# libmir/mir-optim

Measured on AMD Instinct MI355X. Metric: LM iterations/sec, higher is better.
Workload: dtype f64

## Files before the change

include/mir_optim_amd.h:

```cpp
#ifndef MIR_OPTIM_AMD_H
#define MIR_OPTIM_AMD_H

#include <stddef.h>
#include <stdint.h>

#ifdef __cplusplus
extern "C" {
#endif


typedef enum mir_least_squares_status {
    mir_ls_maxIterations = -1,
    mir_ls_furtherImprovement = 0,
    mir_ls_xConverged = 1,
    mir_ls_gConverged = 2,
    mir_ls_fConverged = 3,
    mir_ls_badBounds = -32,
    mir_ls_badGuess = -31,
    mir_ls_badMinStepQuality = -30,
    mir_ls_badGoodStepQuality = -29,
    mir_ls_badStepQuality = -28,
    mir_ls_badLambdaParams = -27,
    mir_ls_numericError = -26
} mir_least_squares_status;

typedef enum mir_box_qp_status {
    mir_box_qp_solved = 0,
    mir_box_qp_numericError = 1,
    mir_box_qp_maxIterations = 2
} mir_box_qp_status;

typedef struct mir_box_qp_settings_d { double relTolerance, absTolerance; uint32_t maxIterations; } mir_box_qp_settings_d;
typedef struct mir_box_qp_settings_s { float relTolerance, absTolerance; uint32_t maxIterations; } mir_box_qp_settings_s;

typedef struct mir_least_squares_settings_d {
    uint32_t maxIterations;
    uint32_t maxAge;
    double jacobianEpsilon;
    double absTolerance;
    double relTolerance;
    double gradTolerance;
    double maxGoodResidual;
    double maxStep;
    double maxLambda;
    double minLambda;
    double minStepQuality;
    double goodStepQuality;
    double lambdaIncrease;
    double lambdaDecrease;
    mir_box_qp_settings_d qpSettings;
} mir_least_squares_settings_d;

typedef struct mir_least_squares_settings_s {
    uint32_t maxIterations, maxAge;
    float jacobianEpsilon, absTolerance, relTolerance, gradTolerance, maxGoodResidual, maxStep,
          maxLambda, minLambda, minStepQuality, goodStepQuality, lambdaIncrease, lambdaDecrease;
    mir_box_qp_settings_s qpSettings;
} mir_least_squares_settings_s;

typedef struct mir_least_squares_result_d {
    int32_t status;
    uint32_t iterations, fCalls, gCalls;
    double residual;
    double lambda;
} mir_least_squares_result_d;
typedef struct mir_least_squares_result_s {
    int32_t status;
    uint32_t iterations, fCalls, gCalls;
    float residual, lambda;
} mir_least_squares_result_s;

typedef struct mir_slice_d { size_t length; double* ptr; } mir_slice_d;
typedef struct mir_slice_s { size_t length; float* ptr; } mir_slice_s;
typedef struct mir_slice_i { size_t length; int32_t* ptr; } mir_slice_i;

typedef void (*mir_least_squares_function_d)(void* context, size_t m, size_t n, const double* x, double* y);
typedef void (*mir_least_squares_jacobian_d)(void* context, size_t m, size_t n, const double* x, double* J);
typedef void (*mir_least_squares_function_s)(void* context, size_t m, size_t n, const float* x, float* y);
typedef void (*mir_least_squares_jacobian_s)(void* context, size_t m, size_t n, const float* x, float* J);

typedef struct mir_least_squares_task { void* context; void* function; } mir_least_squares_task;
typedef void (*mir_least_squares_task_function)(mir_least_squares_task task, uint32_t totalThreads,
                                                uint32_t threadId, uint32_t i);
typedef void (*mir_least_squares_thread_manager)(void* context, uint32_t count,
                                                 mir_least_squares_task taskContext,
                                                 mir_least_squares_task_function task);

size_t mir_least_squares_work_length(size_t m, size_t n);
size_t mir_least_squares_iwork_length(size_t m, size_t n);
size_t mir_box_qp_work_length(size_t n);
size_t mir_box_qp_iwork_length(size_t n);
size_t mir_box_qp_iwork_length_ilp64(size_t n);
size_t mir_least_squares_iwork_length_ilp64(size_t m, size_t n);
const char* mir_least_squares_status_string(mir_least_squares_status st);
void mir_least_squares_init_d(mir_least_squares_settings_d* settings);
void mir_least_squares_init_s(mir_least_squares_settings_s* settings);
void mir_least_squares_reset_d(mir_least_squares_settings_d* settings);
void mir_least_squares_reset_s(mir_least_squares_settings_s* settings);

mir_least_squares_result_d mir_optimize_least_squares_d(
    const mir_least_squares_settings_d* settings, size_t m, size_t n,
    double* x, const double* l, const double* u,
    mir_slice_d work, mir_slice_i iwork,
    void* fContext, mir_least_squares_function_d f,
    void* gContext, mir_least_squares_jacobian_d g,
    void* tmContext, mir_least_squares_thread_manager tm);

mir_least_squares_result_s mir_optimize_least_squares_s(
    const mir_least_squares_settings_s* settings, size_t m, size_t n,
    float* x, const float* l, const float* u,
    mir_slice_s work, mir_slice_i iwork,
    void* fContext, mir_least_squares_function_s f,
    void* gContext, mir_least_squares_jacobian_s g,
    void* tmContext, mir_least_squares_thread_manager tm);


typedef struct mir_lsq_comm mir_lsq_comm;
typedef struct mir_lsq_workspace mir_lsq_workspace;

typedef void (*mir_lsq_batched_function_d)(void* context, size_t m, size_t n, size_t p, const double* X, double* Y);
typedef void (*mir_lsq_batched_function_s)(void* context, size_t m, size_t n, size_t p, const float* X, float* Y);
enum {
    MIR_LSQ_DEVICE_CALLBACKS = 1u,
    MIR_LSQ_TIME_KERNELS = 2u
};

enum {
    MIR_LSQ_VARIANT_BROYDEN_REWRITE = 1u << 0,
    MIR_LSQ_VARIANT_FD_SEPARATE_FILL = 1u << 1,
    MIR_LSQ_VARIANT_NO_SPECULATION = 1u << 4,
    MIR_LSQ_VARIANT_NO_NULL_SKIP = 1u << 5,
    MIR_LSQ_VARIANT_SOLVE_BOUNDED = 1u << 6,
    MIR_LSQ_VARIANT_SOLVE_GENERIC = 1u << 10,
    MIR_LSQ_VARIANT_SOLVE_ONE_WORKGROUP = 1u << 11,
    MIR_LSQ_VARIANT_FD_HOST_COLUMNS = 1u << 13,
    MIR_LSQ_VARIANT_NO_PIPELINE = 1u << 22,
    MIR_LSQ_VARIANT_DEBUG_HELPERS_ABSENT = 1u << 12,
    MIR_LSQ_VARIANT_DEBUG_SOLVE = 1u << 7,
    MIR_LSQ_VARIANT_HOST_PROFILE = 1u << 8,
    MIR_LSQ_VARIANT_LR_CAP_SHIFT = 16
};

typedef struct mir_lsq_stats {
    uint64_t passes, accepted, rejected, step_guard_rejects;
    uint64_t jacobian_full, jacobian_broyden;
    uint64_t jtj_launches;
    uint64_t jtj_broyden_launches;
    double jtj_ms;
    double jtj_broyden_ms;
    double solve_ms;
    uint64_t solve_launches;
    double fd_ms;
    double total_ms;
    uint64_t qp_active_set_passes;
    uint64_t broyden_lr_columns;
    double jtj_fd_ms;
    uint64_t jtj_fd_launches;
    uint64_t elided_evaluations;
    uint64_t allreduce_calls[3];
    uint64_t allreduce_elems[3];
    uint64_t broyden_flushes;
    uint64_t jtj_resyncs;
    double fd_callback_ms;
    uint64_t fd_callback_calls, fd_callback_points;
    double trial_callback_ms;
    uint64_t trial_callback_calls, trial_callback_points;
    uint64_t library_launches;
    uint64_t round_launches[3];
    uint64_t rounds[3];
    double fd_host_wall_ms, fd_host_f_ms;
    uint64_t fd_host_columns;
    double host_f_ms;
    uint64_t host_f_calls;
    uint64_t fused_rounds;
    uint64_t fused_passes;
    uint64_t coop_timeouts;
} mir_lsq_stats;

typedef struct mir_lsq_trace_record {
    int32_t event;
    uint32_t iterations;
    double lambda, residual, trial_residual, dx_dot;
} mir_lsq_trace_record;
typedef struct mir_lsq_trace {
    mir_lsq_trace_record* records;
    uint64_t capacity;
    uint64_t count;
} mir_lsq_trace;

typedef struct mir_lsq_gpu_options {
    uint32_t struct_size;
    uint32_t flags;
    void* stream;
    mir_lsq_comm* comm;
    mir_lsq_workspace* workspace;
    void* fbContext;
    void* fb;
    uint32_t fd_batch;
    uint32_t variant;
    mir_lsq_stats* stats;
    mir_lsq_trace* trace;
    void* fbRowMajor;
    void* fbRowMajorDiff;
    uint32_t stats_size;
    uint32_t reserved0;
} mir_lsq_gpu_options;

mir_least_squares_result_d mir_optimize_least_squares_gpu_d(
    const mir_least_squares_settings_d* settings, size_t m, size_t n,
    double* x, const double* l, const double* u, const mir_lsq_gpu_options* options,
    void* fContext, mir_least_squares_function_d f,
    void* gContext, mir_least_squares_jacobian_d g,
    void* tmContext, mir_least_squares_thread_manager tm);
mir_least_squares_result_s mir_optimize_least_squares_gpu_s(
    const mir_least_squares_settings_s* settings, size_t m, size_t n,
    float* x, const float* l, const float* u, const mir_lsq_gpu_options* options,
    void* fContext, mir_least_squares_function_s f,
    void* gContext, mir_least_squares_jacobian_s g,
    void* tmContext, mir_least_squares_thread_manager tm);

int mir_solve_box_qp_gpu_d(const mir_box_qp_settings_d* settings, size_t n, const double* P,
                           const double* q, const double* l, const double* u, double* x,
                           int unconstrainedSolution, int* iterations);
int mir_solve_box_qp_gpu_s(const mir_box_qp_settings_s* settings, size_t n, const float* P,
                           const float* q, const float* l, const float* u, float* x,
                           int unconstrainedSolution, int* iterations);

enum { MIR_LSQ_MODEL_EXP_DECAY = 0, MIR_LSQ_MODEL_EXP3_AFFINE = 1,
       MIR_LSQ_MODEL_EXP_DECAY_PAD8 = 2 };
enum { MIR_LSQ_BATCHED_ANALYTIC_JACOBIAN = 2 };
enum { MIR_LSQ_BATCHED_NO_LADDER = 1 };
typedef struct mir_lsq_batched_options {
    uint32_t struct_size;
    uint32_t variant;
    void* stream;
    float* basis;
    size_t basis_bytes;
    uint64_t* timing;
} mir_lsq_batched_options;

int mir_optimize_least_squares_batched_s(const mir_least_squares_settings_s* settings, size_t count, size_t m, int model,
                                         float* x, const float* lower, const float* upper,
                                         const float* t, size_t t_stride, const float* data,
                                         mir_least_squares_result_s* results, const mir_lsq_batched_options* options);

enum { MIR_LSQ_BATCHED_NEEDS_GENERAL = -100 };
int mir_lsq_batched_kernel_s(const mir_least_squares_settings_s* settings, size_t count, size_t m, int model,
                             float* x, const float* lower, const float* upper,
                             const float* t, size_t t_stride, const float* data,
                             mir_least_squares_result_s* results, const mir_lsq_batched_options* options);

int mir_optimize_least_squares_batched_d(const mir_least_squares_settings_d* settings, size_t count, size_t m, int model,
                                         double* x, const double* lower, const double* upper,
                                         const double* t, size_t t_stride, const double* data,
                                         mir_least_squares_result_d* results, const mir_lsq_batched_options* options);
int mir_lsq_batched_kernel_d(const mir_least_squares_settings_d* settings, size_t count, size_t m, int model,
                             double* x, const double* lower, const double* upper,
                             const double* t, size_t t_stride, const double* data,
                             mir_least_squares_result_d* results, const mir_lsq_batched_options* options);

enum { MIR_LSQ_BATCHED_ABSOLUTE_SIGMA = 1u };
typedef struct mir_lsq_batched_extras {
    uint32_t struct_size;
    uint32_t flags;
    const void* weights;
    size_t weight_stride;
    void* covariance;
} mir_lsq_batched_extras;
int mir_optimize_least_squares_batched_ex_s(const mir_least_squares_settings_s* settings, size_t count, size_t m, int model,
                                            float* x, const float* lower, const float* upper,
                                            const float* t, size_t t_stride, const float* data,
                                            mir_least_squares_result_s* results, const mir_lsq_batched_options* options,
                                            const mir_lsq_batched_extras* extras);
int mir_optimize_least_squares_batched_ex_d(const mir_least_squares_settings_d* settings, size_t count, size_t m, int model,
                                            double* x, const double* lower, const double* upper,
                                            const double* t, size_t t_stride, const double* data,
                                            mir_least_squares_result_d* results, const mir_lsq_batched_options* options,
                                            const mir_lsq_batched_extras* extras);
int mir_lsq_batched_kernel_ex_s(const mir_least_squares_settings_s* settings, size_t count, size_t m, int model,
                                float* x, const float* lower, const float* upper,
                                const float* t, size_t t_stride, const float* data,
                                mir_least_squares_result_s* results, const mir_lsq_batched_options* options,
                                const mir_lsq_batched_extras* extras);
int mir_lsq_batched_kernel_ex_d(const mir_least_squares_settings_d* settings, size_t count, size_t m, int model,
                                double* x, const double* lower, const double* upper,
                                const double* t, size_t t_stride, const double* data,
                                mir_least_squares_result_d* results, const mir_lsq_batched_options* options,
                                const mir_lsq_batched_extras* extras);
int mir_lsq_batched_covariance_s(const mir_least_squares_settings_s* settings, size_t count, size_t m, int model,
                                 const float* x, const float* lower, const float* upper,
                                 const float* t, size_t t_stride, const float* data,
                                 const mir_least_squares_result_s* results, const mir_lsq_batched_options* options,
                                 const mir_lsq_batched_extras* extras);
int mir_lsq_batched_covariance_d(const mir_least_squares_settings_d* settings, size_t count, size_t m, int model,
                                 const double* x, const double* lower, const double* upper,
                                 const double* t, size_t t_stride, const double* data,
                                 const mir_least_squares_result_d* results, const mir_lsq_batched_options* options,
                                 const mir_lsq_batched_extras* extras);

enum { MIR_LSQ_RESIDENT_NO_NULL_SKIP = 1u,
       MIR_LSQ_RESIDENT_UNBOUNDED = 2u,
       MIR_LSQ_RESIDENT_NO_LOOKAHEAD = 4u,
       MIR_LSQ_RESIDENT_DEBUG_DROP_WORKGROUP = 16u,
       MIR_LSQ_RESIDENT_ANALYTIC_JACOBIAN = 32u,
       MIR_LSQ_RESIDENT_NO_STAMPS = 8u           };
typedef struct mir_lsq_resident_stats {
    uint64_t rounds, passes, accepted, rejected, step_guard_rejects, jacobian_full, jacobian_broyden, qp_active_set_passes,
        elided_evaluations;
    uint64_t t_total, t_stage, t_worker, t_group, t_total_wait, t_solver, t_solve_body, t_cmd_wait;
    uint64_t t_w_eval, t_w_fd, t_w_prod;
    uint64_t t_w_mma;
    uint64_t lookahead_rejections;
    uint64_t t_look;
    uint64_t t_unpack, t_publish;
    uint32_t abort_code, grid, rows, groups;
} mir_lsq_resident_stats;
typedef struct mir_lsq_resident_options {
    uint32_t struct_size;
    uint32_t variant;
    void* stream;
    void* workspace;
    size_t workspace_bytes;
    mir_lsq_trace_record* trace_records;
    uint32_t trace_capacity;
    uint32_t max_workgroups;
    uint32_t* trace_count;
    mir_lsq_resident_stats* stats;
} mir_lsq_resident_options;

int mir_lsq_batched_posvx_s(size_t count, size_t n, const float* P, const float* rhs, float* x, int* info, void* stream);
int mir_lsq_batched_posvx_d(size_t count, size_t n, const double* P, const double* rhs, double* x, int* info, void* stream);

int mir_lsq_jtj_d(size_t m, size_t n, double* J, const double* y, const double* y_old, const double* dx,
                  int broyden, double* JJ, double* Jy, void* stream, float* kernel_ms);
int mir_lsq_jtj_s(size_t m, size_t n, float* J, const float* y, const float* y_old, const float* dx,
                  int broyden, float* JJ, float* Jy, void* stream, float* kernel_ms);
int mir_lsq_fd_jtj_d(size_t m, size_t n, const double* Yrm, const double* twh, const double* y, double* J,
                     double* JJ, double* Jy, void* stream, float* kernel_ms);
int mir_lsq_fd_diff_jtj_d(size_t m, size_t n, const double* Drm, const double* twh, const double* y, double* J,
                          double* JJ, double* Jy, void* stream, float* kernel_ms);
int mir_lsq_jtj_plan(size_t elem_size, size_t m, size_t n, int num_cu, int op, int aligned16, size_t out[10]);

mir_lsq_workspace* mir_lsq_workspace_create(size_t m, size_t n, size_t elem_size);
void mir_lsq_workspace_destroy(mir_lsq_workspace* ws);

int mir_lsq_rccl_unique_id(void* out_128_bytes);
mir_lsq_comm* mir_lsq_comm_create_rccl(int nranks, int rank, const void* unique_id_128_bytes);
typedef void (*mir_lsq_allreduce_fn)(void* ctx, double* device_buf, size_t count, void* stream);
mir_lsq_comm* mir_lsq_comm_create_callback(int nranks, int rank, mir_lsq_allreduce_fn fn, void* ctx);
int mir_lsq_comm_create_local_group(int nranks, mir_lsq_comm** out_comms);
void mir_lsq_comm_destroy(mir_lsq_comm* comm);
int mir_lsq_comm_record(mir_lsq_comm* comm, double* host_buf, size_t capacity);
size_t mir_lsq_comm_recorded(const mir_lsq_comm* comm);
mir_lsq_comm* mir_lsq_comm_create_replay(int nranks, int rank, const double* totals_host, size_t len, mir_lsq_comm* inner);
int mir_lsq_comm_replay_rewind(mir_lsq_comm* comm);
int mir_lsq_comm_replay_set_delay(mir_lsq_comm* comm, unsigned microseconds);
int mir_lsq_comm_ranks(const mir_lsq_comm* comm);
int mir_lsq_comm_describe(const mir_lsq_comm* comm, char* buf, size_t len);
int mir_lsq_comm_allreduce_d(mir_lsq_comm* comm, double* buf, size_t count, void* stream);
int mir_lsq_comm_allreduce_s(mir_lsq_comm* comm, float* buf, size_t count, void* stream);

int mir_lsq_device_count(void);
void* mir_lsq_device_malloc(size_t bytes);
void mir_lsq_device_free(void* p);
int mir_lsq_memcpy_h2d(void* dst_device, const void* src_host, size_t bytes, void* stream);
int mir_lsq_memcpy_d2h(void* dst_host, const void* src_device, size_t bytes, void* stream);
int mir_lsq_memcpy_d2d(void* dst_device, const void* src_device, size_t bytes, void* stream);

int mir_lsq_selftest_reductions(int rounds, int mismatches[4]);
void* mir_lsq_stream_create(void);
void mir_lsq_stream_destroy(void* stream);
int mir_lsq_stream_synchronize(void* stream);
const char* mir_lsq_version(void);

enum { MIR_FIT_SPLINE_OK = 0, MIR_FIT_SPLINE_TOO_FEW_POINTS = 1, MIR_FIT_SPLINE_BAD_ARGUMENT = 2 };

int mir_fit_spline_d(const mir_least_squares_settings_d* settings, size_t npoints, const double* points, size_t nx,
                     const double* x, const double* l, const double* u, double lambda, double (*dist)(double, double),
                     double* splineY, double* splineD, mir_least_squares_result_d* result);
int mir_fit_spline_s(const mir_least_squares_settings_s* settings, size_t npoints, const float* points, size_t nx,
                     const float* x, const float* l, const float* u, float lambda, float (*dist)(float, float),
                     float* splineY, float* splineD, mir_least_squares_result_s* result);
void mir_fit_spline_residuals_d(size_t npoints, const double* points, size_t nx, const double* x, double lambda,
                                const double* splineY, size_t m, double* y);
void mir_spline_c2_derivatives_d(size_t n, const double* x, const double* y, double* d);
void mir_spline_c2_derivatives_s(size_t n, const float* x, const float* y, float* d);
void mir_spline_eval_d(size_t n, const double* x, const double* y, const double* d, double t, double* out3);
void mir_spline_eval_s(size_t n, const float* x, const float* y, const float* d, float t, float* out3);

#ifdef __cplusplus
}
#endif
#endif
```

mir_optim_amd/api.py:

```python
import ctypes as C
import enum
import os

import numpy as np

from . import build as _build

__all__ = [
    "LeastSquaresStatus", "BoxQPStatus", "LeastSquaresSettings", "LeastSquaresResult", "BoxQPSettings",
    "LeastSquaresException", "optimize", "optimizeLeastSquares", "solveBoxQP", "leastSquaresStatusString",
    "mir_least_squares_work_length", "mir_least_squares_iwork_length", "mir_box_qp_work_length",
    "mir_box_qp_iwork_length", "GpuOptions", "Stats", "lib", "workloads_lib", "device_count",
    "DeviceBuffer", "Stream", "jtj", "fd_jtj", "DEVICE_CALLBACKS", "TIME_KERNELS", "optimizeLeastSquaresBatched", "batchedPosvx", "BATCHED_NO_LADDER",
    "MODEL_EXP_DECAY", "MODEL_EXP3_AFFINE", "MODEL_EXP_DECAY_PAD8", "ResultS", "Trace", "TraceRecord", "Spline", "FitSplineResult", "fitSpline",
    "fit_spline_residuals", "variant_lr_cap",
    "VARIANT_BROYDEN_REWRITE", "VARIANT_FD_SEPARATE_FILL", "VARIANT_NO_SPECULATION", "VARIANT_NO_NULL_SKIP",
    "VARIANT_SOLVE_BOUNDED", "VARIANT_DEBUG_SOLVE", "VARIANT_HOST_PROFILE", "VARIANT_SOLVE_GENERIC", "VARIANT_SOLVE_ONE_WORKGROUP", "VARIANT_DEBUG_HELPERS_ABSENT", "VARIANT_FD_HOST_COLUMNS",
    "VARIANT_NO_PIPELINE", "BatchedOptions", "BatchedExtras", "BATCHED_ABSOLUTE_SIGMA",
]

MODEL_EXP_DECAY = 0
MODEL_EXP3_AFFINE = 1
MODEL_EXP_DECAY_PAD8 = 2

DEVICE_CALLBACKS = 1
TIME_KERNELS = 2

VARIANT_BROYDEN_REWRITE = 1 << 0
VARIANT_FD_SEPARATE_FILL = 1 << 1
VARIANT_NO_SPECULATION = 1 << 4
VARIANT_NO_NULL_SKIP = 1 << 5
VARIANT_SOLVE_BOUNDED = 1 << 6
VARIANT_DEBUG_SOLVE = 1 << 7
VARIANT_HOST_PROFILE = 1 << 8
VARIANT_SOLVE_GENERIC = 1 << 10
VARIANT_SOLVE_ONE_WORKGROUP = 1 << 11
VARIANT_DEBUG_HELPERS_ABSENT = 1 << 12
VARIANT_FD_HOST_COLUMNS = 1 << 13
VARIANT_NO_PIPELINE = 1 << 22


def variant_lr_cap(k):
    return (int(k) & 31) << 16


class LeastSquaresStatus(enum.IntEnum):
    maxIterations = -1
    furtherImprovement = 0
    xConverged = 1
    gConverged = 2
    fConverged = 3
    badBounds = -32
    badGuess = -31
    badMinStepQuality = -30
    badGoodStepQuality = -29
    badStepQuality = -28
    badLambdaParams = -27
    numericError = -26


class BoxQPStatus(enum.IntEnum):
    solved = 0
    numericError = 1
    maxIterations = 2


class LeastSquaresException(Exception):

    def __init__(self, status, result=None):
        self.status = LeastSquaresStatus(status)
        self.result = result
        super().__init__("mir-optim Least Squares: " + leastSquaresStatusString(status))


class _QPd(C.Structure):
    _fields_ = [("relTolerance", C.c_double), ("absTolerance", C.c_double), ("maxIterations", C.c_uint32)]


class _QPs(C.Structure):
    _fields_ = [("relTolerance", C.c_float), ("absTolerance", C.c_float), ("maxIterations", C.c_uint32)]


_FIELDS = ["jacobianEpsilon", "absTolerance", "relTolerance", "gradTolerance", "maxGoodResidual", "maxStep",
           "maxLambda", "minLambda", "minStepQuality", "goodStepQuality", "lambdaIncrease", "lambdaDecrease"]


class _Sd(C.Structure):
    _fields_ = ([("maxIterations", C.c_uint32), ("maxAge", C.c_uint32)] + [(k, C.c_double) for k in _FIELDS]
                + [("qpSettings", _QPd)])


class _Ss(C.Structure):
    _fields_ = ([("maxIterations", C.c_uint32), ("maxAge", C.c_uint32)] + [(k, C.c_float) for k in _FIELDS]
                + [("qpSettings", _QPs)])


class _Rd(C.Structure):
    _fields_ = [("status", C.c_int32), ("iterations", C.c_uint32), ("fCalls", C.c_uint32), ("gCalls", C.c_uint32),
                ("residual", C.c_double), ("lambda_", C.c_double)]


class _Rs(C.Structure):
    _fields_ = [("status", C.c_int32), ("iterations", C.c_uint32), ("fCalls", C.c_uint32), ("gCalls", C.c_uint32),
                ("residual", C.c_float), ("lambda_", C.c_float)]


ResultS = _Rs


class _SliceD(C.Structure):
    _fields_ = [("length", C.c_size_t), ("ptr", C.c_void_p)]


class _Task(C.Structure):
    _fields_ = [("context", C.c_void_p), ("function", C.c_void_p)]


class Stats(C.Structure):
    _fields_ = [("passes", C.c_uint64), ("accepted", C.c_uint64), ("rejected", C.c_uint64),
                ("step_guard_rejects", C.c_uint64), ("jacobian_full", C.c_uint64), ("jacobian_broyden", C.c_uint64),
                ("jtj_launches", C.c_uint64), ("jtj_broyden_launches", C.c_uint64), ("jtj_ms", C.c_double),
                ("jtj_broyden_ms", C.c_double), ("solve_ms", C.c_double), ("solve_launches", C.c_uint64),
                ("fd_ms", C.c_double), ("total_ms", C.c_double), ("qp_active_set_passes", C.c_uint64),
                ("broyden_lr_columns", C.c_uint64),
                ("jtj_fd_ms", C.c_double), ("jtj_fd_launches", C.c_uint64),
                ("elided_evaluations", C.c_uint64),
                ("allreduce_calls", C.c_uint64 * 3), ("allreduce_elems", C.c_uint64 * 3),
                ("broyden_flushes", C.c_uint64), ("jtj_resyncs", C.c_uint64),
                ("fd_callback_ms", C.c_double), ("fd_callback_calls", C.c_uint64), ("fd_callback_points", C.c_uint64),
                ("trial_callback_ms", C.c_double), ("trial_callback_calls", C.c_uint64),
                ("trial_callback_points", C.c_uint64),
                ("library_launches", C.c_uint64), ("round_launches", C.c_uint64 * 3), ("rounds", C.c_uint64 * 3),
                ("fd_host_wall_ms", C.c_double), ("fd_host_f_ms", C.c_double), ("fd_host_columns", C.c_uint64),
                ("host_f_ms", C.c_double), ("host_f_calls", C.c_uint64),
                ("fused_rounds", C.c_uint64), ("fused_passes", C.c_uint64), ("coop_timeouts", C.c_uint64)]

    def as_dict(self):
        return {k: (list(getattr(self, k)) if isinstance(getattr(self, k), C.Array) else getattr(self, k)) for k, _ in self._fields_}


class TraceRecord(C.Structure):
    _fields_ = [("event", C.c_int32), ("iterations", C.c_uint32), ("lambda_", C.c_double), ("residual", C.c_double),
                ("trial_residual", C.c_double), ("dx_dot", C.c_double)]


class _TraceHeader(C.Structure):
    _fields_ = [("records", C.POINTER(TraceRecord)), ("capacity", C.c_uint64), ("count", C.c_uint64)]


class Trace:

    EVENTS = {0: "jacobian_full", 1: "jacobian_broyden", 2: "rejected", 3: "accepted", 4: "step_guard"}

    def __init__(self, capacity=4096):
        self._buf = (TraceRecord * capacity)()
        self.header = _TraceHeader(C.cast(self._buf, C.POINTER(TraceRecord)), capacity, 0)

    @property
    def count(self):
        return int(self.header.count)

    def records(self):
        k = min(self.count, int(self.header.capacity))
        return [(r.event, r.iterations, r.lambda_, r.residual, r.trial_residual, r.dx_dot) for r in self._buf[:k]]


class GpuOptions(C.Structure):
    _fields_ = [("struct_size", C.c_uint32), ("flags", C.c_uint32), ("stream", C.c_void_p), ("comm", C.c_void_p),
                ("workspace", C.c_void_p), ("fbContext", C.c_void_p), ("fb", C.c_void_p), ("fd_batch", C.c_uint32),
                ("variant", C.c_uint32), ("stats", C.POINTER(Stats)), ("trace", C.POINTER(_TraceHeader)),
                ("fbRowMajor", C.c_void_p), ("fbRowMajorDiff", C.c_void_p), ("stats_size", C.c_uint32),
                ("reserved0", C.c_uint32)]

    def __init__(self, **kw):
        super().__init__(**kw)
        self.struct_size = C.sizeof(GpuOptions)
        self.stats_size = C.sizeof(Stats)


class BatchedOptions(C.Structure):
    _fields_ = [("struct_size", C.c_uint32), ("variant", C.c_uint32), ("stream", C.c_void_p), ("basis", C.c_void_p),
                ("basis_bytes", C.c_size_t), ("timing", C.c_void_p)]

    def __init__(self, **kw):
        super().__init__(**kw)
        self.struct_size = C.sizeof(BatchedOptions)


class BatchedExtras(C.Structure):
    _fields_ = [("struct_size", C.c_uint32), ("flags", C.c_uint32), ("weights", C.c_void_p), ("weight_stride", C.c_size_t),
                ("covariance", C.c_void_p)]

    def __init__(self, **kw):
        super().__init__(**kw)
        self.struct_size = C.sizeof(BatchedExtras)


TASK_FN = C.CFUNCTYPE(None, _Task, C.c_uint32, C.c_uint32, C.c_uint32)
TM_FN = C.CFUNCTYPE(None, C.c_void_p, C.c_uint32, _Task, TASK_FN)
ALLREDUCE_FN = C.CFUNCTYPE(None, C.c_void_p, C.c_void_p, C.c_size_t, C.c_void_p)


def _ftype(dtype):
    ct = C.c_double if dtype == np.float64 else C.c_float
    return C.CFUNCTYPE(None, C.c_void_p, C.c_size_t, C.c_size_t, C.POINTER(ct), C.POINTER(ct))


_lib = None
_wl = None


def _load(path):
    if not os.path.exists(path):
        raise ImportError(f"{path} is missing: build it with `python -m mir_optim_amd.build` "
                          "(hipcc --offload-arch=gfx950). mir_optim_amd has no CPU fallback.")
    return C.CDLL(path, mode=C.RTLD_GLOBAL)


def lib():
    global _lib
    if _lib is None:
        L = _load(_build.SOLVER_LIB)
        sz = C.c_size_t
        for name in ("mir_least_squares_work_length", "mir_least_squares_iwork_length"):
            getattr(L, name).restype = sz
            getattr(L, name).argtypes = [sz, sz]
        for name in ("mir_box_qp_work_length", "mir_box_qp_iwork_length"):
            getattr(L, name).restype = sz
            getattr(L, name).argtypes = [sz]
        L.mir_box_qp_iwork_length_ilp64.restype = sz
        L.mir_box_qp_iwork_length_ilp64.argtypes = [sz]
        L.mir_least_squares_iwork_length_ilp64.restype = sz
        L.mir_least_squares_iwork_length_ilp64.argtypes = [sz, sz]
        L.mir_least_squares_status_string.restype = C.c_char_p
        L.mir_least_squares_status_string.argtypes = [C.c_int]
        for suf, S, R in (("d", _Sd, _Rd), ("s", _Ss, _Rs)):
            getattr(L, "mir_least_squares_init_" + suf).argtypes = [C.POINTER(S)]
            getattr(L, "mir_least_squares_reset_" + suf).argtypes = [C.POINTER(S)]
            fn = getattr(L, "mir_optimize_least_squares_" + suf)
            fn.restype = R
            fn.argtypes = [C.POINTER(S), sz, sz, C.c_void_p, C.c_void_p, C.c_void_p, _SliceD, _SliceD,
                           C.c_void_p, C.c_void_p, C.c_void_p, C.c_void_p, C.c_void_p, C.c_void_p]
            fn = getattr(L, "mir_optimize_least_squares_gpu_" + suf)
            fn.restype = R
            fn.argtypes = [C.POINTER(S), sz, sz, C.c_void_p, C.c_void_p, C.c_void_p, C.POINTER(GpuOptions),
                           C.c_void_p, C.c_void_p, C.c_void_p, C.c_void_p, C.c_void_p, C.c_void_p]
            fn = getattr(L, "mir_solve_box_qp_gpu_" + suf)
            fn.restype = C.c_int
            fn.argtypes = [C.c_void_p, sz, C.c_void_p, C.c_void_p, C.c_void_p, C.c_void_p, C.c_void_p, C.c_int,
                           C.POINTER(C.c_int)]
            fn = getattr(L, "mir_lsq_jtj_" + suf)
            fn.restype = C.c_int
            fn.argtypes = [sz, sz, C.c_void_p, C.c_void_p, C.c_void_p, C.c_void_p, C.c_int, C.c_void_p, C.c_void_p,
                           C.c_void_p, C.POINTER(C.c_float)]
        L.mir_lsq_comm_create_local_group.restype = C.c_int
        L.mir_lsq_comm_create_local_group.argtypes = [C.c_int, C.POINTER(C.c_void_p)]
        L.mir_lsq_fd_diff_jtj_d.restype = C.c_int
        L.mir_lsq_fd_diff_jtj_d.argtypes = [sz, sz, C.c_void_p, C.c_void_p, C.c_void_p, C.c_void_p, C.c_void_p, C.c_void_p,
                                            C.c_void_p, C.POINTER(C.c_float)]
        L.mir_lsq_fd_jtj_d.restype = C.c_int
        L.mir_lsq_fd_jtj_d.argtypes = [sz, sz, C.c_void_p, C.c_void_p, C.c_void_p, C.c_void_p, C.c_void_p, C.c_void_p,
                                       C.c_void_p, C.c_void_p]
        L.mir_optimize_least_squares_batched_s.restype = C.c_int
        L.mir_optimize_least_squares_batched_s.argtypes = [C.POINTER(_Ss), sz, sz, C.c_int, C.c_void_p, C.c_void_p, C.c_void_p,
                                                           C.c_void_p, sz, C.c_void_p, C.c_void_p, C.POINTER(BatchedOptions)]
        L.mir_lsq_batched_kernel_s.restype = C.c_int
        L.mir_lsq_batched_kernel_s.argtypes = [C.POINTER(_Ss), sz, sz, C.c_int, C.c_void_p, C.c_void_p, C.c_void_p,
                                               C.c_void_p, sz, C.c_void_p, C.c_void_p, C.POINTER(BatchedOptions)]
        L.mir_lsq_jtj_plan.restype = C.c_int
        L.mir_lsq_jtj_plan.argtypes = [sz, sz, sz, C.c_int, C.c_int, C.c_int, C.POINTER(sz * 10)]
        L.mir_lsq_selftest_reductions.restype = C.c_int
        L.mir_lsq_selftest_reductions.argtypes = [C.c_int, C.POINTER(C.c_int * 4)]
        L.mir_lsq_batched_posvx_s.restype = C.c_int
        L.mir_lsq_batched_posvx_s.argtypes = [sz, sz, C.c_void_p, C.c_void_p, C.c_void_p, C.c_void_p, C.c_void_p]
        L.mir_optimize_least_squares_batched_d.restype = C.c_int
        L.mir_optimize_least_squares_batched_d.argtypes = [C.POINTER(_Sd), sz, sz, C.c_int, C.c_void_p, C.c_void_p, C.c_void_p,
                                                           C.c_void_p, sz, C.c_void_p, C.c_void_p, C.POINTER(BatchedOptions)]
        L.mir_lsq_batched_kernel_d.restype = C.c_int
        L.mir_lsq_batched_kernel_d.argtypes = [C.POINTER(_Sd), sz, sz, C.c_int, C.c_void_p, C.c_void_p, C.c_void_p,
                                               C.c_void_p, sz, C.c_void_p, C.c_void_p, C.POINTER(BatchedOptions)]
        L.mir_lsq_batched_posvx_d.restype = C.c_int
        L.mir_lsq_batched_posvx_d.argtypes = [sz, sz, C.c_void_p, C.c_void_p, C.c_void_p, C.c_void_p, C.c_void_p]
        for suf, S in (("s", _Ss), ("d", _Sd)):
            for name in ("mir_optimize_least_squares_batched_ex_", "mir_lsq_batched_kernel_ex_", "mir_lsq_batched_covariance_"):
                fn = getattr(L, name + suf)
                fn.restype = C.c_int
                fn.argtypes = [C.POINTER(S), sz, sz, C.c_int, C.c_void_p, C.c_void_p, C.c_void_p, C.c_void_p, sz, C.c_void_p,
                               C.c_void_p, C.POINTER(BatchedOptions), C.POINTER(BatchedExtras)]
        L.mir_lsq_comm_describe.restype = C.c_int
        L.mir_lsq_comm_describe.argtypes = [C.c_void_p, C.c_char_p, C.c_size_t]
        L.mir_lsq_workspace_create.restype = C.c_void_p
        L.mir_lsq_workspace_create.argtypes = [sz, sz, sz]
        L.mir_lsq_workspace_destroy.argtypes = [C.c_void_p]
        L.mir_lsq_rccl_unique_id.restype = C.c_int
        L.mir_lsq_rccl_unique_id.argtypes = [C.c_void_p]
        L.mir_lsq_comm_create_rccl.restype = C.c_void_p
        L.mir_lsq_comm_create_rccl.argtypes = [C.c_int, C.c_int, C.c_void_p]
        L.mir_lsq_comm_create_callback.restype = C.c_void_p
        L.mir_lsq_comm_create_callback.argtypes = [C.c_int, C.c_int, ALLREDUCE_FN, C.c_void_p]
        L.mir_lsq_comm_destroy.argtypes = [C.c_void_p]
        L.mir_lsq_comm_record.restype = C.c_int
        L.mir_lsq_comm_record.argtypes = [C.c_void_p, C.c_void_p, sz]
        L.mir_lsq_comm_recorded.restype = sz
        L.mir_lsq_comm_recorded.argtypes = [C.c_void_p]
        L.mir_lsq_comm_create_replay.restype = C.c_void_p
        L.mir_lsq_comm_create_replay.argtypes = [C.c_int, C.c_int, C.c_void_p, sz, C.c_void_p]
        L.mir_lsq_comm_replay_rewind.restype = C.c_int
        L.mir_lsq_comm_replay_rewind.argtypes = [C.c_void_p]
        L.mir_lsq_comm_replay_set_delay.restype = C.c_int
        L.mir_lsq_comm_replay_set_delay.argtypes = [C.c_void_p, C.c_uint]
        L.mir_lsq_comm_ranks.restype = C.c_int
        L.mir_lsq_comm_ranks.argtypes = [C.c_void_p]
        for name in ("mir_lsq_comm_allreduce_d", "mir_lsq_comm_allreduce_s"):
            getattr(L, name).restype = C.c_int
            getattr(L, name).argtypes = [C.c_void_p, C.c_void_p, sz, C.c_void_p]
        L.mir_lsq_device_count.restype = C.c_int
        L.mir_lsq_device_malloc.restype = C.c_void_p
        L.mir_lsq_device_malloc.argtypes = [sz]
        L.mir_lsq_device_free.argtypes = [C.c_void_p]
        for name in ("mir_lsq_memcpy_h2d", "mir_lsq_memcpy_d2h", "mir_lsq_memcpy_d2d"):
            getattr(L, name).restype = C.c_int
            getattr(L, name).argtypes = [C.c_void_p, C.c_void_p, sz, C.c_void_p]
        L.mir_lsq_stream_create.restype = C.c_void_p
        L.mir_lsq_stream_destroy.argtypes = [C.c_void_p]
        L.mir_lsq_stream_synchronize.restype = C.c_int
        L.mir_lsq_stream_synchronize.argtypes = [C.c_void_p]
        L.mir_lsq_version.restype = C.c_char_p
        for suf, S, R, ct in (("d", _Sd, _Rd, C.c_double), ("s", _Ss, _Rs, C.c_float)):
            fn = getattr(L, "mir_fit_spline_" + suf)
            fn.restype = C.c_int
            fn.argtypes = [C.POINTER(S), sz, C.c_void_p, sz, C.c_void_p, C.c_void_p, C.c_void_p, ct, C.c_void_p,
                           C.c_void_p, C.c_void_p, C.POINTER(R)]
            getattr(L, "mir_spline_c2_derivatives_" + suf).argtypes = [sz, C.c_void_p, C.c_void_p, C.c_void_p]
            getattr(L, "mir_spline_eval_" + suf).argtypes = [sz, C.c_void_p, C.c_void_p, C.c_void_p, ct, C.c_void_p]
        L.mir_fit_spline_residuals_d.argtypes = [sz, C.c_void_p, sz, C.c_void_p, C.c_double, C.c_void_p, sz, C.c_void_p]
        _lib = L
    return _lib


def workloads_lib():
    global _wl
    if _wl is None:
        W = _load(_build.WORKLOADS_LIB)
        W.wl_uniform.argtypes = [C.c_uint64, C.c_uint64, C.c_size_t, C.c_void_p]
        W.wl_tanh_linear_generate.argtypes = [C.c_size_t, C.c_size_t, C.c_size_t, C.c_double, C.c_void_p, C.c_void_p,
                                              C.c_void_p, C.c_void_p]
        _wl = W
    return _wl


def device_count():
    return lib().mir_lsq_device_count()


def leastSquaresStatusString(st):
    return lib().mir_least_squares_status_string(int(st)).decode()


def mir_least_squares_work_length(m, n):
    return lib().mir_least_squares_work_length(m, n)


def mir_least_squares_iwork_length(m, n):
    return lib().mir_least_squares_iwork_length(m, n)


def mir_box_qp_work_length(n):
    return lib().mir_box_qp_work_length(n)


def mir_box_qp_iwork_length(n):
    return lib().mir_box_qp_iwork_length(n)


def LeastSquaresSettings(dtype=np.float64):
    s = _Sd() if dtype == np.float64 else _Ss()
    (lib().mir_least_squares_init_d if dtype == np.float64 else lib().mir_least_squares_init_s)(C.byref(s))
    return s


def BoxQPSettings(dtype=np.float64):
    return LeastSquaresSettings(dtype).qpSettings


class LeastSquaresResult:

    def __init__(self, raw):
        self.status = LeastSquaresStatus(raw.status)
        self.iterations = raw.iterations
        self.fCalls = raw.fCalls
        self.gCalls = raw.gCalls
        self.residual = raw.residual
        self.lambda_ = raw.lambda_

    def __repr__(self):
        return (f"LeastSquaresResult(status={self.status.name}, iterations={self.iterations}, fCalls={self.fCalls}, "
                f"gCalls={self.gCalls}, residual={self.residual!r}, lambda={self.lambda_!r})")


class Stream:
    def __init__(self):
        self.handle = lib().mir_lsq_stream_create()
        if not self.handle:
            raise RuntimeError("hipStreamCreate failed (no GPU?)")

    def synchronize(self):
        if lib().mir_lsq_stream_synchronize(self.handle) != 0:
            raise RuntimeError("stream synchronize failed")

    def close(self):
        if self.handle:
            lib().mir_lsq_stream_destroy(self.handle)
            self.handle = None

    def __del__(self):
        try:
            self.close()
        except Exception:
            pass


class DeviceBuffer:

    def __init__(self, array=None, nbytes=None, dtype=None, shape=None):
        if array is not None:
            array = np.ascontiguousarray(array)
            nbytes, dtype, shape = array.nbytes, array.dtype, array.shape
        self.nbytes, self.dtype, self.shape = int(nbytes), np.dtype(dtype), tuple(shape)
        self.ptr = lib().mir_lsq_device_malloc(max(self.nbytes, 8))
        if not self.ptr:
            raise MemoryError(f"hipMalloc({self.nbytes}) failed (no GPU?)")
        if array is not None:
            self.upload(array)

    def upload(self, array):
        array = np.ascontiguousarray(array, dtype=self.dtype)
        assert array.nbytes == self.nbytes
        if lib().mir_lsq_memcpy_h2d(self.ptr, array.ctypes.data, self.nbytes, None) != 0:
            raise RuntimeError("H2D copy failed")

    def upload_at(self, byte_offset, array):
        array = np.ascontiguousarray(array, dtype=self.dtype)
        assert 0 <= byte_offset and byte_offset + array.nbytes <= self.nbytes
        if lib().mir_lsq_memcpy_h2d(self.ptr + byte_offset, array.ctypes.data, array.nbytes, None) != 0:
            raise RuntimeError("H2D copy failed")

    def download(self):
        out = np.empty(self.shape, dtype=self.dtype)
        if lib().mir_lsq_memcpy_d2h(out.ctypes.data, self.ptr, self.nbytes, None) != 0:
            raise RuntimeError("D2H copy failed")
        return out

    def free(self):
        if self.ptr:
            lib().mir_lsq_device_free(self.ptr)
            self.ptr = None

    def __del__(self):
        try:
            self.free()
        except Exception:
            pass


def _as_fnptr(cb, ftype, wrap, keep):
    if cb is None:
        return C.c_void_p(None)
    if callable(cb):
        c = ftype(wrap(cb))
        keep.append(c)
        return C.cast(c, C.c_void_p)
    return C.c_void_p(int(cb))


def optimizeLeastSquares(f, m, x, l=None, u=None, g=None, tm=None, settings=None, dtype=np.float64,
                         fContext=None, gContext=None, options=None, gpu_entry=None):
    L = lib()
    dbl = dtype == np.float64
    x = np.ascontiguousarray(x, dtype=dtype)
    n = x.size
    lo = np.full(n, -np.inf, dtype=dtype) if l is None else np.ascontiguousarray(l, dtype=dtype)
    up = np.full(n, np.inf, dtype=dtype) if u is None else np.ascontiguousarray(u, dtype=dtype)
    if settings is None:
        settings = LeastSquaresSettings(dtype)
    ft = _ftype(dtype)
    keep = []
    errors = []

    def wrap_f(fn):
        def cb(_ctx, m_, n_, xp, yp):
            yv = np.ctypeslib.as_array(yp, shape=(m_,))
            try:
                xv = np.ctypeslib.as_array(xp, shape=(n_,))
                yv[:] = 0
                fn(xv, yv)
            except BaseException as e:
                errors.append(e)
                yv[:] = np.nan
        return cb

    def wrap_g(fn):
        def cb(_ctx, m_, n_, xp, Jp):
            Jv = np.ctypeslib.as_array(Jp, shape=(m_ * n_,)).reshape(m_, n_)
            try:
                xv = np.ctypeslib.as_array(xp, shape=(n_,))
                Jv[:] = 0
                fn(xv, Jv)
            except BaseException as e:
                errors.append(e)
                Jv[:] = np.nan
        return cb

    fptr = _as_fnptr(f, ft, wrap_f, keep)
    gptr = _as_fnptr(g, ft, wrap_g, keep)
    tmptr = C.c_void_p(None)
    if tm is not None:
        def tm_cb(_ctx, count, task, taskfn):
            try:
                tm(count, lambda total, tid, i: taskfn(task, total, tid, i))
            except BaseException as e:
                errors.append(e)
        tmc = TM_FN(tm_cb)
        keep.append(tmc)
        tmptr = C.cast(tmc, C.c_void_p)
    use_gpu_entry = gpu_entry if gpu_entry is not None else (options is not None)
    suf = "d" if dbl else "s"
    if use_gpu_entry:
        fn = getattr(L, "mir_optimize_least_squares_gpu_" + suf)
        raw = fn(C.byref(settings), m, n, x.ctypes.data, lo.ctypes.data, up.ctypes.data,
                 C.byref(options) if options is not None else None, fContext, fptr, gContext, gptr, None, tmptr)
    else:
        wl = L.mir_least_squares_work_length(m, n)
        iwl = L.mir_least_squares_iwork_length(m, n)
        iwork = np.zeros(iwl + 4, dtype=np.int32)
        work_slice = _SliceD(wl, None)
        iwork_slice = _SliceD(iwl, iwork.ctypes.data)
        fn = getattr(L, "mir_optimize_least_squares_" + suf)
        raw = fn(C.byref(settings), m, n, x.ctypes.data, lo.ctypes.data, up.ctypes.data, work_slice, iwork_slice,
                 fContext, fptr, gContext, gptr, None, tmptr)
    del keep
    if errors:
        raise errors[0]
    return LeastSquaresResult(raw), x


def optimize(f, m, x, l=None, u=None, g=None, tm=None, settings=None, dtype=np.float64, taskPool=None, **kw):
    if taskPool is not None and tm is None:
        import threading
        workers = max(1, getattr(taskPool, "_max_workers", 1))
        ids = {}
        lock = threading.Lock()

        def tm(count, task):
            def run(i):
                with lock:
                    tid = ids.setdefault(threading.get_ident(), len(ids))
                task(workers, tid % workers, i)
            list(taskPool.map(run, range(count)))
    res, xo = optimizeLeastSquares(f, m, x, l, u, g, tm, settings, dtype, **kw)
    if res.status < 0:
        raise LeastSquaresException(res.status, res)
    return res, xo


def _batched_suffix(dtype):
    if np.dtype(dtype) == np.float32:
        return "s"
    if np.dtype(dtype) == np.float64:
        return "d"
    raise ValueError(f"the batched entries exist in float32 and float64, not {np.dtype(dtype)}")


def optimizeLeastSquaresBatched(model, x, t, data, l=None, u=None, settings=None, variant=0, dtype=np.float32, weights=None,
                                covariance=False, absolute_sigma=False):
    suf = _batched_suffix(dtype)
    dtype = np.float32 if suf == "s" else np.float64
    L = lib()
    x = np.array(x, dtype=dtype, order="C")
    count, n = x.shape
    data = np.ascontiguousarray(data, dtype=dtype)
    m = data.shape[1]
    t = np.ascontiguousarray(t, dtype=dtype)
    t_stride = 0 if t.ndim == 1 else m
    lo = np.full(n, -np.inf, dtype=dtype) if l is None else np.ascontiguousarray(l, dtype=dtype)
    up = np.full(n, np.inf, dtype=dtype) if u is None else np.ascontiguousarray(u, dtype=dtype)
    if settings is None:
        settings = LeastSquaresSettings(dtype)
    raw = ((_Rs if suf == "s" else _Rd) * count)()
    if weights is None and not covariance and not absolute_sigma:
        fn = getattr(L, "mir_optimize_least_squares_batched_" + suf)
        rc = fn(C.byref(settings), count, m, int(model), x.ctypes.data, lo.ctypes.data, up.ctypes.data, t.ctypes.data, t_stride,
                data.ctypes.data, raw, C.byref(BatchedOptions(variant=variant)))
        if rc != 0:
            raise RuntimeError(f"mir_optimize_least_squares_batched_{suf} failed: {rc}")
        return [LeastSquaresResult(r) for r in raw], x
    ex = BatchedExtras(flags=BATCHED_ABSOLUTE_SIGMA if absolute_sigma else 0)
    if weights is not None:
        weights = np.ascontiguousarray(weights, dtype=dtype)
        if weights.shape not in ((m,), (count, m)):
            raise ValueError(f"weights: {m} values or {count} x {m}, not {weights.shape}")
        ex.weights = weights.ctypes.data
        ex.weight_stride = 0 if weights.ndim == 1 else m
    cov = np.empty((count, n, n), dtype=dtype) if covariance else None
    if covariance:
        ex.covariance = cov.ctypes.data
    fn = getattr(L, "mir_optimize_least_squares_batched_ex_" + suf)
    rc = fn(C.byref(settings), count, m, int(model), x.ctypes.data, lo.ctypes.data, up.ctypes.data, t.ctypes.data, t_stride,
            data.ctypes.data, raw, C.byref(BatchedOptions(variant=variant)), C.byref(ex))
    if rc != 0:
        raise RuntimeError(f"mir_optimize_least_squares_batched_ex_{suf} failed: {rc}")
    res = [LeastSquaresResult(r) for r in raw]
    return (res, x, cov) if covariance else (res, x)


BATCHED_NO_LADDER = 1
BATCHED_ABSOLUTE_SIGMA = 1


def batchedPosvx(P, rhs, dtype=np.float32):
    suf = _batched_suffix(dtype)
    dtype = np.float32 if suf == "s" else np.float64
    L = lib()
    P = np.asarray(P, dtype=dtype)
    count, n = P.shape[0], P.shape[1]
    Pp = np.zeros((count, 8, 8), dtype=dtype); Pp[:, :n, :n] = P
    bp = np.zeros((count, 8), dtype=dtype); bp[:, :n] = rhs
    dP, db = DeviceBuffer(Pp), DeviceBuffer(bp)
    dx = DeviceBuffer(nbytes=count * 8 * np.dtype(dtype).itemsize, dtype=dtype, shape=(count, 8))
    di = DeviceBuffer(nbytes=count * 4, dtype=np.int32, shape=(count,))
    st = Stream()
    rc = getattr(L, "mir_lsq_batched_posvx_" + suf)(count, n, dP.ptr, db.ptr, dx.ptr, di.ptr, st.handle)
    if rc != 0:
        raise RuntimeError(f"mir_lsq_batched_posvx_{suf} failed: {rc}")
    st.synchronize()
    x, info = dx.download()[:, :n].copy(), di.download().copy()
    for b in (dP, db, dx, di):
        b.free()
    return x, info


def solveBoxQP(P, q, l, u, x=None, settings=None, dtype=np.float64, unconstrainedSolution=False):
    L = lib()
    P = np.ascontiguousarray(P, dtype=dtype)
    n = P.shape[0]
    q = np.ascontiguousarray(q, dtype=dtype)
    l = np.ascontiguousarray(l, dtype=dtype)
    u = np.ascontiguousarray(u, dtype=dtype)
    xo = np.zeros(n, dtype=dtype) if x is None else np.ascontiguousarray(x, dtype=dtype).copy()
    if settings is None:
        settings = BoxQPSettings(dtype)
    it = C.c_int(0)
    fn = L.mir_solve_box_qp_gpu_d if dtype == np.float64 else L.mir_solve_box_qp_gpu_s
    st = fn(C.byref(settings), n, P.ctypes.data, q.ctypes.data, l.ctypes.data, u.ctypes.data, xo.ctypes.data,
            1 if unconstrainedSolution else 0, C.byref(it))
    return BoxQPStatus(st), xo, it.value


def jtj(J, y, y_old=None, dx=None, dtype=np.float64):
    L = lib()
    J = np.ascontiguousarray(J, dtype=dtype)
    m, n = J.shape
    dJ = DeviceBuffer(J)
    dy = DeviceBuffer(np.ascontiguousarray(y, dtype=dtype))
    broyden = dx is not None
    dyo = DeviceBuffer(np.ascontiguousarray(y_old if broyden else y, dtype=dtype))
    ddx = DeviceBuffer(np.ascontiguousarray(dx if broyden else np.zeros(n), dtype=dtype))
    dJJ = DeviceBuffer(nbytes=n * n * J.itemsize, dtype=dtype, shape=(n, n))
    dJy = DeviceBuffer(nbytes=n * J.itemsize, dtype=dtype, shape=(n,))
    ms = C.c_float(0)
    fn = L.mir_lsq_jtj_d if dtype == np.float64 else L.mir_lsq_jtj_s
    rc = fn(m, n, dJ.ptr, dy.ptr, dyo.ptr, ddx.ptr, 1 if broyden else 0, dJJ.ptr, dJy.ptr, None, C.byref(ms))
    if rc != 0:
        raise RuntimeError(f"mir_lsq_jtj failed: {rc}")
    out = dJJ.download(), dJy.download(), dJ.download(), ms.value
    for b in (dJ, dy, dyo, ddx, dJJ, dJy):
        b.free()
    return out


JTJ_OPS = ("plain", "rewrite", "fd", "fd_diff")
JTJ_FAMILIES = ("none", "stream", "fdp", "pc32", "ring8", "fdp8", "wide")


def jtj_plan(elem_size, m, n, num_cu, op, aligned=True):
    out = (C.c_size_t * 10)()
    rc = lib().mir_lsq_jtj_plan(elem_size, m, n, num_cu, JTJ_OPS.index(op), int(bool(aligned)), C.byref(out))
    if rc != 0:
        raise ValueError(f"mir_lsq_jtj_plan: {rc}")
    d = dict(zip(("family", "ncb", "flat", "grid", "jobs", "lds", "slabs", "slab_len", "reduce_ncb", "workspace_slab_elems"), map(int, out)))
    d["family"] = JTJ_FAMILIES[d["family"]]
    return d


def fd_jtj(Yrm, twh, y, diff=False):
    L = lib()
    Yrm = np.ascontiguousarray(Yrm, dtype=np.float64)
    m, n2 = Yrm.shape
    n = n2 if diff else n2 // 2
    dY = DeviceBuffer(Yrm)
    dt = DeviceBuffer(np.ascontiguousarray(twh, dtype=np.float64))
    dy = DeviceBuffer(np.ascontiguousarray(y, dtype=np.float64))
    dJ = DeviceBuffer(nbytes=m * n * 8, dtype=np.float64, shape=(m, n))
    dJJ = DeviceBuffer(nbytes=n * n * 8, dtype=np.float64, shape=(n, n))
    dJy = DeviceBuffer(nbytes=n * 8, dtype=np.float64, shape=(n,))
    ms = C.c_float(0)
    rc = (L.mir_lsq_fd_diff_jtj_d if diff else L.mir_lsq_fd_jtj_d)(m, n, dY.ptr, dt.ptr, dy.ptr, dJ.ptr, dJJ.ptr, dJy.ptr, None, C.byref(ms))
    if rc != 0:
        raise RuntimeError(f"mir_lsq_fd_jtj_d failed: {rc}")
    out = dJ.download(), dJJ.download(), dJy.download(), ms.value
    for b in (dY, dt, dy, dJ, dJJ, dJy):
        b.free()
    return out



class Spline:

    def __init__(self, x, values, dtype=np.float64):
        self.dtype = dtype
        self.x = np.ascontiguousarray(x, dtype=dtype)
        self.values = np.ascontiguousarray(values, dtype=dtype)
        self.derivatives = np.zeros_like(self.values)
        suf = "d" if dtype == np.float64 else "s"
        getattr(lib(), "mir_spline_c2_derivatives_" + suf)(self.x.size, self.x.ctypes.data, self.values.ctypes.data,
                                                         self.derivatives.ctypes.data)
        self._eval = getattr(lib(), "mir_spline_eval_" + suf)

    def withTwoDerivatives(self, t):
        out = np.zeros(3, dtype=self.dtype)
        self._eval(self.x.size, self.x.ctypes.data, self.values.ctypes.data, self.derivatives.ctypes.data, t, out.ctypes.data)
        return out

    def __call__(self, t):
        if np.ndim(t) == 0:
            return self.withTwoDerivatives(float(t))[0]
        return np.array([self.withTwoDerivatives(float(v))[0] for v in np.asarray(t).ravel()]).reshape(np.shape(t))


class FitSplineResult:

    def __init__(self, leastSquaresResult, spline):
        self.leastSquaresResult = leastSquaresResult
        self.spline = spline


def fit_spline_residuals(points, x, lambda_, splineY):
    points = np.ascontiguousarray(points, dtype=np.float64)
    x = np.ascontiguousarray(x, dtype=np.float64)
    v = np.ascontiguousarray(splineY, dtype=np.float64)
    m = points.shape[0] + (1 if lambda_ == 0 else 0)
    y = np.zeros(m)
    lib().mir_fit_spline_residuals_d(points.shape[0], points.ctypes.data, x.size, x.ctypes.data, lambda_, v.ctypes.data, m,
                                     y.ctypes.data)
    return y


def fitSpline(settings, points, x, l, u, lambda_=0.0, dtype=np.float64):
    L = lib()
    points = np.ascontiguousarray(points, dtype=dtype)
    x = np.ascontiguousarray(x, dtype=dtype)
    lo = np.ascontiguousarray(l, dtype=dtype)
    up = np.ascontiguousarray(u, dtype=dtype)
    if not lambda_ >= 0:
        raise ValueError("fitSpline: lambda has to be non-negative")
    y = np.zeros(x.size, dtype=dtype)
    d = np.zeros(x.size, dtype=dtype)
    dbl = dtype == np.float64
    raw = (_Rd if dbl else _Rs)()
    fn = L.mir_fit_spline_d if dbl else L.mir_fit_spline_s
    rc = fn(C.byref(settings) if settings is not None else None, points.shape[0], points.ctypes.data, x.size,
            x.ctypes.data, lo.ctypes.data, up.ctypes.data, lambda_, None, y.ctypes.data, d.ctypes.data, C.byref(raw))
    if rc == 1:
        raise Exception("fitSpline: points.length has to be greater or equal x.length when lambda is 0.0")
    if rc != 0:
        raise ValueError("fitSpline: bad argument")
    res = LeastSquaresResult(raw)
    if res.status < 0:
        raise LeastSquaresException(int(res.status), res)
    return FitSplineResult(res, Spline(x, y, dtype))
```

mir_optim_amd/csrc/broyden_launch.h:

```cpp
#pragma once

#include "common.h"
#include "solve_types.h"

namespace mirlsq {

template <typename T>
struct LrArgs {
    const T* J;
    T* U;
    const T* D;
    const T* dx;
    const T* dx_dot;
    const T* y;
    const T* y_old;
    T* partials;
    size_t m;
    int n;
    int k;
    const ChainRec<T>* spec_rec;
    T absTolerance, relTolerance;
};

constexpr int kLrMaxBlocks = 1024;
inline int lr_blocks(size_t m, int num_cu)
{
    const size_t G = (m + 3) / 4;
    size_t want = (G + 4 * 8 - 1) / (4 * 8);
    size_t cap = (size_t)num_cu * 4;
    if (cap > (size_t)kLrMaxBlocks) cap = kLrMaxBlocks;
    if (want > cap) want = cap;
    return (int)(want ? want : 1);
}

template <typename T> hipError_t lr_sweep(const LrArgs<T>& a, int nblk, hipStream_t s);
template <typename T> hipError_t lr_reduce(const T* partials, int nblk, int n, T* out, hipStream_t s);
template <typename T> hipError_t lr_finish(const T* lr, T* D, const T* dx, int k, int n, T* JJ, T* Jy, LmState<T>* st, hipStream_t s);
template <typename T> hipError_t lr_sumsq(const T* v, size_t m, int count, size_t vstride, T* partials, int pstride, int nblk, hipStream_t s);
template <typename T> hipError_t lr_sumsq_final(const T* partials, int pstride, int nblk, int count, T* out, hipStream_t s);
template <typename T> hipError_t lr_flush(T* J, const T* U, const T* D, int k, size_t m, int n, int num_cu, hipStream_t s);

}
```

mir_optim_amd/csrc/broyden_lr.h:

```cpp
#pragma once

#include "broyden_launch.h"
#include "common.h"
#include "solve_types.h"

namespace mirlsq {


template <typename T> struct LrPair;
template <> struct LrPair<double> { using type = double2; };
template <> struct LrPair<float> { using type = float2; };



template <typename T>
__device__ __forceinline__ bool lr_spec_go(const ChainRec<T>& r, T absTolerance, T relTolerance)
{
    const T dxn = dsqrt(r.new_dx_dot);
    return r.qp_status == 0 && !(r.flags & (kFlagDxNaN | kFlagXNaN | kFlagStepTooLong | kFlagNullStep | kFlagGradSmall))
        && (dxn > absTolerance && r.trial_xnorm > dxn * relTolerance);
}

template <typename T>
__device__ __forceinline__ T lr_wave_sumsq(const T* __restrict__ y, size_t m, size_t gb, size_t ge, int q)
{
    T yy = 0;
    for (size_t g0 = gb; g0 < ge; g0 += 8) {
        T v[8];
#pragma unroll
        for (int e = 0; e < 8; ++e) {
            const size_t row = 4 * (g0 + e) + q;
            v[e] = (g0 + e < ge && row < m) ? y[row] : T(0);
        }
#pragma unroll
        for (int e = 0; e < 8; ++e)
            if (g0 + e < ge) yy = dfma(v[e], v[e], yy);
    }
    yy += wave_shfl_xor(yy, 16);
    yy += wave_shfl_xor(yy, 32);
    return yy;
}

template <typename T, int NCP, bool VEC>
__global__ __launch_bounds__(256, (NCP <= 4 ? 4 : 1)) void k_broyden_lr(const LrArgs<T> a)
{
    using P2 = typename LrPair<T>::type;
    __shared__ T red[4][lr_len(kLrMaxN)];
    __shared__ T coef[kLrMax];
    const int lane = threadIdx.x & 63, wave = threadIdx.x >> 6;
    const int q = lane >> 4, p = lane & 15;
    const int n = a.n, k = a.k;
    const size_t m = a.m;
    const size_t G = (m + 3) / 4;
    const size_t nw = (size_t)gridDim.x * 4, wid = (size_t)blockIdx.x * 4 + wave;
    const size_t per = (G + nw - 1) / nw;
    const size_t gb = wid * per;
    const size_t ge = gb + per < G ? gb + per : G;
    if (a.spec_rec && !lr_spec_go(a.spec_rec[0], a.absTolerance, a.relTolerance)) {
        const T yy = lr_wave_sumsq(a.y, m, gb, ge, q);
        if (q == 0 && p == 0) red[wave][0] = yy;
        __syncthreads();
        const int len = lr_len(n);
        T* out = a.partials + (size_t)blockIdx.x * len;
        for (int e = threadIdx.x; e < len; e += blockDim.x) out[e] = e == lr_yy(n) ? (red[0][0] + red[1][0]) + (red[2][0] + red[3][0]) : T(0);
        return;
    }

    for (int l = wave; l < k; l += 4) {
        T s = 0;
        for (int j = lane; j < n; j += kWave) s += a.D[(size_t)l * n + j] * a.dx[j];
        s = wave_sum(s);
        if (lane == 0) coef[l] = s;
    }
    T d0[NCP], d1[NCP];
    int coff[NCP];
    bool ok0[NCP], ok1[NCP];
#pragma unroll
    for (int c = 0; c < NCP; ++c) {
        const int col = 32 * c + 2 * p;
        ok0[c] = col < n;
        ok1[c] = col + 1 < n;
        coff[c] = ok0[c] ? col : 0;
        const T t0 = a.dx[ok0[c] ? col : 0], t1 = a.dx[ok1[c] ? col + 1 : 0];
        d0[c] = ok0[c] ? t0 : T(0);
        d1[c] = ok1[c] ? t1 : T(0);
    }
    __syncthreads();
    const bool own = p < k;
    const T cp = own ? coef[p] : T(0);
    const T* __restrict__ Up = a.U + (size_t)(own ? p : 0) * m;
    T* __restrict__ Uk = a.U + (size_t)k * m;
    const T nd = -(T(1) / *a.dx_dot);

    T va0[NCP], va1[NCP], ga0[NCP], ga1[NCP];
#pragma unroll
    for (int c = 0; c < NCP; ++c) { va0[c] = 0; va1[c] = 0; ga0[c] = 0; ga1[c] = 0; }
    T wl = 0, hl = 0, uu = 0, uy = 0, yy = 0;

    constexpr int UNR = NCP == 1 ? 4 : (NCP == 2 ? 2 : 1);
    for (size_t g0 = gb; g0 < ge; g0 += UNR) {
        T v0[UNR][NCP], v1[UNR][NCP], ynv[UNR], yov[UNR], ulv[UNR];
#pragma unroll
        for (int e = 0; e < UNR; ++e) {
            const size_t g = g0 + e < ge ? g0 + e : ge - 1;
            const size_t row = 4 * g + q;
            const size_t rr = row < m ? row : m - 1;
            const T* __restrict__ rp = a.J + rr * (size_t)n;
#pragma unroll
            for (int c = 0; c < NCP; ++c) {
                if constexpr (VEC) {
                    typedef T lr_v2 __attribute__((ext_vector_type(2)));
                    const lr_v2 t = __builtin_nontemporal_load(reinterpret_cast<const lr_v2*>(rp + coff[c]));
                    v0[e][c] = t.x;
                    v1[e][c] = t.y;
                } else {
                    v0[e][c] = rp[coff[c]];
                    v1[e][c] = rp[ok1[c] ? coff[c] + 1 : 0];
                }
            }
            ynv[e] = a.y[rr];
            yov[e] = a.y_old[rr];
            ulv[e] = own ? Up[rr] : T(0);
        }
#pragma unroll
        for (int e = 0; e < UNR; ++e) {
            if (g0 + e < ge) {
                const size_t row = 4 * (g0 + e) + q;
                const bool rok = row < m;
                T yn = ynv[e];
                const T yo = yov[e], ul = ulv[e];
                T s = ul * cp;
#pragma unroll
                for (int c = 0; c < NCP; ++c) s += v0[e][c] * d0[c] + v1[e][c] * d1[c];
                s = sum16(s);
                T u = nd * ((yo - yn) + s);
                if (!rok) { u = 0; yn = 0; }
                if (rok && p == 0) Uk[row] = u;
#pragma unroll
                for (int c = 0; c < NCP; ++c) {
                    va0[c] += v0[e][c] * u;
                    va1[c] += v1[e][c] * u;
                    ga0[c] += v0[e][c] * yn;
                    ga1[c] += v1[e][c] * yn;
                }
                wl += ul * u;
                hl += ul * yn;
                uu += u * u;
                uy += u * yn;
                yy = dfma(yn, yn, yy);
            }
        }
    }

    auto qsum = [](T v) { v += wave_shfl_xor(v, 16); v += wave_shfl_xor(v, 32); return v; };
#pragma unroll
    for (int c = 0; c < NCP; ++c) { va0[c] = qsum(va0[c]); va1[c] = qsum(va1[c]); ga0[c] = qsum(ga0[c]); ga1[c] = qsum(ga1[c]); }
    wl = qsum(wl); hl = qsum(hl); uu = qsum(uu); uy = qsum(uy); yy = qsum(yy);
    if (q == 0) {
#pragma unroll
        for (int c = 0; c < NCP; ++c) {
            if (ok0[c]) { red[wave][coff[c]] = va0[c]; red[wave][n + coff[c]] = ga0[c]; }
            if (ok1[c]) { red[wave][coff[c] + 1] = va1[c]; red[wave][n + coff[c] + 1] = ga1[c]; }
        }
        red[wave][2 * n + p] = wl;
        red[wave][2 * n + kLrMax + p] = hl;
        if (p == 0) { red[wave][2 * n + 2 * kLrMax] = uu; red[wave][2 * n + 2 * kLrMax + 1] = uy; red[wave][lr_yy(n)] = yy; }
    }
    __syncthreads();
    const int len = lr_len(n);
    T* out = a.partials + (size_t)blockIdx.x * len;
    for (int e = threadIdx.x; e < len; e += blockDim.x) out[e] = (red[0][e] + red[1][e]) + (red[2][e] + red[3][e]);
}

template <typename T>
__global__ __launch_bounds__(32 * kReduceRanges) void k_lr_reduce(const T* __restrict__ partials, int nparts, int len, T* __restrict__ out)
{
    __shared__ T part[kReduceRanges][33];
    const int es = threadIdx.x & 31, sp = threadIdx.x >> 5;
    const int e = blockIdx.x * 32 + es;
    T s = 0;
    if (e < len) {
        const int per = (nparts + kReduceRanges - 1) / kReduceRanges;
        const int b0 = sp * per, b1 = (b0 + per < nparts) ? b0 + per : nparts;
#pragma unroll 8
        for (int b = b0; b < b1; ++b) s += partials[(size_t)b * len + e];
    }
    part[sp][es] = s;
    __syncthreads();
    if (sp == 0 && e < len) {
        T tot = part[0][es];
#pragma unroll
        for (int r = 1; r < kReduceRanges; ++r) tot += part[r][es];
        out[e] = tot;
    }
}

template <typename T>
__device__ inline T lr_reduce_scalar(const T* __restrict__ partials, int nparts, T* part )
{
    if ((int)threadIdx.x < kReduceRanges) {
        const int per = (nparts + kReduceRanges - 1) / kReduceRanges;
        const int b0 = (int)threadIdx.x * per, b1 = (b0 + per < nparts) ? b0 + per : nparts;
        T s = 0;
#pragma unroll 8
        for (int b = b0; b < b1; ++b) s += partials[b];
        part[threadIdx.x] = s;
    }
    __syncthreads();
    T tot = part[0];
#pragma unroll
    for (int r = 1; r < kReduceRanges; ++r) tot += part[r];
    __syncthreads();
    return tot;
}

template <typename T>
__global__ __launch_bounds__(256) void k_lr_sumsq(const T* __restrict__ v0, size_t m, size_t vstride, T* __restrict__ partials0, int pstride)
{
    __shared__ T red[4];
    const int lane = threadIdx.x & 63, wave = threadIdx.x >> 6;
    const T* __restrict__ v = v0 + (size_t)blockIdx.y * vstride;
    const size_t G = (m + 3) / 4;
    const size_t nw = (size_t)gridDim.x * 4, wid = (size_t)blockIdx.x * 4 + wave;
    const size_t per = (G + nw - 1) / nw;
    const size_t gb = wid * per;
    const size_t ge = gb + per < G ? gb + per : G;
    const T yy = lr_wave_sumsq(v, m, gb, ge, lane >> 4);
    if (lane == 0) red[wave] = yy;
    __syncthreads();
    if (threadIdx.x == 0) partials0[(size_t)blockIdx.y * pstride + blockIdx.x] = (red[0] + red[1]) + (red[2] + red[3]);
}
template <typename T>
__global__ __launch_bounds__(256) void k_lr_sumsq_final(const T* __restrict__ partials0, int pstride, int nparts, T* __restrict__ out)
{
    __shared__ T part[kReduceRanges];
    const T tot = lr_reduce_scalar(partials0 + (size_t)blockIdx.x * pstride, nparts, part);
    if (threadIdx.x == 0) out[blockIdx.x] = tot;
}

template <typename T>
__global__ __launch_bounds__(256) void k_lr_finish(const T* __restrict__ lr, T* __restrict__ D, const T* __restrict__ dx,
                                                   int k, int n, T* __restrict__ JJ, T* __restrict__ Jy, LmState<T>* st)
{
    __shared__ T v[kLrMaxN];
    __shared__ T red[4];
    const T* __restrict__ w = lr + 2 * n;
    const T* __restrict__ h = w + kLrMax;
    const T uu = lr[2 * n + 2 * kLrMax], uy = lr[2 * n + 2 * kLrMax + 1];
    const int i = blockIdx.x;
    if (i < n) {
        for (int j = threadIdx.x; j < n; j += blockDim.x) {
            T s = lr[j];
            for (int l = 0; l < k; ++l) s = dfma(D[(size_t)l * n + j], w[l], s);
            v[j] = s;
        }
        __syncthreads();
        for (int j = threadIdx.x; j < n; j += blockDim.x) {
            const int r = i >= j ? i : j, c = i >= j ? j : i;
            JJ[(size_t)i * n + j] += lr_jj_term(v[r], v[c], dx[r], dx[c], uu);
        }
        return;
    }
    T mx = 0;
    for (int j = threadIdx.x; j < n; j += blockDim.x) {
        T s = lr[n + j];
        for (int l = 0; l < k; ++l) s = dfma(D[(size_t)l * n + j], h[l], s);
        s = dfma(dx[j], uy, s);
        Jy[j] = s;
        const T av = dabs(s);
        if (av > mx) mx = av;
        D[(size_t)k * n + j] = dx[j];
    }
    mx = wave_max(mx);
    if ((threadIdx.x & 63) == 0) red[threadIdx.x >> 6] = mx;
    __syncthreads();
    if (threadIdx.x == 0) {
        T r = red[0];
        for (int wv = 1; wv < (int)(blockDim.x >> 6); ++wv) r = red[wv] > r ? red[wv] : r;
        st->jy_inf = r;
    }
}

template <typename T, int NCP, bool VEC>
__global__ __launch_bounds__(256) void k_lr_flush(T* J, const T* __restrict__ U, const T* __restrict__ D,
                                                  int k, size_t m, int n)
{
    using P2 = typename LrPair<T>::type;
    extern __shared__ unsigned char lr_smem[];
    T* Ds = reinterpret_cast<T*>(lr_smem);
    for (int e = threadIdx.x; e < k * n; e += blockDim.x) Ds[e] = D[e];
    __syncthreads();
    const int lane = threadIdx.x & 63;
    const int q = lane >> 4, p = lane & 15;
    int coff[NCP];
    bool ok0[NCP], ok1[NCP];
#pragma unroll
    for (int c = 0; c < NCP; ++c) {
        const int col = 32 * c + 2 * p;
        ok0[c] = col < n;
        ok1[c] = col + 1 < n;
        coff[c] = ok0[c] ? col : 0;
    }
    const size_t G = (m + 3) / 4;
    const size_t wave_id = ((size_t)blockIdx.x * blockDim.x + threadIdx.x) >> 6;
    const size_t nwaves = ((size_t)gridDim.x * blockDim.x) >> 6;
    for (size_t g = wave_id; g < G; g += nwaves) {
        const size_t row = 4 * g + q;
        const bool rok = row < m;
        const size_t rr = rok ? row : m - 1;
        T* rp = J + rr * (size_t)n;
        const T* sp = rp;
        T v0[NCP], v1[NCP];
#pragma unroll
        for (int c = 0; c < NCP; ++c) {
            if constexpr (VEC) {
                typedef T lr_v2 __attribute__((ext_vector_type(2)));
                const lr_v2 t = __builtin_nontemporal_load(reinterpret_cast<const lr_v2*>(sp + coff[c]));
                v0[c] = t.x;
                v1[c] = t.y;
            } else {
                v0[c] = sp[coff[c]];
                v1[c] = sp[ok1[c] ? coff[c] + 1 : 0];
            }
        }
        for (int l = 0; l < k; ++l) {
            const T ul = U[(size_t)l * m + rr];
#pragma unroll
            for (int c = 0; c < NCP; ++c) {
                v0[c] += ul * Ds[l * n + coff[c]];
                v1[c] += ul * Ds[l * n + (ok1[c] ? coff[c] + 1 : 0)];
            }
        }
        if (rok) {
#pragma unroll
            for (int c = 0; c < NCP; ++c) {
                if constexpr (VEC) {
                    if (ok0[c]) {
                        typedef T lr_v2 __attribute__((ext_vector_type(2)));
                        lr_v2 t; t.x = v0[c]; t.y = v1[c];
                        __builtin_nontemporal_store(t, reinterpret_cast<lr_v2*>(rp + coff[c]));
                    }
                } else {
                    if (ok0[c]) rp[coff[c]] = v0[c];
                    if (ok1[c]) rp[coff[c] + 1] = v1[c];
                }
            }
        }
    }
}

}
```

mir_optim_amd/csrc/driver.h:

```cpp
#pragma once

#include <hip/hip_runtime.h>

#include <atomic>
#include <chrono>
#include <cmath>
#include <cstdlib>
#include <cstring>
#include <mutex>
#include <thread>
#include <vector>

#include "../../include/mir_optim_amd.h"
#include "broyden_launch.h"
#include "comm.h"
#include "common.h"
#include "jtj_plan.h"
#include "solve_launch.h"
#include "solve_types.h"

struct mir_lsq_workspace {
    size_t m = 0, n = 0, elem = 0;
    void* dev = nullptr;
    size_t dev_bytes = 0;
    void* ypanel = nullptr;
    size_t ypanel_bytes = 0;
    void* ytrial = nullptr;
    void* ulr = nullptr;
    int device = 0;
    std::vector<hipEvent_t> event_pool;
    void* pinned = nullptr;
    void* pinned_dev = nullptr;
    void* pinned_y = nullptr;
    void* pinned_J = nullptr;
    void* pinned_panel = nullptr;
    size_t pinned_panel_bytes = 0;
    static constexpr int kCopyStreams = 4;
    hipStream_t copy_stream[kCopyStreams] = {nullptr, nullptr, nullptr, nullptr};
    hipEvent_t copy_event[kCopyStreams] = {nullptr, nullptr, nullptr, nullptr};
    int num_cu = 256;
    uint32_t solve_epoch = 0;
};

namespace mirlsq {

template <typename T> struct Abi;
template <> struct Abi<double> {
    using Settings = mir_least_squares_settings_d;
    using Result = mir_least_squares_result_d;
    using F = mir_least_squares_function_d;
    using G = mir_least_squares_jacobian_d;
    using FB = mir_lsq_batched_function_d;
};
template <> struct Abi<float> {
    using Settings = mir_least_squares_settings_s;
    using Result = mir_least_squares_result_s;
    using F = mir_least_squares_function_s;
    using G = mir_least_squares_jacobian_s;
    using FB = mir_lsq_batched_function_s;
};

inline size_t align_up(size_t v, size_t a) { return (v + a - 1) / a * a; }

template <typename Settings>
int bad_settings(const Settings* S)
{
    using T = decltype(Settings::minStepQuality);
    if (!(0 <= S->minStepQuality && S->minStepQuality < 1)) return mir_ls_badMinStepQuality;
    if (!(0 <= S->goodStepQuality && S->goodStepQuality <= 1)) return mir_ls_badGoodStepQuality;
    if (!(S->minStepQuality < S->goodStepQuality)) return mir_ls_badStepQuality;
    if (!(1 <= S->lambdaIncrease && S->lambdaIncrease <= std::sqrt(Lim<T>::max))) return mir_ls_badLambdaParams;
    if (!(std::sqrt(Lim<T>::min_normal) <= S->lambdaDecrease && S->lambdaDecrease <= 1)) return mir_ls_badLambdaParams;
    return 0;
}

inline void cpu_relax()
{
#if defined(__x86_64__) || defined(__i386__)
    __builtin_ia32_pause();
#elif defined(__aarch64__)
    asm volatile("yield" ::: "memory");
#else
    std::atomic_signal_fence(std::memory_order_seq_cst);
#endif
}

bool device_available();
int query_num_cu();

template <typename T>
struct Buffers {
    T *J, *y, *mB, *ytmp;
    T *X, *twh;
    T *x, *lower, *upper, *dx, *dx_acc, *trial, *Jy, *JJ, *packed, *partials, *sum;
    LmState<T>* st;
    ChainRec<T>* rec;
    T* slabs;
    T *lrD, *lrvec, *lrpart;
    SolveScratch<T> sc[kChainMax];
    size_t bytes;
};

constexpr int kPartials = 1024;

template <typename T> Buffers<T> carve(void* base, size_t m, size_t n, int num_cu);
template <typename T> mir_lsq_workspace* workspace_create(size_t m, size_t n);
void workspace_destroy(mir_lsq_workspace* ws);

struct EventPair { hipEvent_t a, b; int kind; };

template <typename T>
struct Solver {
    using Settings = typename Abi<T>::Settings;
    using Result = typename Abi<T>::Result;
    using F = typename Abi<T>::F;
    using G = typename Abi<T>::G;
    using FB = typename Abi<T>::FB;

    const Settings* S;
    size_t m;
    uint32_t n;
    T* xh;
    const T *lh, *uh;
    void* fctx; F f;
    void* gctx; G g;
    void* tmctx; mir_least_squares_thread_manager tm;
    void* fbctx; FB fb;
    FB fbr = nullptr;
    FB fbd = nullptr;
    int fd_fused = 0;
    int sums_pending = 0;
    uint32_t fd_batch;
    bool device_cb;
    bool time_kernels;
    mir_lsq_comm* comm;
    mir_lsq_stats* stats;
    mir_lsq_trace* trace = nullptr;

    hipStream_t stream = nullptr;
    bool own_stream = false;
    mir_lsq_workspace* ws = nullptr;
    bool own_ws = false;
    Buffers<T> B;
    JtjPlan plan;
    LmSettingsDev<T> sd;
    uint32_t variant = 0;
    bool dbg_solve = false, no_speculation = false, lowrank = true, no_null_skip = false, host_profile = false;
    mir_lsq_stats stats_local{};
    mir_lsq_stats* stats_user = nullptr;
    size_t stats_bytes = 0;
    uint64_t launches_mark = 0;
    int round_kind = -1;
    uint64_t launches_excluded = 0;
    std::atomic<uint64_t> worker_launches{0};
    int lr_cap = kLrMax;
    int lr_k = 0;
    int device = 0, caller_device = -1;
    T* y = nullptr;
    T* mB = nullptr;
    T* fr = nullptr;
    bool has_bounds = true;
    bool tail_null = false;
    bool fused = false;
    bool spec_enqueue = false;
    size_t spec_events_from = 0;
    bool big_solve = false;
    bool coop_disabled = false;

    LmState<T>* st_h;
    LmState<T>* st_slot[2] = {nullptr, nullptr};
    LmState<T>* st_slot_d[2] = {nullptr, nullptr};
    T* x_slot[2] = {nullptr, nullptr};
    T* x_slot_d[2] = {nullptr, nullptr};
    T* x_h = nullptr;
    uint32_t seq = 0;
    T* trial_h;
    std::vector<T> twh_h;
    std::vector<EventPair> events;
    Result ret;

    struct Slot { T* p = nullptr; T* yp = nullptr; T* ym = nullptr; };
    std::vector<Slot> slots;
    std::vector<int> slot_count;
    std::mutex fd_mutex;
    std::atomic<bool> fd_failed{false};
    bool fd_panel_mode = false;
    std::atomic<uint32_t> fd_streams_used{0};
    std::atomic<uint64_t> fd_f_ns{0};
    std::atomic<uint32_t> fd_tasks_run{0};

    double hp_ms[6] = {0, 0, 0, 0, 0, 0};
    struct HpScope {
        Solver* s; int cat; std::chrono::steady_clock::time_point t0;
        HpScope(Solver* s_, int c) : s(s_), cat(c) { if (s->host_profile) t0 = std::chrono::steady_clock::now(); }
        ~HpScope() {
            if (!s->host_profile) return;
            const double ms = std::chrono::duration<double, std::milli>(std::chrono::steady_clock::now() - t0).count();
            s->hp_ms[cat] += ms;
            if (ms > s->hp_ms[5]) s->hp_ms[5] = ms;
        }
    };

    bool ok(hipError_t e, const char* what)
    {
        if (e == hipSuccess) return true;
        std::fprintf(stderr, "[mir_optim_amd] %s failed: %s\n", what, hipGetErrorName(e));
        return false;
    }
    uint64_t launches_now() const { return tl_launches + worker_launches.load(std::memory_order_relaxed); }
    void close_round()
    {
        const uint64_t now = launches_now();
        if (stats) {
            stats->library_launches += now - launches_mark;
            if (round_kind >= 0) { stats->round_launches[round_kind] += now - launches_mark - launches_excluded; stats->rounds[round_kind]++; }
        }
        launches_mark = now;
        launches_excluded = 0;
        round_kind = -1;
    }
    void ev_begin(int kind);
    void ev_end();

    bool setup();
    void teardown();
    bool eval_f(const T* x_dev, const T* x_host, T* y_dev);
    int sumsq_blocks() const;
    bool sumsq(const T* v, int slot);
    bool trial_sums(const T* v, int count, size_t vstride);
    bool allreduce(T* buf, size_t count, int kind);
    void trace_emit(int event, uint32_t iterations, T lambda, T residual, T trial_residual, T dx_dot);
    bool trace_round(int ks, T residual_before, uint32_t iterations_before);
    bool wait_state(uint32_t expect);
    bool read_state(const T* vec_dev);
    void print_solve_dbg(bool fused_round);
    LmSolveArgs<T> solve_args(int ks, const T* lam, bool check_grad, bool lambda_from_state);
    bool enqueue_solve(int ks, const T* lam, bool check_grad, bool lambda_from_state);
    DecideArgs<T> decide_args(int ks, bool check_grad, bool lambda_from_state);
    bool enqueue_decide(int ks, bool check_grad, bool lambda_from_state, const T* sum_v = nullptr);
    bool enqueue_fused_tail(const T* ytr, bool check_grad, bool lambda_from_state);
    void commit_spec_round();
    void drop_spec_round();
    Result run();

    bool broyden_lowrank(const T* y_dev, const T* yold_dev);
    bool plain_products(const T* y_vec);
    bool unpack_in_reduce(JtjOp op) const { return !comm && jtj_unpacks(plan, op); }
    JtjUnpack<T> unpack_target() { JtjUnpack<T> u; u.JJ = B.JJ; u.Jy = B.Jy; return u; }
    bool finish_products(bool direct);
    bool jacobian_products(bool broyden, const T* y_dev, const T* yold_dev);
    bool fd_device();
    static void fd_task_trampoline(mir_least_squares_task task, uint32_t totalThreads, uint32_t threadId, uint32_t j);
    void fd_task(uint32_t totalThreads, uint32_t threadId, uint32_t j);
    bool fd_host_prepare_panel();
    bool fd_host();
    bool analytic_jacobian();
};

template <typename T>
typename Abi<T>::Result solve_entry(const typename Abi<T>::Settings* settings, size_t m, size_t n, T* x, const T* l,
                                    const T* u, const mir_lsq_gpu_options* opt, void* fctx, typename Abi<T>::F f,
                                    void* gctx, typename Abi<T>::G g, void* tmctx, mir_least_squares_thread_manager tm);

}
```

mir_optim_amd/csrc/launch_broyden.hip:

```cpp
#include <hip/hip_runtime.h>

#include "broyden_launch.h"
#include "launch_util.h"
#include "broyden_lr.h"

namespace mirlsq {

namespace {
template <typename T, int NCP>
hipError_t lr_sweep_ncp(const LrArgs<T>& a, int nblk, bool vec, hipStream_t s)
{
    if (vec) MIRLSQ_LAUNCH((k_broyden_lr<T, NCP, true>), dim3(nblk), dim3(256), 0, s, a);
    else MIRLSQ_LAUNCH((k_broyden_lr<T, NCP, false>), dim3(nblk), dim3(256), 0, s, a);
    return hipGetLastError();
}
}
template <typename T>
hipError_t lr_sweep(const LrArgs<T>& a, int nblk, hipStream_t s)
{
    if (a.n > kLrMaxN || a.k < 0 || a.k >= kLrMax) return hipErrorInvalidValue;
    const bool vec = (a.n % 2 == 0) && (reinterpret_cast<uintptr_t>(a.J) % (2 * sizeof(T)) == 0);
    const int ncp = (a.n + 31) / 32;
    if (ncp <= 1) return lr_sweep_ncp<T, 1>(a, nblk, vec, s);
    if (ncp <= 2) return lr_sweep_ncp<T, 2>(a, nblk, vec, s);
    if (ncp <= 4) return lr_sweep_ncp<T, 4>(a, nblk, vec, s);
    if (ncp <= 8) return lr_sweep_ncp<T, 8>(a, nblk, vec, s);
    return lr_sweep_ncp<T, 16>(a, nblk, vec, s);
}

namespace {
template <typename T, int NCP>
hipError_t lr_flush_ncp(T* J, const T* U, const T* D, int k, size_t m, int n, int nblk, bool vec, hipStream_t s)
{
    const size_t lds = (size_t)k * n * sizeof(T);
    if (vec) MIRLSQ_LAUNCH((k_lr_flush<T, NCP, true>), dim3(nblk), dim3(256), lds, s, J, U, D, k, m, n);
    else MIRLSQ_LAUNCH((k_lr_flush<T, NCP, false>), dim3(nblk), dim3(256), lds, s, J, U, D, k, m, n);
    return hipGetLastError();
}
}
template <typename T>
hipError_t lr_flush(T* J, const T* U, const T* D, int k, size_t m, int n, int num_cu, hipStream_t s)
{
    if (k <= 0) return hipSuccess;
    if (n > kLrMaxN || k > kLrMax) return hipErrorInvalidValue;
    const size_t G = (m + 3) / 4;
    size_t blocks = (G + 3) / 4;
    if (blocks > (size_t)num_cu * 8) blocks = (size_t)num_cu * 8;
    if (blocks < 1) blocks = 1;
    const bool vec = (n % 2 == 0) && (reinterpret_cast<uintptr_t>(J) % (2 * sizeof(T)) == 0);
    const int ncp = (n + 31) / 32;
    if (ncp <= 1) return lr_flush_ncp<T, 1>(J, U, D, k, m, n, (int)blocks, vec, s);
    if (ncp <= 2) return lr_flush_ncp<T, 2>(J, U, D, k, m, n, (int)blocks, vec, s);
    if (ncp <= 4) return lr_flush_ncp<T, 4>(J, U, D, k, m, n, (int)blocks, vec, s);
    if (ncp <= 8) return lr_flush_ncp<T, 8>(J, U, D, k, m, n, (int)blocks, vec, s);
    return lr_flush_ncp<T, 16>(J, U, D, k, m, n, (int)blocks, vec, s);
}

template <typename T>
hipError_t lr_reduce(const T* partials, int nblk, int n, T* out, hipStream_t s)
{
    const int len = lr_len(n);
    MIRLSQ_LAUNCH(k_lr_reduce<T>, dim3((len + 31) / 32), dim3(32 * kReduceRanges), 0, s, partials, nblk, len, out);
    return hipGetLastError();
}

template <typename T>
hipError_t lr_finish(const T* lr, T* D, const T* dx, int k, int n, T* JJ, T* Jy, LmState<T>* st, hipStream_t s)
{
    MIRLSQ_LAUNCH(k_lr_finish<T>, dim3(n + 1), dim3(256), 0, s, lr, D, dx, k, n, JJ, Jy, st);
    return hipGetLastError();
}

template <typename T>
hipError_t lr_sumsq(const T* v, size_t m, int count, size_t vstride, T* partials, int pstride, int nblk, hipStream_t s)
{
    if (count < 1 || nblk < 1 || nblk > pstride) return hipErrorInvalidValue;
    MIRLSQ_LAUNCH(k_lr_sumsq<T>, dim3(nblk, count), dim3(256), 0, s, v, m, vstride, partials, pstride);
    return hipGetLastError();
}
template <typename T>
hipError_t lr_sumsq_final(const T* partials, int pstride, int nblk, int count, T* out, hipStream_t s)
{
    MIRLSQ_LAUNCH(k_lr_sumsq_final<T>, dim3(count), dim3(256), 0, s, partials, pstride, nblk, out);
    return hipGetLastError();
}

#define MIRLSQ_INSTANTIATE(T)                                                                                             \
    template hipError_t lr_sweep<T>(const LrArgs<T>&, int, hipStream_t);                                                  \
    template hipError_t lr_reduce<T>(const T*, int, int, T*, hipStream_t);                                                \
    template hipError_t lr_finish<T>(const T*, T*, const T*, int, int, T*, T*, LmState<T>*, hipStream_t);                 \
    template hipError_t lr_sumsq<T>(const T*, size_t, int, size_t, T*, int, int, hipStream_t);                            \
    template hipError_t lr_sumsq_final<T>(const T*, int, int, int, T*, hipStream_t);                                      \
    template hipError_t lr_flush<T>(T*, const T*, const T*, int, size_t, int, int, hipStream_t);
MIRLSQ_INSTANTIATE(double)
MIRLSQ_INSTANTIATE(float)
#undef MIRLSQ_INSTANTIATE

}

MIRLSQ_DEFINE_PRELOAD(broyden)
```

mir_optim_amd/csrc/misc_kernels.h:

```cpp
#pragma once

#include "broyden_lr.h"
#include "common.h"
#include "solve_types.h"

namespace mirlsq {

template <typename T>
__global__ __launch_bounds__(256) void k_sumsq_partial(const T* __restrict__ v0, size_t m, T* __restrict__ partials0,
                                                       size_t vstride = 0, int pstride = 0)
{
    __shared__ T red[4];
    const T* __restrict__ v = v0 + (size_t)blockIdx.y * vstride;
    T* __restrict__ partials = partials0 + (size_t)blockIdx.y * pstride;
    T s = 0;
    const size_t stride = (size_t)gridDim.x * blockDim.x;
    const size_t per = (m + gridDim.x - 1) / gridDim.x;
    const size_t b0 = (size_t)blockIdx.x * per;
    const size_t b1 = b0 + per < m ? b0 + per : m;
    (void)stride;
    for (size_t i = b0 + threadIdx.x; i < b1; i += blockDim.x) { const T t = v[i]; s += t * t; }
    s = wave_sum(s);
    if ((threadIdx.x & 63) == 0) red[threadIdx.x >> 6] = s;
    __syncthreads();
    if (threadIdx.x == 0) partials[blockIdx.x] = (red[0] + red[1]) + (red[2] + red[3]);
}

template <typename T>
__device__ inline T sumsq_final_block(const T* partials, int nparts, T* red )
{
    T s = 0;
    for (int i = threadIdx.x; i < nparts; i += 256) s += partials[i];
    s = wave_sum(s);
    if ((threadIdx.x & 63) == 0) red[threadIdx.x >> 6] = s;
    __syncthreads();
    const T tot = (red[0] + red[1]) + (red[2] + red[3]);
    __syncthreads();
    return tot;
}
template <typename T>
__global__ __launch_bounds__(256) void k_sumsq_final(const T* __restrict__ partials0, int nparts, T* __restrict__ out, int pstride = 0)
{
    __shared__ T red[4];
    const T tot = sumsq_final_block(partials0 + (size_t)blockIdx.x * pstride, nparts, red);
    if (threadIdx.x == 0) out[blockIdx.x] = tot;
}

template <typename T>
__device__ inline void publish_state(const LmState<T>& s, LmState<T>* host_st, uint32_t seq)
{
    if (!host_st) return;
    LmState<T> t = s;
    t.seq = 0;
    *host_st = t;
    __threadfence_system();
    *reinterpret_cast<volatile uint32_t*>(&host_st->seq) = seq;
    __threadfence_system();
}

template <typename T>
__global__ void k_init_state(const T* sum, LmState<T>* st, LmState<T>* host_st, uint32_t seq)
{
    LmState<T> s{};
    s.lambda = 0;
    s.mu = 1;
    s.residual = *sum;
    *st = s;
    publish_state(s, host_st, seq);
}

template <typename T>
__global__ __launch_bounds__(256) void k_unpack_grad(const T* __restrict__ packed, int n, T* __restrict__ JJ,
                                                     T* __restrict__ Jy, LmState<T>* st)
{
    __shared__ T red[4];
    const int i = blockIdx.x;
    if (i < n) {
        for (int j = threadIdx.x; j < n; j += blockDim.x) {
            const int r = i >= j ? i : j, c = i >= j ? j : i;
            JJ[(size_t)i * n + j] = packed[(size_t)r * (r + 1) / 2 + c];
        }
        return;
    }
    T mx = 0;
    for (int j = threadIdx.x; j < n; j += blockDim.x) {
        const T v = packed[(size_t)n * (n + 1) / 2 + j];
        Jy[j] = v;
        const T av = dabs(v);
        if (av > mx) mx = av;
    }
    mx = wave_max(mx);
    if ((threadIdx.x & 63) == 0) red[threadIdx.x >> 6] = mx;
    __syncthreads();
    if (threadIdx.x == 0) {
        T r = red[0];
        for (int w = 1; w < (int)(blockDim.x >> 6); ++w) r = red[w] > r ? red[w] : r;
        st->jy_inf = r;
    }
}

template <typename T>
__global__ void k_fd_points(const T* __restrict__ x, const T* __restrict__ lower, const T* __restrict__ upper,
                            T eps, int n, T* __restrict__ X, T* __restrict__ twh)
{
    const int j = blockIdx.x;
    const T save = x[j];
    T xmh = save - eps, xph = save + eps;
    xmh = dfmax(xmh, lower[j]);
    xph = dfmin(xph, upper[j]);
    for (int k = threadIdx.x; k < n; k += blockDim.x) {
        const T xv = x[k];
        X[(size_t)(2 * j) * n + k] = k == j ? xph : xv;
        X[(size_t)(2 * j + 1) * n + k] = k == j ? xmh : xv;
    }
    if (threadIdx.x == 0) twh[j] = xph - xmh;
}

template <typename T>
__global__ __launch_bounds__(256) void k_fd_fill(const T* __restrict__ Y, size_t ldy, const T* __restrict__ twh,
                                                 T* __restrict__ J, size_t m, int n, int j0, int pc)
{
    __shared__ T tile[32][65];
    const size_t i0 = (size_t)blockIdx.x * 64;
    const int c0 = blockIdx.y * 32;
    const int lane = threadIdx.x & 63, cw = threadIdx.x >> 6;
    for (int c = cw; c < 32; c += 4) {
        const int cc = c0 + c;
        T v = 0;
        if (cc < pc && i0 + lane < m) {
            const T t = twh[j0 + cc];
            if (t != 0) {
                const T a = Y[(size_t)(2 * cc) * ldy + i0 + lane];
                const T b = Y[(size_t)(2 * cc + 1) * ldy + i0 + lane];
                T d = a;
                d += T(-1) * b;
                v = d * (T(1) / t);
            }
        }
        tile[c][lane] = v;
    }
    __syncthreads();
    const int ncol = (pc - c0) < 32 ? (pc - c0) : 32;
    for (int idx = threadIdx.x; idx < 64 * 32; idx += 256) {
        const int r = idx >> 5, c = idx & 31;
        if (c < ncol && i0 + r < m) J[(i0 + r) * (size_t)n + j0 + c0 + c] = tile[c][r];
    }
}

template <typename T>
__global__ __launch_bounds__(256) void k_fd_fill_col(const T* __restrict__ yp, const T* __restrict__ ym, T twh,
                                                     T* __restrict__ J, size_t m, int n, int j)
{
    const size_t i = (size_t)blockIdx.x * blockDim.x + threadIdx.x;
    if (i >= m) return;
    T v = 0;
    if (twh != 0) { T d = yp[i]; d += T(-1) * ym[i]; v = d * (T(1) / twh); }
    J[i * (size_t)n + j] = v;
}

template <typename T> struct DecidePre { T xv, dv; };

template <typename T>
__device__ inline int decide_chain_body(const DecideArgs<T>& a, const DecidePre<T>* pre = nullptr, long long* dbg = nullptr)
{
    __shared__ int acc_s;
    __shared__ LmState<T> s_pub;
    if (a.nparts > 0) {
        __shared__ T part[kReduceRanges];
        for (int k = 0; k < a.ks; ++k) {
            const T tot = lr_reduce_scalar(a.partials + (size_t)k * a.pstride, a.nparts, part);
            if (threadIdx.x == 0) a.sums[k] = tot;
        }
    }
    if (threadIdx.x == 0) {
        LmState<T> s = *a.st;
        if (dbg) { asm volatile("s_waitcnt vmcnt(0)" ::: "memory"); dbg[29] = wall_clock64(); }
        int dec = kDecideReject, acc = -1;
        uint32_t consumed = 0, fcalls = 0, rejects = 0, guards = 0, qpact = 0, null_tail = 0;
        for (int k = 0; k < a.ks; ++k) {
            const ChainRec<T> r = a.rec[k];
            if (k == 0 && a.check_grad && (r.flags & kFlagGradSmall)) { dec = kDecideGradSmall; break; }
            ++consumed;
            if (k == 0 && a.lambda_from_state) s.lambda = r.lambda;
            if (r.qp_iterations > 0) ++qpact;
            s.qp_status = r.qp_status; s.qp_iterations = r.qp_iterations; s.flags = r.flags;
            if (r.qp_status != 0 || (r.flags & kFlagDxNaN)) { dec = kDecideNumericError; break; }
            if (r.flags & kFlagStepTooLong) {
                LM_REJECT(s.lambda, s.mu, a.set);
                ++guards;
                continue;
            }
            ++fcalls;
            const bool null_step = (r.flags & kFlagNullStep) != 0;
            if (null_step) a.sums[k] = s.residual;
            null_tail = null_step ? 1u : 0u;
            const T tr = a.sums[k];
            s.trial_residual = tr;
            if (!(tr <= Lim<T>::inf())) { dec = kDecideNumericError; s.flags |= kFlagTrialNotFinite; break; }
            const T improvement = s.residual - tr;
            s.improvement = improvement;
            if (!(improvement > 0)) {
                LM_REJECT(s.lambda, s.mu, a.set);
                ++rejects;
                continue;
            }
            s.mu = 1;
            s.iterations++;
            s.residual = tr;
            s.dx_dot = r.new_dx_dot;
            s.new_dx_dot = r.new_dx_dot;
            s.predicted = r.predicted;
            s.trial_xnorm = r.trial_xnorm;
            acc = k;
            if (!(r.predicted > 0)) { dec = kDecideAcceptNoPrediction; break; }
            const T rho = r.predicted / improvement;
            s.rho = rho;
            LM_RATE_STEP(rho, s.lambda, s.mu, a.set);
            dec = kDecideAccept;
            break;
        }
        int spec = 0;
        if (a.spec_static && dec == kDecideAccept && acc == 0) {
            spec = LM_PASS_MAY_START(s.residual, s.lambda, s.iterations, a.maxIterations, a.set)
                && LM_LAMBDA_SET(s.lambda, a.set) && lr_spec_go(a.rec[0], a.set.absTolerance, a.set.relTolerance);
        }
        s.spec_ok = spec;
        uint32_t rescued = 0;
        for (int k = 0; k < a.ks; ++k) if (a.rec[k].flags & kFlagCoopRescued) ++rescued;
        s.coop_rescued = rescued;
        s.decision = dec; s.accepted_k = acc; s.consumed = consumed; s.fcalls = fcalls;
        s.rejects = rejects; s.guards = guards; s.qp_active = qpact;
        s.null_tail = (dec == kDecideReject) ? null_tail : 0u;
        *a.st = s;
        s_pub = s;
        acc_s = acc;
        if (a.host_st) { LmState<T> t = s; t.seq = 0; *a.host_st = t; }
    }
    lds_barrier();
    const int acc = acc_s;
    if (acc >= 0) {
        if (pre) {
            if ((int)threadIdx.x < a.n) {
                a.x[threadIdx.x] = pre->xv;
                if (a.host_x) a.host_x[threadIdx.x] = pre->xv;
                a.dx_acc[threadIdx.x] = pre->dv;
            }
        } else {
            for (int i = threadIdx.x; i < a.n; i += blockDim.x) {
                const T xv = a.trial[(size_t)acc * a.n + i];
                a.x[i] = xv;
                if (a.host_x) a.host_x[i] = xv;
                a.dx_acc[i] = a.dx_chain[(size_t)acc * a.n + i];
            }
        }
    }
    if (dbg && threadIdx.x == 0) dbg[30] = wall_clock64();
    if (a.host_st) {
        __threadfence_system();
        __syncthreads();
        if (threadIdx.x == 0) *reinterpret_cast<volatile uint32_t*>(&a.host_st->seq) = a.seq;
    }
    if (dbg && threadIdx.x == 0) dbg[31] = wall_clock64();
    const int spec = s_pub.spec_ok;
    __syncthreads();
    return spec;
}

template <typename T>
__global__ __launch_bounds__(kSolveThreads) void k_decide_chain(DecideArgs<T> a)
{
    (void)decide_chain_body(a);
}

template <typename T>
__global__ void k_reset_mu(LmState<T>* st) { st->mu = 1; }

}
```

mir_optim_amd/csrc/solver_jacobian.hip:

```cpp
#include "driver.h"
#include "launch_util.h"
#include "misc_kernels.h"

namespace mirlsq {

template <typename T>
bool Solver<T>::broyden_lowrank(const T* y_dev, const T* yold_dev)
{
    T* U = static_cast<T*>(ws->ulr);
    if (lr_k >= lr_cap) {
        const uint64_t launches_before = launches_now();
        struct Excl { Solver* s; uint64_t l0; ~Excl() { s->launches_excluded += s->launches_now() - l0; } } excl{this, launches_before};
        if (!ok(lr_flush<T>(B.J, U, B.lrD, lr_k, m, (int)n, ws->num_cu, stream), "broyden flush")) return false;
        lr_k = 0;
        if (stats) stats->broyden_flushes++;
        if (!plain_products(yold_dev)) return false;
        if (stats) stats->jtj_resyncs++;
    }
    LrArgs<T> a{};
    a.J = B.J; a.U = U; a.D = B.lrD; a.dx = B.dx_acc; a.dx_dot = &B.st->dx_dot; a.y = y_dev; a.y_old = yold_dev;
    a.partials = B.lrpart; a.m = m; a.n = (int)n; a.k = lr_k;
    const int nblk = lr_blocks(m, ws->num_cu), len = lr_len((int)n);
    ev_begin(1);
    if (!ok(lr_sweep<T>(a, nblk, stream), "broyden sweep")) return false;
    ev_end();
    if (!ok(lr_reduce<T>(B.lrpart, nblk, (int)n, B.lrvec, stream), "broyden reduce")) return false;
    if (comm && !allreduce(B.lrvec, (size_t)len, 1)) return false;
    if (!ok(lr_finish<T>(B.lrvec, B.lrD, B.dx_acc, lr_k, (int)n, B.JJ, B.Jy, B.st, stream), "broyden finish")) return false;
    if (stats) stats->broyden_lr_columns += (uint64_t)lr_k;
    ++lr_k;
    return true;
}

template <typename T>
bool Solver<T>::plain_products(const T* y_vec)
{
    JtjArgs<T> a{};
    a.J = B.J; a.Jout = B.J; a.y = y_vec; a.y_old = y_vec; a.dx = B.dx_acc; a.dx_dot = &B.st->dx_dot;
    a.slabs = B.slabs; a.m = m; a.n = (int)n;
    const bool direct = unpack_in_reduce(JtjOp::plain);
    ev_begin(0);
    if (!ok(jtj_run<T>(plan, JtjOp::plain, a, B.packed, stream, direct ? unpack_target() : JtjUnpack<T>{}), "jtj kernel")) return false;
    ev_end();
    return finish_products(direct);
}

template <typename T>
bool Solver<T>::finish_products(bool direct)
{
    if (direct) return ok(hipGetLastError(), "jtj reduce");
    if (comm && !allreduce(B.packed, (size_t)n * (n + 1) / 2 + n, 0)) return false;
    return ok(jtj_unpack<T>(B.packed, (int)n, B.JJ, B.Jy, B.st, stream), "unpack");
}

template <typename T>
bool Solver<T>::jacobian_products(bool broyden, const T* y_dev, const T* yold_dev)
{
    if (broyden && lowrank) return broyden_lowrank(y_dev, yold_dev);
    if (!broyden) lr_k = 0;
    JtjArgs<T> a{};
    a.J = B.J; a.Jout = B.J; a.y = y_dev; a.y_old = yold_dev; a.dx = B.dx_acc; a.dx_dot = &B.st->dx_dot;
    a.slabs = B.slabs; a.m = m; a.n = (int)n;
    if (!broyden && fd_fused) {
        const JtjOp op = fd_fused == 2 ? JtjOp::fd_diff : JtjOp::fd;
        fd_fused = 0;
        a.J = static_cast<const T*>(ws->ypanel); a.twh = B.twh;
        const bool direct = unpack_in_reduce(op);
        ev_begin(3);
        if (!ok(jtj_run<T>(plan, op, a, B.packed, stream, direct ? unpack_target() : JtjUnpack<T>{}), "fd + jtj kernel")) return false;
        ev_end();
        return finish_products(direct);
    }
    const JtjOp op = broyden ? JtjOp::rewrite : JtjOp::plain;
    const bool direct = unpack_in_reduce(op);
    ev_begin(broyden ? 1 : 0);
    if (!ok(jtj_run<T>(plan, op, a, B.packed, stream, direct ? unpack_target() : JtjUnpack<T>{}), "jtj kernel")) return false;
    ev_end();
    return finish_products(direct);
}

template <typename T>
bool Solver<T>::fd_device()
{
    MIRLSQ_LAUNCH(k_fd_points<T>, dim3(n), dim3(64), 0, stream, B.x, B.lower, B.upper, sd.jacobianEpsilon, (int)n, B.X, B.twh);
    for (uint32_t j = 0; j < n; ++j) {
        const T save = xh[j];
        T xmh = save - S->jacobianEpsilon, xph = save + S->jacobianEpsilon;
        xmh = std::fmax(xmh, lh[j]);
        xph = std::fmin(xph, uh[j]);
        twh_h[j] = xph - xmh;
    }
    size_t pb = n;
    size_t cap = (size_t)64 << 30;
    if (ws->ypanel_bytes < 2 * pb * m * sizeof(T)) {
        size_t free_b = 0, total_b = 0;
        if (hipMemGetInfo(&free_b, &total_b) == hipSuccess) {
            const size_t have = ws->ypanel_bytes + free_b;
            if (have / 2 < cap) cap = have / 2;
        }
        if (cap < ((size_t)1 << 30)) cap = (size_t)1 << 30;
    }
    if (2 * pb * m * sizeof(T) > cap) {
        pb = cap / (2 * m * sizeof(T));
        if (pb >= 64) pb -= pb % 64;
    }
    if (pb < 1) pb = 1;
    if (fb && fd_batch && fd_batch / 2 < pb) pb = fd_batch / 2 ? fd_batch / 2 : 1;
    const bool no_fuse = (variant & MIR_LSQ_VARIANT_FD_SEPARATE_FILL) != 0;
    const bool use_diff = fbd && plan.fd_diff.kernel != JtjKernel::none && pb == n && !no_fuse;
    const size_t need = (use_diff ? 1 : 2) * pb * m * sizeof(T);
    if (ws->ypanel_bytes < need) {
        if (ws->ypanel) (void)hipFree(ws->ypanel);
        ws->ypanel = nullptr; ws->ypanel_bytes = 0;
        if (!ok(hipMalloc(&ws->ypanel, need), "hipMalloc(FD panel)")) return false;
        ws->ypanel_bytes = need;
    }
    T* Y = static_cast<T*>(ws->ypanel);
    if (use_diff) {
        ev_begin(4);
        fbd(fbctx, m, n, 2 * (size_t)n, B.X, Y);
        ev_end();
        if (stats) { stats->fd_callback_points += 2 * (uint64_t)n; stats->fd_callback_calls++; }
        fd_fused = 2;
        ret.fCalls += n;
        return ok(hipGetLastError(), "fd batched callback");
    }
    if (fbr && plan.fd.kernel != JtjKernel::none && pb == n && !no_fuse) {
        ev_begin(4);
        fbr(fbctx, m, n, 2 * (size_t)n, B.X, Y);
        ev_end();
        if (stats) { stats->fd_callback_points += 2 * (uint64_t)n; stats->fd_callback_calls++; }
        fd_fused = 1;
        ret.fCalls += n;
        return ok(hipGetLastError(), "fd batched callback");
    }
    for (size_t j0 = 0; j0 < n; j0 += pb) {
        const size_t pc = (j0 + pb <= n) ? pb : n - j0;
        ev_begin(4);
        if (fb) {
            fb(fbctx, m, n, 2 * pc, B.X + 2 * j0 * n, Y);
            if (stats) stats->fd_callback_points += 2 * (uint64_t)pc;
        } else {
            for (size_t c = 0; c < pc; ++c) {
                if (twh_h[j0 + c] == 0) continue;
                f(fctx, m, n, B.X + (2 * (j0 + c)) * n, Y + (2 * c) * m);
                f(fctx, m, n, B.X + (2 * (j0 + c) + 1) * n, Y + (2 * c + 1) * m);
                if (stats) stats->fd_callback_points += 2;
            }
        }
        ev_end();
        if (stats) stats->fd_callback_calls++;
        dim3 grid((unsigned)((m + 63) / 64), (unsigned)((pc + 31) / 32));
        MIRLSQ_LAUNCH(k_fd_fill<T>, grid, dim3(256), 0, stream, Y, m, B.twh, B.J, m, (int)n, (int)j0, (int)pc);
    }
    ret.fCalls += n;
    return ok(hipGetLastError(), "fd fill");
}

template <typename T>
void Solver<T>::fd_task_trampoline(mir_least_squares_task task, uint32_t totalThreads, uint32_t threadId, uint32_t j)
{
    static_cast<Solver<T>*>(task.context)->fd_task(totalThreads, threadId, j);
}
template <typename T>
void Solver<T>::fd_task(uint32_t totalThreads, uint32_t threadId, uint32_t j)
{
    const uint32_t idx = totalThreads >= n ? j : threadId;
    if (idx >= n || j >= n) { fd_failed = true; return; }
    ++fd_tasks_run;
    if (hipSetDevice(device) != hipSuccess) { fd_failed = true; return; }
    Slot* s;
    {
        std::lock_guard<std::mutex> lk(fd_mutex);
        s = &slots[idx];
        if (!s->p) {
            s->p = static_cast<T*>(std::malloc(n * sizeof(T)));
            if (!s->p) { fd_failed = true; return; }
        }
        if (!fd_panel_mode && !s->yp) {
            if (hipHostMalloc((void**)&s->yp, m * sizeof(T), hipHostMallocDefault) != hipSuccess
                || hipHostMalloc((void**)&s->ym, m * sizeof(T), hipHostMallocDefault) != hipSuccess) {
                fd_failed = true;
                return;
            }
        }
        if (slot_count[idx]++ == 0) std::memcpy(s->p, xh, n * sizeof(T));
    }
    T* p = s->p;
    const T save = p[j];
    T xmh = save - S->jacobianEpsilon, xph = save + S->jacobianEpsilon;
    xmh = std::fmax(xmh, lh[j]);
    xph = std::fmin(xph, uh[j]);
    const T twh = xph - xmh;
    if (fd_panel_mode) {
        if (twh != 0) {
            T* hp = static_cast<T*>(ws->pinned_panel) + (size_t)(2 * j) * m;
            const auto t0 = std::chrono::steady_clock::now();
            p[j] = xph;
            f(fctx, m, n, p, hp);
            p[j] = xmh;
            f(fctx, m, n, p, hp + m);
            p[j] = save;
            fd_f_ns += (uint64_t)std::chrono::duration_cast<std::chrono::nanoseconds>(std::chrono::steady_clock::now() - t0).count();
            const int k = (int)(idx % mir_lsq_workspace::kCopyStreams);
            fd_streams_used |= 1u << k;
            if (hipMemcpyAsync(static_cast<T*>(ws->ypanel) + (size_t)(2 * j) * m, hp, 2 * m * sizeof(T), hipMemcpyHostToDevice,
                               ws->copy_stream[k]) != hipSuccess)
                fd_failed = true;
        }
        return;
    }
    if (twh != 0) {
        p[j] = xph;
        f(fctx, m, n, p, s->yp);
        p[j] = xmh;
        f(fctx, m, n, p, s->ym);
        p[j] = save;
    }
    std::lock_guard<std::mutex> lk(fd_mutex);
    if (twh != 0) {
        if (hipMemcpyAsync(mB, s->yp, m * sizeof(T), hipMemcpyHostToDevice, stream) != hipSuccess
            || hipMemcpyAsync(fr, s->ym, m * sizeof(T), hipMemcpyHostToDevice, stream) != hipSuccess) {
            fd_failed = true;
            return;
        }
    }
    hipLaunchKernelGGL(k_fd_fill_col<T>, dim3((unsigned)((m + 255) / 256)), dim3(256), 0, stream, mB, fr, twh, B.J, m, (int)n, (int)j);
    worker_launches.fetch_add(1, std::memory_order_relaxed);
    if (hipStreamSynchronize(stream) != hipSuccess) fd_failed = true;
}
template <typename T>
bool Solver<T>::fd_host_prepare_panel()
{
    if (variant & MIR_LSQ_VARIANT_FD_HOST_COLUMNS) return false;
    const size_t need = 2 * (size_t)n * m * sizeof(T);
    if (need > ((size_t)16 << 30)) return false;
    if (ws->ypanel_bytes < need) {
        size_t free_b = 0, total_b = 0;
        if (hipMemGetInfo(&free_b, &total_b) != hipSuccess) return false;
        size_t cap = (ws->ypanel_bytes + free_b) / 2;
        if (cap > ((size_t)64 << 30)) cap = (size_t)64 << 30;
        if (need > cap) return false;
        if (ws->ypanel) (void)hipFree(ws->ypanel);
        ws->ypanel = nullptr; ws->ypanel_bytes = 0;
        if (hipMalloc(&ws->ypanel, need) != hipSuccess) return false;
        ws->ypanel_bytes = need;
    }
    if (ws->pinned_panel_bytes < need) {
        if (ws->pinned_panel) (void)hipHostFree(ws->pinned_panel);
        ws->pinned_panel = nullptr; ws->pinned_panel_bytes = 0;
        if (hipHostMalloc(&ws->pinned_panel, need, hipHostMallocDefault) != hipSuccess) return false;
        ws->pinned_panel_bytes = need;
    }
    for (int k = 0; k < mir_lsq_workspace::kCopyStreams; ++k) {
        if (!ws->copy_stream[k] && hipStreamCreateWithFlags(&ws->copy_stream[k], hipStreamNonBlocking) != hipSuccess) return false;
        if (!ws->copy_event[k] && hipEventCreateWithFlags(&ws->copy_event[k], hipEventDisableTiming) != hipSuccess) return false;
    }
    return true;
}
template <typename T>
bool Solver<T>::fd_host()
{
    slots.resize(n);
    slot_count.assign(n, 0);
    fd_panel_mode = fd_host_prepare_panel();
    fd_streams_used = 0;
    fd_tasks_run = 0;
    if (fd_panel_mode) {
        MIRLSQ_LAUNCH(k_fd_points<T>, dim3(n), dim3(64), 0, stream, B.x, B.lower, B.upper, sd.jacobianEpsilon, (int)n, B.X, B.twh);
    }
    mir_least_squares_task task{this, nullptr};
    const auto t0 = std::chrono::steady_clock::now();
    if (tm) tm(tmctx, n, task, &fd_task_trampoline);
    else for (uint32_t j = 0; j < n; ++j) fd_task(1, 0, j);
    uint32_t calls = 0;
    for (uint32_t k = 0; k < n; ++k) calls += (uint32_t)slot_count[k];
    ret.fCalls += calls;
    if (stats) {
        stats->fd_host_wall_ms += std::chrono::duration<double, std::milli>(std::chrono::steady_clock::now() - t0).count();
        stats->fd_host_f_ms += (double)fd_f_ns.exchange(0) * 1e-6;
        stats->fd_host_columns += n;
    }
    const bool incomplete = fd_tasks_run.load() != n;
    if (incomplete)
        std::fprintf(stderr, "[mir_optim_amd] thread manager ran %u of %u finite-difference tasks\n", fd_tasks_run.load(), n);
    if (incomplete || fd_failed) {
        if (fd_panel_mode)
            for (int k = 0; k < mir_lsq_workspace::kCopyStreams; ++k)
                if (fd_streams_used.load() & (1u << k)) (void)hipStreamSynchronize(ws->copy_stream[k]);
        return false;
    }
    if (fd_panel_mode) {
        const uint32_t used = fd_streams_used.load();
        for (int k = 0; k < mir_lsq_workspace::kCopyStreams; ++k) {
            if (!(used & (1u << k))) continue;
            if (!ok(hipEventRecord(ws->copy_event[k], ws->copy_stream[k]), "copy event")
                || !ok(hipStreamWaitEvent(stream, ws->copy_event[k], 0), "wait for the panel copies")) return false;
        }
        dim3 grid((unsigned)((m + 63) / 64), (unsigned)((n + 31) / 32));
        MIRLSQ_LAUNCH(k_fd_fill<T>, grid, dim3(256), 0, stream, static_cast<const T*>(ws->ypanel), m, B.twh, B.J, m, (int)n, 0, (int)n);
        return ok(hipGetLastError(), "fd fill");
    }
    return true;
}

template <typename T>
bool Solver<T>::analytic_jacobian()
{
    if (device_cb) {
        g(gctx, m, n, B.x, B.J);
    } else {
        if (!ws->pinned_J && !ok(hipHostMalloc(&ws->pinned_J, m * n * sizeof(T), hipHostMallocDefault), "hipHostMalloc(J)")) return false;
        T* Jh = static_cast<T*>(ws->pinned_J);
        g(gctx, m, n, xh, Jh);
        if (!ok(hipMemcpyAsync(B.J, Jh, m * n * sizeof(T), hipMemcpyHostToDevice, stream), "H2D J")
            || !ok(hipStreamSynchronize(stream), "sync")) return false;
    }
    ret.gCalls += 1;
    return true;
}

#define MIRLSQ_INSTANTIATE(T)                                                                       \
    template bool Solver<T>::broyden_lowrank(const T*, const T*);                                   \
    template bool Solver<T>::plain_products(const T*);                                              \
    template bool Solver<T>::finish_products(bool);                                                 \
    template bool Solver<T>::jacobian_products(bool, const T*, const T*);                           \
    template bool Solver<T>::fd_device();                                                           \
    template void Solver<T>::fd_task_trampoline(mir_least_squares_task, uint32_t, uint32_t, uint32_t); \
    template void Solver<T>::fd_task(uint32_t, uint32_t, uint32_t);                                 \
    template bool Solver<T>::fd_host_prepare_panel();                                               \
    template bool Solver<T>::fd_host();                                                             \
    template bool Solver<T>::analytic_jacobian();
MIRLSQ_INSTANTIATE(double)
MIRLSQ_INSTANTIATE(float)
#undef MIRLSQ_INSTANTIATE

}

MIRLSQ_DEFINE_PRELOAD(jacobian)
```

mir_optim_amd/csrc/solver_loop.hip:

```cpp
#include "driver.h"
#include "launch_util.h"
#include "misc_kernels.h"

namespace mirlsq {

template <typename T>
void Solver<T>::ev_begin(int kind)
{
    if (!time_kernels) return;
    HpScope hp(this, 0);
    EventPair p{};
    p.kind = spec_enqueue ? kind + 100 : kind;
    if (ws->event_pool.size() < 2 * (events.size() + 1)) {
        hipEvent_t ea, eb;
        (void)hipEventCreate(&ea);
        (void)hipEventCreate(&eb);
        ws->event_pool.push_back(ea);
        ws->event_pool.push_back(eb);
    }
    p.a = ws->event_pool[2 * events.size()];
    p.b = ws->event_pool[2 * events.size() + 1];
    (void)hipEventRecord(p.a, stream);
    events.push_back(p);
}
template <typename T>
void Solver<T>::ev_end()
{
    if (!time_kernels) return;
    HpScope hp(this, 0);
    (void)hipEventRecord(events.back().b, stream);
}

template <typename T>
bool Solver<T>::setup()
{
    if (!ws) {
        ws = workspace_create<T>(m, n);
        own_ws = true;
        if (!ws) return false;
    } else if (ws->m != m || ws->n != n || ws->elem != sizeof(T)) {
        std::fprintf(stderr, "[mir_optim_amd] workspace shape mismatch\n");
        ws = nullptr;
        return false;
    }
    if (hipGetDevice(&caller_device) != hipSuccess) caller_device = ws->device;
    if (caller_device != ws->device && !ok(hipSetDevice(ws->device), "hipSetDevice")) return false;
    plan = jtj_plan<T>(m, (int)n, ws->num_cu);
    B = carve<T>(ws->dev, m, n, ws->num_cu);
    device = ws->device;
    for (int k = 0; k < 2; ++k) {
        st_slot[k] = reinterpret_cast<LmState<T>*>(ws->pinned) + k;
        st_slot_d[k] = reinterpret_cast<LmState<T>*>(ws->pinned_dev) + k;
        x_slot[k] = reinterpret_cast<T*>(static_cast<char*>(ws->pinned) + 2 * sizeof(LmState<T>)) + (size_t)k * n;
        x_slot_d[k] = reinterpret_cast<T*>(static_cast<char*>(ws->pinned_dev) + 2 * sizeof(LmState<T>)) + (size_t)k * n;
        st_slot[k]->seq = 0;
    }
    st_h = st_slot[0];
    trial_h = reinterpret_cast<T*>(static_cast<char*>(ws->pinned) + 2 * sizeof(LmState<T>)) + 2 * (size_t)n;
    if (!stream) {
        if (!ok(hipStreamCreate(&stream), "hipStreamCreate")) return false;
        own_stream = true;
    }
    sd = lm_settings_dev(S);
    dbg_solve = (variant & MIR_LSQ_VARIANT_DEBUG_SOLVE) != 0;
    no_speculation = (variant & MIR_LSQ_VARIANT_NO_SPECULATION) != 0;
    lowrank = (variant & MIR_LSQ_VARIANT_BROYDEN_REWRITE) == 0;
    no_null_skip = (variant & MIR_LSQ_VARIANT_NO_NULL_SKIP) != 0;
    host_profile = (variant & MIR_LSQ_VARIANT_HOST_PROFILE) != 0;
    {
        const int v = (int)((variant >> MIR_LSQ_VARIANT_LR_CAP_SHIFT) & 31u);
        if (v >= 1 && v <= kLrMax) lr_cap = v;
    }
    y = B.y;
    mB = B.mB;
    fr = B.ytmp;
    big_solve = n > (uint32_t)kSolveMaxN || (variant & MIR_LSQ_VARIANT_SOLVE_GENERIC) != 0;
    if (n > (uint32_t)kLrMaxN) lowrank = false;
    fused = device_cb && lowrank && !big_solve && !trace && !(variant & MIR_LSQ_VARIANT_NO_PIPELINE);
    twh_h.resize(n);
    char* stage = static_cast<char*>(ws->pinned) + align_up(2 * sizeof(LmState<T>) + (3 * (size_t)n + 8) * sizeof(T), 256);
    const size_t ol = (size_t)(reinterpret_cast<char*>(B.lower) - reinterpret_cast<char*>(B.x));
    const size_t ou = (size_t)(reinterpret_cast<char*>(B.upper) - reinterpret_cast<char*>(B.x));
    std::memcpy(stage, xh, n * sizeof(T));
    std::memcpy(stage + ol, lh, n * sizeof(T));
    std::memcpy(stage + ou, uh, n * sizeof(T));
    return ok(hipMemcpyAsync(B.x, stage, ou + n * sizeof(T), hipMemcpyHostToDevice, stream), "H2D x, l, u");
}

template <typename T>
void Solver<T>::teardown()
{
    if (stream) (void)hipStreamSynchronize(stream);
    if (host_profile) std::fprintf(stderr, "[host profile] J %p  FD panel %p  y %p\n", (void*)B.J, ws ? ws->ypanel : nullptr, (void*)B.y);
    if (host_profile)
        std::fprintf(stderr, "[host profile] events %.3f ms  all-reduce calls %.3f  trial callbacks %.3f  readback+sync %.3f  solve launch %.3f  "
                             "longest single call %.3f\n", hp_ms[0], hp_ms[1], hp_ms[2], hp_ms[3], hp_ms[4], hp_ms[5]);
    if (stats) {
        for (auto& e : events) {
            if (e.kind < 0 || e.kind >= 100) continue;
            float ms = 0;
            (void)hipEventElapsedTime(&ms, e.a, e.b);
            if (e.kind == 0) { stats->jtj_ms += ms; stats->jtj_launches++; }
            else if (e.kind == 1) { stats->jtj_ms += ms; stats->jtj_launches++; stats->jtj_broyden_ms += ms; stats->jtj_broyden_launches++; }
            else if (e.kind == 2) { stats->solve_ms += ms; stats->solve_launches++; }
            else if (e.kind == 3) { stats->jtj_ms += ms; stats->jtj_launches++; stats->jtj_fd_ms += ms; stats->jtj_fd_launches++; }
            else if (e.kind == 4) stats->fd_callback_ms += ms;
            else if (e.kind == 5) stats->trial_callback_ms += ms;
        }
    }
    events.clear();
    for (auto& s : slots) {
        if (s.p) std::free(s.p);
        if (s.yp) (void)hipHostFree(s.yp);
        if (s.ym) (void)hipHostFree(s.ym);
    }
    slots.clear();
    if (own_stream && stream) (void)hipStreamDestroy(stream);
    if (ws && caller_device >= 0 && caller_device != ws->device) (void)hipSetDevice(caller_device);
    if (own_ws && ws) workspace_destroy(ws);
}

template <typename T>
bool Solver<T>::eval_f(const T* x_dev, const T* x_host, T* y_dev)
{
    if (device_cb) {
        f(fctx, m, n, x_dev, y_dev);
        return true;
    }
    if (!ws->pinned_y && !ok(hipHostMalloc(&ws->pinned_y, m * sizeof(T), hipHostMallocDefault), "hipHostMalloc(y)")) return false;
    T* yh = static_cast<T*>(ws->pinned_y);
    const auto t0 = std::chrono::steady_clock::now();
    f(fctx, m, n, x_host, yh);
    if (stats) { stats->host_f_ms += std::chrono::duration<double, std::milli>(std::chrono::steady_clock::now() - t0).count(); stats->host_f_calls++; }
    return ok(hipMemcpyAsync(y_dev, yh, m * sizeof(T), hipMemcpyHostToDevice, stream), "H2D y")
        && ok(hipStreamSynchronize(stream), "sync");
}

template <typename T>
int Solver<T>::sumsq_blocks() const
{
    int nb = (int)((m + 4095) / 4096);
    if (nb > kPartials) nb = kPartials;
    return nb < 1 ? 1 : nb;
}
template <typename T>
bool Solver<T>::sumsq(const T* v, int slot)
{
    const int nb = sumsq_blocks();
    MIRLSQ_LAUNCH(k_sumsq_partial<T>, dim3(nb), dim3(256), 0, stream, v, m, B.partials, (size_t)0, kPartials);
    MIRLSQ_LAUNCH(k_sumsq_final<T>, dim3(1), dim3(256), 0, stream, B.partials, nb, B.sum + slot, kPartials);
    if (comm && !allreduce(B.sum + slot, 1, 2)) return false;
    return ok(hipGetLastError(), "sumsq");
}

template <typename T>
bool Solver<T>::trial_sums(const T* v, int count, size_t vstride)
{
    static_assert(kPartials >= kLrMaxBlocks, "one partial per workgroup of the sweep's grid");
    const int nb = lr_blocks(m, ws->num_cu);
    if (!ok(lr_sumsq<T>(v, m, count, vstride, B.partials, kPartials, nb, stream), "trial sums")) return false;
    if (!comm) { sums_pending = nb; return true; }
    if (!ok(lr_sumsq_final<T>(B.partials, kPartials, nb, count, B.sum + 1, stream), "trial sums, stage 2")) return false;
    return allreduce(B.sum + 1, (size_t)count, 2);
}

template <typename T>
bool Solver<T>::allreduce(T* buf, size_t count, int kind)
{
    HpScope hp(this, 1);
    if (stats && !spec_enqueue) { stats->allreduce_calls[kind]++; stats->allreduce_elems[kind] += count; }
    return comm_allreduce<T>(comm, buf, count, stream) == 0;
}

template <typename T>
void Solver<T>::trace_emit(int event, uint32_t iterations, T lambda, T residual, T trial_residual, T dx_dot)
{
    if (!trace) return;
    if (trace->count < trace->capacity && trace->records) {
        mir_lsq_trace_record& r = trace->records[trace->count];
        r.event = event; r.iterations = iterations; r.lambda = (double)lambda; r.residual = (double)residual;
        r.trial_residual = (double)trial_residual; r.dx_dot = (double)dx_dot;
    }
    trace->count++;
}
template <typename T>
bool Solver<T>::trace_round(int ks, T residual_before, uint32_t iterations_before)
{
    ChainRec<T> rec[kChainMax];
    T sums[kChainMax];
    if (!ok(hipMemcpyAsync(rec, B.rec, (size_t)ks * sizeof(ChainRec<T>), hipMemcpyDeviceToHost, stream), "D2H rec")
        || !ok(hipMemcpyAsync(sums, B.sum + 1, (size_t)ks * sizeof(T), hipMemcpyDeviceToHost, stream), "D2H sums")
        || !ok(hipStreamSynchronize(stream), "sync"))
        return false;
    const int dec = st_h->decision;
    if (dec == kDecideGradSmall || dec == kDecideNumericError) return true;
    for (uint32_t k = 0; k < st_h->consumed && k < (uint32_t)ks; ++k) {
        if (rec[k].flags & kFlagStepTooLong)
            trace_emit(4, iterations_before, rec[k].lambda, residual_before, 0, rec[k].new_dx_dot);
        else if ((int)k != st_h->accepted_k)
            trace_emit(2, iterations_before, rec[k].lambda, residual_before, sums[k], rec[k].new_dx_dot);
        else
            trace_emit(3, iterations_before + 1, rec[k].lambda, sums[k], sums[k], rec[k].new_dx_dot);
    }
    return true;
}

template <typename T>
bool Solver<T>::wait_state(uint32_t expect)
{
    HpScope hp(this, 3);
    st_h = st_slot[expect & 1];
    x_h = x_slot[expect & 1];
    volatile uint32_t* sq = &st_h->seq;
    constexpr double kWaitBoundSeconds = 600.0;
    std::chrono::steady_clock::time_point t_wait{};
    for (uint64_t spins = 0;; ++spins) {
        if (*sq == expect) break;
        if ((spins & 0xfff) == 0xfff) {
            const hipError_t q = hipStreamQuery(stream);
            if (q == hipSuccess) {
                if (*sq == expect) break;
                std::fprintf(stderr, "[mir_optim_amd] decision point %u was not published\n", expect);
                return false;
            }
            if (q != hipErrorNotReady) return ok(q, "stream query");
            const auto now = std::chrono::steady_clock::now();
            if (t_wait == std::chrono::steady_clock::time_point{}) t_wait = now;
            else if (std::chrono::duration<double>(now - t_wait).count() > kWaitBoundSeconds) {
                std::fprintf(stderr, "[mir_optim_amd] decision point %u: no progress for %.0f s, giving up\n", expect, kWaitBoundSeconds);
                return false;
            }
        }
        if (spins < 20000) cpu_relax(); else std::this_thread::yield();
    }
    std::atomic_thread_fence(std::memory_order_acquire);
    return true;
}

template <typename T>
bool Solver<T>::read_state(const T* vec_dev)
{
    HpScope hp(this, 3);
    if (!ok(hipMemcpyAsync(st_h, B.st, sizeof(LmState<T>), hipMemcpyDeviceToHost, stream), "D2H state")) return false;
    if (vec_dev && !ok(hipMemcpyAsync(trial_h, vec_dev, n * sizeof(T), hipMemcpyDeviceToHost, stream), "D2H vec")) return false;
    return ok(hipStreamSynchronize(stream), "sync");
}

template <typename T>
void Solver<T>::print_solve_dbg(bool fused_round)
{
    long long h[32];
    if (hipMemcpy(h, B.sc[0].dbg, sizeof h, hipMemcpyDeviceToHost) != hipSuccess) return;
    if (fused_round)
        std::fprintf(stderr, "[solve dbg] fused round head (10ns ticks): decision + publication %lld (loads landed %lld, decided + point copied %lld, fence + sequence number %lld)  n x n side of the Broyden pass %lld\n", h[27] - h[26], h[29] - h[26], h[30] - h[29], h[31] - h[30], h[28] - h[27]);
    std::fprintf(stderr, "[solve dbg] (10ns ticks) build %lld  copy/equil %lld  scale %lld  potrf %lld  potrs %lld  refine %lld  epilogue %lld  total %lld  shader MHz %.0f  [matvec1 %lld berr %lld]\n",
                 h[1] - h[0], h[2] - h[1], h[3] - h[2], h[4] - h[3], h[5] - h[4], h[6] - h[5], h[8] - h[7], h[8] - h[0], (double)(h[10] - h[9]) / (double)(h[8] - h[0]) * 100.0, h[11] - h[5], h[12] - h[11]);
    if (n <= 128)
        std::fprintf(stderr, "[solve dbg] load (10ns ticks): kernel entry -> loads landed %lld (of which inside posvx %lld)  reduction + LDS commit %lld  rest of the phase %lld\n",
                     h[24] - h[0], h[24] - h[2], h[25] - h[24], h[3] - h[25]);
    if (n <= 128)
        std::fprintf(stderr, "[solve dbg] refinement (10ns ticks): residual 1 %lld  berr 1 %lld  potrs 2 %lld  residual 2 %lld  rest %lld  (correction applied: %lld)\n",
                     h[11] - h[5], h[12] - h[11], h[13] - h[12], h[14] - h[13], h[6] - h[14], h[15]);
    if (n <= 128)
        std::fprintf(stderr, "[solve dbg] lds_potrf, wave 0 (shader cycles, summed over the panels): diagonal update + factor %lld  wait %lld  rows below %lld  wait %lld\n", h[20], h[21], h[22], h[23]);
    if (n > 128)
        std::fprintf(stderr, "[solve dbg] potrf_panel steps (10ns ticks, summed over the panels): earlier panels on MFMA %lld (of which publishing / waiting for the helpers' look-ahead jobs %lld)  diagonal rows %lld  other rows + store %lld\n", h[16], h[19], h[17], h[18]);
}

template <typename T>
LmSolveArgs<T> Solver<T>::solve_args(int ks, const T* lam, bool check_grad, bool lambda_from_state)
{
    LmSolveArgs<T> a{};
    a.JJ = B.JJ; a.Jy = B.Jy; a.x = B.x; a.lower = B.lower; a.upper = B.upper;
    a.dx = B.dx; a.trial = B.trial; a.st = B.st; a.rec = B.rec; a.set = sd; a.n = (int)n;
    for (int k = 0; k < kChainMax; ++k) { a.sc[k] = B.sc[k]; a.lam[k] = (lam && k < ks) ? lam[k] : T(0); }
    a.f_in_lds = solve_nb((int)n, (int)sizeof(T)) > 0;
    a.check_grad = check_grad ? 1 : 0;
    a.lambda_from_state = lambda_from_state ? 1 : 0;
    if (!dbg_solve) a.sc[0].dbg = nullptr;
    a.coop_w = (big_solve && n > (uint32_t)kSolveMaxN && !(variant & MIR_LSQ_VARIANT_SOLVE_ONE_WORKGROUP) && !coop_disabled) ? coop_peers((int)n) : 1;
    if (a.coop_w > ws->num_cu / 2) a.coop_w = ws->num_cu / 2 >= 2 ? ws->num_cu / 2 : 1;
    a.coop_epoch = a.coop_w > 1 ? ++ws->solve_epoch : 0;
    a.coop_absent = (variant & MIR_LSQ_VARIANT_DEBUG_HELPERS_ABSENT) ? 1 : 0;
    return a;
}
template <typename T>
bool Solver<T>::enqueue_solve(int ks, const T* lam, bool check_grad, bool lambda_from_state)
{
    const LmSolveArgs<T> a = solve_args(ks, lam, check_grad, lambda_from_state);
    ev_begin(2);
    {
        HpScope hp(this, 4);
        if (!ok(launch_lm_solve<T>(a, ks, has_bounds, big_solve, stream), "solve launch")) return false;
    }
    ev_end();
    return true;
}

template <typename T>
DecideArgs<T> Solver<T>::decide_args(int ks, bool check_grad, bool lambda_from_state)
{
    DecideArgs<T> d{};
    d.sums = B.sum + 1; d.rec = B.rec; d.st = B.st; d.set = sd; d.x = B.x; d.trial = B.trial; d.dx_chain = B.dx;
    d.dx_acc = B.dx_acc; d.n = (int)n; d.ks = ks; d.check_grad = check_grad ? 1 : 0;
    d.lambda_from_state = lambda_from_state ? 1 : 0;
    ++seq;
    d.host_st = st_slot_d[seq & 1]; d.host_x = x_slot_d[seq & 1]; d.seq = seq;
    d.maxIterations = S->maxIterations;
    d.partials = B.partials; d.nparts = sums_pending; d.pstride = kPartials;
    sums_pending = 0;
    return d;
}
template <typename T>
bool Solver<T>::enqueue_decide(int ks, bool check_grad, bool lambda_from_state, const T* sum_v)
{
    if (sum_v && !trial_sums(sum_v, ks, m)) return false;
    const DecideArgs<T> d = decide_args(ks, check_grad, lambda_from_state);
    MIRLSQ_LAUNCH(k_decide_chain<T>, dim3(1), dim3(kSolveThreads), 0, stream, d);
    return ok(hipGetLastError(), "decide kernel");
}

template <typename T>
bool Solver<T>::enqueue_fused_tail(const T* ytr, bool check_grad, bool lambda_from_state)
{
    spec_events_from = events.size();
    if (stats) stats->fused_rounds++;
    LrArgs<T> a{};
    a.J = B.J; a.U = static_cast<T*>(ws->ulr); a.D = B.lrD; a.dx = B.dx; a.dx_dot = &B.rec[0].new_dx_dot; a.y = ytr; a.y_old = y;
    a.partials = B.lrpart; a.m = m; a.n = (int)n; a.k = lr_k;
    a.spec_rec = B.rec; a.absTolerance = sd.absTolerance; a.relTolerance = sd.relTolerance;
    const int nblk = lr_blocks(m, ws->num_cu), len = lr_len((int)n);
    spec_enqueue = true;
    ev_begin(1);
    const bool swept = ok(lr_sweep<T>(a, nblk, stream), "broyden sweep");
    ev_end();
    spec_enqueue = false;
    if (!swept || !ok(lr_reduce<T>(B.lrpart, nblk, (int)n, B.lrvec, stream), "broyden reduce")) return false;
    if (comm && !allreduce(B.lrvec, (size_t)len, 1)) return false;
    LmSolveArgs<T> sa = solve_args(1, nullptr, true, false);
    sa.lambda_from_device = 1;
    sa.fused = 1;
    sa.dec = decide_args(1, check_grad, lambda_from_state);
    sa.dec.sums = B.lrvec + lr_yy((int)n);
    sa.dec.spec_static = 1;
    sa.fin_lr = B.lrvec; sa.fin_D = B.lrD; sa.fin_JJ = B.JJ; sa.fin_Jy = B.Jy; sa.fin_k = lr_k;
    spec_enqueue = true;
    ev_begin(2);
    bool good;
    {
        HpScope hp(this, 4);
        good = ok(launch_lm_solve<T>(sa, 1, has_bounds, false, stream), "fused round launch");
    }
    ev_end();
    spec_enqueue = false;
    return good;
}
template <typename T>
void Solver<T>::commit_spec_round()
{
    for (size_t i = spec_events_from; i < events.size(); ++i) if (events[i].kind >= 100) events[i].kind -= 100;
    if (stats) {
        stats->jacobian_broyden++;
        stats->fused_passes++;
        stats->broyden_lr_columns += (uint64_t)lr_k;
    }
    ++lr_k;
}
template <typename T>
void Solver<T>::drop_spec_round()
{
    for (size_t i = spec_events_from; i < events.size(); ++i) if (events[i].kind >= 100) events[i].kind = -1;
}

template <typename T>
typename Solver<T>::Result Solver<T>::run()
{
    ret.status = mir_ls_numericError; ret.iterations = 0; ret.fCalls = 0; ret.gCalls = 0;
    ret.residual = Lim<T>::inf(); ret.lambda = 0;
    const auto t_start = std::chrono::steady_clock::now();
    launches_mark = launches_now();

    {
        bool finite = true;
        for (uint32_t i = 0; i < n; ++i) if (!(-Lim<T>::inf() < xh[i] && xh[i] < Lim<T>::inf())) finite = false;
        if (m == 0 || n == 0 || !finite) { ret.status = mir_ls_badGuess; return ret; }
        for (uint32_t i = 0; i < n; ++i) if (!(lh[i] <= xh[i]) || !(xh[i] <= uh[i])) { ret.status = mir_ls_badBounds; return ret; }
        if (const int bad = bad_settings(S)) { ret.status = bad; return ret; }
    }
    if (!device_available()) return ret;
    if (!setup()) { teardown(); return ret; }
    has_bounds = (variant & MIR_LSQ_VARIANT_SOLVE_BOUNDED) != 0;
    for (uint32_t i = 0; i < n; ++i)
        if (lh[i] > -Lim<T>::inf() || uh[i] < Lim<T>::inf()) has_bounds = true;

    const uint32_t maxAge = S->maxAge ? S->maxAge : (g ? 3 : 2 * n);

    bool fail = false;
    do {
        if (!eval_f(B.x, xh, y)) { fail = true; break; }
        ++ret.fCalls;
        ++seq;
        if (!sumsq(y, 0)) { fail = true; break; }
        MIRLSQ_LAUNCH(k_init_state<T>, dim3(1), dim3(1), 0, stream, B.sum, B.st, st_slot_d[seq & 1], seq);
        if (!ok(hipGetLastError(), "init state") || !wait_state(seq)) { fail = true; break; }
    } while (false);
    if (fail) { teardown(); ret.status = mir_ls_numericError; return ret; }

    ret.residual = st_h->residual;
    bool fConverged = LM_F_CONVERGED(ret.residual, sd);
    bool needJacobian = true;
    bool last_rejected = false;
    bool spec_live = false;
    bool spec_predict = true;
    const bool speculate = device_cb && !no_speculation;
    uint32_t age = maxAge;
    ret.lambda = 0;
    T mu = 1;
    ret.status = mir_ls_maxIterations;

    do {
        close_round();
        if (stats) stats->passes++;
        if (fConverged) { ret.status = mir_ls_fConverged; break; }
        if (!LM_LAMBDA_IN_RANGE(ret.lambda, sd)) { ret.status = mir_ls_furtherImprovement; break; }
        if (mu > kSuspiciousMu && age) {
            needJacobian = true;
            age = maxAge;
            mu = 1;
            MIRLSQ_LAUNCH(k_reset_mu<T>, dim3(1), dim3(1), 0, stream, B.st);
        }
        {
            bool nan = false;
            for (uint32_t i = 0; i < n; ++i) if (!(xh[i] <= xh[i])) nan = true;
            if (nan) { ret.status = mir_ls_numericError; break; }
        }
        bool newJacobian = false;
        int ks = 1;
        bool lambda_from_state = false, skip_eval = false;
        T* ytr = fr;
        bool solve_enqueued = false;
        if (spec_live) {
            spec_live = false;
            if (!needJacobian || !(age < maxAge) || lr_k >= lr_cap) {
                std::fprintf(stderr, "[mir_optim_amd] internal error: the pass run ahead by the fused round is not the next pass\n");
                fail = true;
                break;
            }
            needJacobian = false;
            newJacobian = true;
            last_rejected = false;
            age++;
            commit_spec_round();
            solve_enqueued = true;
        }
        round_kind = solve_enqueued ? 1 : 2;
        if (needJacobian) {
            needJacobian = false;
            newJacobian = true;
            last_rejected = false;
            round_kind = age < maxAge ? 1 : 0;
            if (age < maxAge) {
                age++;
                if (stats) stats->jacobian_broyden++;
                if (!jacobian_products(true, y, mB)) { fail = true; break; }
                trace_emit(1, ret.iterations, ret.lambda, ret.residual, 0, st_h->dx_dot);
            } else {
                age = 0;
                if (stats) stats->jacobian_full++;
                const auto t0 = std::chrono::steady_clock::now();
                bool okj;
                if (g) okj = analytic_jacobian();
                else okj = device_cb ? fd_device() : fd_host();
                if (!okj) { fail = true; break; }
                if (stats && !device_cb)
                    stats->fd_ms += std::chrono::duration<double, std::milli>(std::chrono::steady_clock::now() - t0).count();
                if (!jacobian_products(false, y, mB)) { fail = true; break; }
                trace_emit(0, ret.iterations, ret.lambda, ret.residual, 0, st_h->dx_dot);
            }
        }

        lambda_from_state = !solve_enqueued && !LM_LAMBDA_SET(ret.lambda, sd);
        T lam[kChainMax];
        lam[0] = ret.lambda;
        if (speculate && !newJacobian && !lambda_from_state && last_rejected) {
            T l2 = ret.lambda, m2 = mu;
            while (ks < kChainMax) {
                LM_REJECT(l2, m2, sd);
                if (!LM_LAMBDA_IN_RANGE(l2, sd)) break;
                if (m2 > kSuspiciousMu && age) break;
                lam[ks++] = l2;
            }
        }
        if (!solve_enqueued && !enqueue_solve(ks, lam, newJacobian, lambda_from_state)) { fail = true; break; }
        if (dbg_solve && !solve_enqueued) print_solve_dbg(false);

        if (device_cb && tail_null && last_rejected && !newJacobian && !no_null_skip) {
            HpScope hp(this, 3);
            ChainRec<T> rr[kChainMax];
            if (!ok(hipMemcpyAsync(rr, B.rec, (size_t)ks * sizeof(ChainRec<T>), hipMemcpyDeviceToHost, stream), "D2H rec")
                || !ok(hipStreamSynchronize(stream), "sync")) { fail = true; break; }
            skip_eval = true;
            for (int k = 0; k < ks; ++k) if (!(rr[k].flags & kFlagNullStep)) skip_eval = false;
            if (skip_eval && stats) stats->elided_evaluations += (uint64_t)ks;
        }

        if (ks > 1) ytr = static_cast<T*>(ws->ytrial);
        if (skip_eval) {
        } else if (device_cb) {
            HpScope hp(this, 2);
            ev_begin(5);
            if (ks > 1 && fb) fb(fbctx, m, n, (size_t)ks, B.trial, ytr);
            else for (int k = 0; k < ks; ++k) f(fctx, m, n, B.trial + (size_t)k * n, ytr + (size_t)k * m);
            ev_end();
            if (stats) { stats->trial_callback_points += (uint64_t)ks; stats->trial_callback_calls++; }
        } else {
            ChainRec<T> r0;
            if (!ok(hipMemcpyAsync(&r0, B.rec, sizeof r0, hipMemcpyDeviceToHost, stream), "D2H rec") || !read_state(B.trial)) { fail = true; break; }
            const bool null_step = (r0.flags & kFlagNullStep) && !no_null_skip;
            if (null_step && stats) stats->elided_evaluations++;
            const bool no_f = (newJacobian && (r0.flags & kFlagGradSmall)) || r0.qp_status != 0
                || (r0.flags & (kFlagDxNaN | kFlagStepTooLong)) || null_step;
            if (!no_f && !eval_f(B.trial, trial_h, ytr)) { fail = true; break; }
        }

        const bool fuse = fused && spec_predict && ks == 1 && !skip_eval && age < maxAge && lr_k < lr_cap;
        if (fuse ? !enqueue_fused_tail(ytr, newJacobian, lambda_from_state)
                 : !enqueue_decide(ks, newJacobian, lambda_from_state, skip_eval ? nullptr : ytr)) { fail = true; break; }
        const uint32_t round_seq = seq;
        if (!wait_state(round_seq)) { fail = true; break; }
        if (fuse) {
            if (st_h->spec_ok) spec_live = true; else drop_spec_round();
            if (dbg_solve && spec_live) print_solve_dbg(true);
        }
        if (ks == 1 && newJacobian) spec_predict = st_h->decision == kDecideAccept;

        if (trace && !trace_round(ks, ret.residual, ret.iterations)) { fail = true; break; }
        if (st_h->coop_rescued) {
            if (stats) stats->coop_timeouts += st_h->coop_rescued;
            coop_disabled = true;
        }
        const int dec = st_h->decision;
        tail_null = st_h->null_tail != 0;
        ret.fCalls += st_h->fcalls;
        if (stats) {
            if (st_h->consumed > 1) stats->passes += st_h->consumed - 1;
            stats->rejected += st_h->rejects;
            stats->step_guard_rejects += st_h->guards;
            stats->qp_active_set_passes += st_h->qp_active;
        }
        if (dec == kDecideGradSmall) {
            if (age == 0) { ret.status = mir_ls_gConverged; break; }
            age = maxAge;
            continue;
        }
        ret.lambda = st_h->lambda;
        mu = st_h->mu;
        if (dec == kDecideNumericError) { ret.status = mir_ls_numericError; break; }
        if (dec == kDecideReject) { last_rejected = true; continue; }
        last_rejected = false;

        needJacobian = true;
        ret.iterations = st_h->iterations;
        for (uint32_t i = 0; i < n; ++i) xh[i] = x_h[i];
        if (ytr != fr) {
            if (!ok(hipMemcpyAsync(fr, ytr + (size_t)st_h->accepted_k * m, m * sizeof(T), hipMemcpyDeviceToDevice, stream), "D2D y")) { fail = true; break; }
        }
        { T* t = mB; mB = y; y = fr; fr = t; }
        ret.residual = st_h->residual;
        fConverged = LM_F_CONVERGED(ret.residual, sd);
        if (stats) stats->accepted++;

        if (dec == kDecideAcceptNoPrediction) { ret.status = mir_ls_furtherImprovement; break; }

        const T dxn = std::sqrt(st_h->dx_dot);
        if (!LM_X_MOVING(dxn, st_h->trial_xnorm, sd)) {
            if (age == 0) { ret.status = mir_ls_xConverged; break; }
            age = maxAge;
            continue;
        }
    } while (ret.iterations < S->maxIterations);

    close_round();
    if (fail) ret.status = mir_ls_numericError;
    if (stats) stats->total_ms += std::chrono::duration<double, std::milli>(std::chrono::steady_clock::now() - t_start).count();
    teardown();
    return ret;
}

template <typename T>
typename Abi<T>::Result solve_entry(const typename Abi<T>::Settings* settings, size_t m, size_t n, T* x, const T* l,
                                    const T* u, const mir_lsq_gpu_options* opt, void* fctx, typename Abi<T>::F f,
                                    void* gctx, typename Abi<T>::G g, void* tmctx, mir_least_squares_thread_manager tm)
{
    Solver<T> s{};
    s.S = settings; s.m = m; s.n = (uint32_t)n; s.xh = x; s.lh = l; s.uh = u;
    s.fctx = fctx; s.f = f; s.gctx = gctx; s.g = g; s.tmctx = tmctx; s.tm = tm;
    if (opt) {
        s.device_cb = (opt->flags & MIR_LSQ_DEVICE_CALLBACKS) != 0;
        s.time_kernels = (opt->flags & MIR_LSQ_TIME_KERNELS) != 0 && opt->stats;
        s.stream = static_cast<hipStream_t>(opt->stream);
        s.comm = opt->comm;
        s.ws = opt->workspace;
        s.fbctx = opt->fbContext;
        s.fb = s.device_cb ? reinterpret_cast<typename Abi<T>::FB>(opt->fb) : nullptr;
        s.fd_batch = opt->fd_batch;
        s.variant = opt->variant;
        if (opt->stats) {
            size_t bytes = opt->struct_size >= offsetof(mir_lsq_gpu_options, fbRowMajorDiff) + sizeof(void*)
                ? offsetof(mir_lsq_stats, trial_callback_points) + sizeof(uint64_t)
                : (opt->struct_size >= offsetof(mir_lsq_gpu_options, fbRowMajor) + sizeof(void*)
                       ? offsetof(mir_lsq_stats, jtj_fd_launches) + sizeof(uint64_t)
                       : offsetof(mir_lsq_stats, qp_active_set_passes) + sizeof(uint64_t));
            if (opt->struct_size >= offsetof(mir_lsq_gpu_options, stats_size) + sizeof(uint32_t) && opt->stats_size)
                bytes = opt->stats_size;
            if (bytes > sizeof(mir_lsq_stats)) bytes = sizeof(mir_lsq_stats);
            s.stats_user = opt->stats;
            s.stats_bytes = bytes;
            std::memcpy(&s.stats_local, opt->stats, bytes);
            s.stats = &s.stats_local;
        }
        if (opt->struct_size >= offsetof(mir_lsq_gpu_options, trace) + sizeof(void*)) s.trace = opt->trace;
        if (opt->struct_size >= offsetof(mir_lsq_gpu_options, fbRowMajor) + sizeof(void*) && s.device_cb)
            s.fbr = reinterpret_cast<typename Abi<T>::FB>(opt->fbRowMajor);
        if (opt->struct_size >= offsetof(mir_lsq_gpu_options, fbRowMajorDiff) + sizeof(void*) && s.device_cb)
            s.fbd = reinterpret_cast<typename Abi<T>::FB>(opt->fbRowMajorDiff);
        if (s.trace) s.trace->count = 0;
    }
    const typename Abi<T>::Result r = s.run();
    if (s.stats_user) std::memcpy(s.stats_user, &s.stats_local, s.stats_bytes);
    return r;
}

#define MIRLSQ_INSTANTIATE(T)                                                                                                   \
    template struct Solver<T>;                                                                                                  \
    template Abi<T>::Result solve_entry<T>(const Abi<T>::Settings*, size_t, size_t, T*, const T*, const T*, const mir_lsq_gpu_options*, \
                                           void*, Abi<T>::F, void*, Abi<T>::G, void*, mir_least_squares_thread_manager);
MIRLSQ_INSTANTIATE(double)
MIRLSQ_INSTANTIATE(float)
#undef MIRLSQ_INSTANTIATE

}

MIRLSQ_DEFINE_PRELOAD(loop)
```

mir_optim_amd/csrc/unit_entries.hip:

```cpp
#include "driver.h"
#include "misc_kernels.h"

using namespace mirlsq;

namespace {
__global__ __launch_bounds__(256) void k_selftest_reductions(int rounds, uint32_t seed, int* out)
{
#pragma clang fp contract(off)
    uint32_t sr = seed ^ (0x9E3779B9u * (blockIdx.x * blockDim.x + threadIdx.x + 1));
    auto rnd = [&]() { sr ^= sr << 13; sr ^= sr >> 17; sr ^= sr << 5; return sr; };
    int bad[4] = {0, 0, 0, 0};
    for (int it = 0; it < rounds; ++it) {
        const float f = (float)(int32_t)rnd() * (1.0f / 65536.0f) * ((it & 7) == 0 ? 1e-20f : 1.0f);
        const double d = ((double)(int32_t)rnd() + (double)rnd() * 2.3283064365386963e-10) * ((it & 3) == 0 ? 1e-200 : 1.0);
        auto ref_sum = [](auto v) {
            v += __shfl_xor(v, 8, kWave); v += __shfl_xor(v, 4, kWave); v += __shfl_xor(v, 2, kWave); v += __shfl_xor(v, 1, kWave);
            v += __shfl_xor(v, 16, kWave); v += __shfl_xor(v, 32, kWave);
            return v;
        };
        auto ref_max = [](auto v) {
            for (int m : {8, 4, 2, 1, 16, 32}) { const auto o = __shfl_xor(v, m, kWave); v = o > v ? o : v; }
            return v;
        };
        const float sf = wave_sum(f), rf = ref_sum(f);
        const double sd = wave_sum(d), rdd = ref_sum(d);
        bad[0] += __float_as_uint(sf) != __float_as_uint(rf);
        bad[1] += __double_as_longlong(sd) != __double_as_longlong(rdd);
        bad[2] += __float_as_uint(wave_max(f)) != __float_as_uint(ref_max(f));
        bad[3] += __double_as_longlong(wave_max(d)) != __double_as_longlong(ref_max(d));
    }
    for (int k = 0; k < 4; ++k) if (bad[k]) atomicAdd(out + k, bad[k]);
}

template <typename T, typename QS>
int box_qp_entry(const QS* settings, size_t n_, const T* P, const T* q, const T* l, const T* u, T* x,
                 int unconstrainedSolution, int* iterations)
{
    if (iterations) *iterations = 0;
    if (n_ == 0) return mir_box_qp_solved;
    if (!device_available()) return mir_box_qp_numericError;
    const int n = (int)n_;
    size_t off = 0;
    auto take = [&](size_t bytes) { size_t o = off; off = align_up(off + bytes, 256); return o; };
    const size_t oP = take(sizeof(T) * n * n), oq = take(sizeof(T) * n), ol = take(sizeof(T) * n), ou = take(sizeof(T) * n),
                 ox = take(sizeof(T) * n), oPm = take(sizeof(T) * n * n), oA = take(sizeof(T) * n * n),
                 oF = take(sizeof(T) * n * (n | 1)), ov = take(sizeof(T) * 12 * n), oi = take(sizeof(int32_t) * 2 * n),
                 oo = take(sizeof(int) * 4);
    char* base = nullptr;
    if (hipMalloc((void**)&base, off) != hipSuccess) return mir_box_qp_numericError;
    BoxQpArgs<T> a{};
    a.P = (T*)(base + oP); a.q = (T*)(base + oq); a.l = (T*)(base + ol); a.u = (T*)(base + ou); a.x = (T*)(base + ox);
    a.sc.Pm = (T*)(base + oPm); a.sc.A = (T*)(base + oA); a.sc.Fg = (T*)(base + oF); a.sc.vec = (T*)(base + ov);
    a.sc.ivec = (int32_t*)(base + oi); a.out = (int*)(base + oo); a.sc.dbg = nullptr;
    a.relTol = settings->relTolerance; a.absTol = settings->absTolerance; a.maxIterations = settings->maxIterations;
    a.unconstrained = unconstrainedSolution; a.n = n;
    a.f_in_lds = solve_nb(n, (int)sizeof(T)) > 0;
    int out[2] = {mir_box_qp_numericError, 0};
    bool good = hipMemcpy((void*)a.P, P, sizeof(T) * n * n, hipMemcpyHostToDevice) == hipSuccess
        && hipMemcpy((void*)a.q, q, sizeof(T) * n, hipMemcpyHostToDevice) == hipSuccess
        && hipMemcpy((void*)a.l, l, sizeof(T) * n, hipMemcpyHostToDevice) == hipSuccess
        && hipMemcpy((void*)a.u, u, sizeof(T) * n, hipMemcpyHostToDevice) == hipSuccess
        && hipMemcpy((void*)a.x, x, sizeof(T) * n, hipMemcpyHostToDevice) == hipSuccess;
    if (good) good = launch_box_qp<T>(a, nullptr) == hipSuccess;
    if (good) {
        good = hipGetLastError() == hipSuccess && hipDeviceSynchronize() == hipSuccess
            && hipMemcpy(out, a.out, sizeof(out), hipMemcpyDeviceToHost) == hipSuccess
            && hipMemcpy(x, a.x, sizeof(T) * n, hipMemcpyDeviceToHost) == hipSuccess;
    }
    (void)hipFree(base);
    if (!good) return mir_box_qp_numericError;
    if (iterations) *iterations = out[1];
    return out[0];
}

template <typename T>
int jtj_entry(size_t m, size_t n, T* J, const T* y, const T* y_old, const T* dx, int broyden, T* JJ, T* Jy,
              void* stream_, float* kernel_ms)
{
    if (!device_available()) return -1;
    if (n == 0 || m == 0) return -2;
    hipStream_t stream = static_cast<hipStream_t>(stream_);
    const JtjPlan plan = jtj_plan<T>(m, (int)n, query_num_cu());
    const size_t packed_len = n * (n + 1) / 2 + n + 8;
    T *slabs = nullptr, *packed = nullptr, *dxdot = nullptr;
    LmState<T>* st = nullptr;
    const size_t slab_count = jtj_slab_elems(plan);
    if (hipMalloc((void**)&slabs, sizeof(T) * slab_count) != hipSuccess) return -3;
    if (hipMalloc((void**)&packed, sizeof(T) * packed_len) != hipSuccess) { (void)hipFree(slabs); return -3; }
    if (hipMalloc((void**)&st, sizeof(LmState<T>) + sizeof(T) * 8) != hipSuccess) { (void)hipFree(slabs); (void)hipFree(packed); return -3; }
    dxdot = reinterpret_cast<T*>(st + 1);
    int rc = 0;
    if (broyden) {
        hipLaunchKernelGGL(k_sumsq_partial<T>, dim3(1), dim3(256), 0, stream, dx, n, packed);
        hipLaunchKernelGGL(k_sumsq_final<T>, dim3(1), dim3(256), 0, stream, packed, 1, dxdot);
    }
    JtjArgs<T> a{};
    a.J = J; a.Jout = J; a.y = y; a.y_old = y_old; a.dx = dx; a.dx_dot = dxdot; a.slabs = slabs; a.m = m; a.n = (int)n;
    hipEvent_t e0, e1;
    (void)hipEventCreate(&e0); (void)hipEventCreate(&e1);
    (void)hipEventRecord(e0, stream);
    if (jtj_run<T>(plan, broyden ? JtjOp::rewrite : JtjOp::plain, a, packed, stream) != hipSuccess) rc = -4;
    (void)hipEventRecord(e1, stream);
    (void)jtj_unpack<T>(packed, (int)n, JJ, Jy, st, stream);
    if (hipStreamSynchronize(stream) != hipSuccess) rc = -5;
    if (kernel_ms) { float ms = 0; (void)hipEventElapsedTime(&ms, e0, e1); *kernel_ms = ms; }
    (void)hipEventDestroy(e0); (void)hipEventDestroy(e1);
    (void)hipFree(slabs); (void)hipFree(packed); (void)hipFree(st);
    return rc;
}
int fd_jtj_entry(size_t m, size_t n, const double* Yrm, const double* twh, const double* y, double* J,
                 double* JJ, double* Jy, void* stream_, float* kernel_ms, bool diff)
{
    if (!device_available()) return -1;
    if (n == 0 || m == 0) return -2;
    hipStream_t stream = static_cast<hipStream_t>(stream_);
    const JtjPlan plan = jtj_plan<double>(m, (int)n, query_num_cu());
    const JtjOp op = diff ? JtjOp::fd_diff : JtjOp::fd;
    if (plan.of(op).kernel == JtjKernel::none) return -6;
    const size_t packed_len = n * (n + 1) / 2 + n + 8;
    double *slabs = nullptr, *packed = nullptr;
    LmState<double>* st = nullptr;
    const size_t slab_count = jtj_slab_elems(plan);
    if (hipMalloc((void**)&slabs, sizeof(double) * slab_count) != hipSuccess) return -3;
    if (hipMalloc((void**)&packed, sizeof(double) * packed_len) != hipSuccess) { (void)hipFree(slabs); return -3; }
    if (hipMalloc((void**)&st, sizeof(LmState<double>)) != hipSuccess) { (void)hipFree(slabs); (void)hipFree(packed); return -3; }
    int rc = 0;
    JtjArgs<double> a{};
    a.J = Yrm; a.Jout = J; a.y = y; a.y_old = y; a.dx = nullptr; a.dx_dot = nullptr; a.slabs = slabs; a.m = m; a.n = (int)n;
    a.twh = twh;
    hipEvent_t e0, e1;
    (void)hipEventCreate(&e0); (void)hipEventCreate(&e1);
    (void)hipEventRecord(e0, stream);
    if (jtj_run<double>(plan, op, a, packed, stream) != hipSuccess) rc = -4;
    (void)hipEventRecord(e1, stream);
    (void)jtj_unpack<double>(packed, (int)n, JJ, Jy, st, stream);
    if (hipStreamSynchronize(stream) != hipSuccess) rc = -5;
    if (kernel_ms) { float ms = 0; (void)hipEventElapsedTime(&ms, e0, e1); *kernel_ms = ms; }
    (void)hipEventDestroy(e0); (void)hipEventDestroy(e1);
    (void)hipFree(slabs); (void)hipFree(packed); (void)hipFree(st);
    return rc;
}
}

extern "C" {

int mir_solve_box_qp_gpu_d(const mir_box_qp_settings_d* settings, size_t n, const double* P, const double* q,
                           const double* l, const double* u, double* x, int unconstrainedSolution, int* iterations)
{
    return box_qp_entry<double>(settings, n, P, q, l, u, x, unconstrainedSolution, iterations);
}
int mir_solve_box_qp_gpu_s(const mir_box_qp_settings_s* settings, size_t n, const float* P, const float* q,
                           const float* l, const float* u, float* x, int unconstrainedSolution, int* iterations)
{
    return box_qp_entry<float>(settings, n, P, q, l, u, x, unconstrainedSolution, iterations);
}

int mir_lsq_jtj_d(size_t m, size_t n, double* J, const double* y, const double* y_old, const double* dx, int broyden,
                  double* JJ, double* Jy, void* stream, float* kernel_ms)
{
    return jtj_entry<double>(m, n, J, y, y_old, dx, broyden, JJ, Jy, stream, kernel_ms);
}
int mir_lsq_fd_jtj_d(size_t m, size_t n, const double* Yrm, const double* twh, const double* y, double* J,
                     double* JJ, double* Jy, void* stream_, float* kernel_ms)
{
    return fd_jtj_entry(m, n, Yrm, twh, y, J, JJ, Jy, stream_, kernel_ms, false);
}
int mir_lsq_fd_diff_jtj_d(size_t m, size_t n, const double* Drm, const double* twh, const double* y, double* J,
                          double* JJ, double* Jy, void* stream_, float* kernel_ms)
{
    return fd_jtj_entry(m, n, Drm, twh, y, J, JJ, Jy, stream_, kernel_ms, true);
}
int mir_lsq_jtj_plan(size_t elem_size, size_t m, size_t n, int num_cu, int op, int aligned16, size_t out[10])
{
    if ((elem_size != 4 && elem_size != 8) || m == 0 || n == 0 || n > (size_t)1 << 20 || num_cu < 1 || op < 0 || op > 3 || !out) return -1;
    const JtjPlan p = elem_size == 8 ? jtj_plan<double>(m, (int)n, num_cu) : jtj_plan<float>(m, (int)n, num_cu);
    const JtjLaunch l = jtj_resolve(p, (JtjOp)op, aligned16 != 0);
    const bool wide = l.kernel == JtjKernel::wide;
    const size_t v[10] = {(size_t)l.kernel, (size_t)l.ncb, (size_t)l.flat, (size_t)l.nblk, (size_t)l.njobs, l.lds,
                          (size_t)l.nblk * l.njobs, (size_t)l.slab_len, wide ? 0 : (size_t)l.ncb, jtj_slab_elems(p)};
    for (int i = 0; i < 10; ++i) out[i] = v[i];
    return 0;
}
int mir_lsq_jtj_s(size_t m, size_t n, float* J, const float* y, const float* y_old, const float* dx, int broyden,
                  float* JJ, float* Jy, void* stream, float* kernel_ms)
{
    return jtj_entry<float>(m, n, J, y, y_old, dx, broyden, JJ, Jy, stream, kernel_ms);
}
int mir_lsq_selftest_reductions(int rounds, int mismatches[4])
{
    if (!mismatches || rounds <= 0) return -1;
    if (!device_available()) return -2;
    int* d = nullptr;
    if (hipMalloc((void**)&d, 4 * sizeof(int)) != hipSuccess) return -3;
    bool ok = hipMemset(d, 0, 4 * sizeof(int)) == hipSuccess;
    if (ok) {
        hipLaunchKernelGGL(k_selftest_reductions, dim3(2048), dim3(256), 0, nullptr, rounds, 12345u, d);
        ok = hipGetLastError() == hipSuccess && hipDeviceSynchronize() == hipSuccess
          && hipMemcpy(mismatches, d, 4 * sizeof(int), hipMemcpyDeviceToHost) == hipSuccess;
    }
    (void)hipFree(d);
    return ok ? 0 : -4;
}

}
```

mir_optim_amd/csrc/workspace.hip:

```cpp
#include "driver.h"
#include "launch_util.h"

namespace mirlsq {

bool device_available()
{
    int cnt = 0;
    if (hipGetDeviceCount(&cnt) != hipSuccess || cnt <= 0) {
        std::fprintf(stderr, "[mir_optim_amd] no usable HIP device: the MI355X kernels cannot run "
                             "(this library has no CPU fallback)\n");
        return false;
    }
    return true;
}

int query_num_cu()
{
    int dev = 0;
    hipDeviceProp_t prop;
    if (hipGetDevice(&dev) != hipSuccess || hipGetDeviceProperties(&prop, dev) != hipSuccess) return 256;
    return prop.multiProcessorCount > 0 ? prop.multiProcessorCount : 256;
}

template <typename T>
Buffers<T> carve(void* base, size_t m, size_t n, int num_cu)
{
    Buffers<T> b{};
    size_t off = 0;
    auto take = [&](size_t count, size_t elem) {
        void* p = base ? static_cast<char*>(base) + off : nullptr;
        off = align_up(off + count * elem, 256);
        return p;
    };
    b.J = (T*)take(m * n, sizeof(T));
    b.y = (T*)take(m, sizeof(T));
    b.mB = (T*)take(m, sizeof(T));
    b.ytmp = (T*)take(m, sizeof(T));
    b.X = (T*)take(2 * n * n, sizeof(T));
    b.twh = (T*)take(n, sizeof(T));
    b.x = (T*)take(n, sizeof(T));
    b.lower = (T*)take(n, sizeof(T));
    b.upper = (T*)take(n, sizeof(T));
    b.dx = (T*)take(kChainMax * n, sizeof(T));
    b.dx_acc = (T*)take(n, sizeof(T));
    b.trial = (T*)take(kChainMax * n, sizeof(T));
    b.Jy = (T*)take(n, sizeof(T));
    b.JJ = (T*)take(n * n, sizeof(T));
    b.packed = (T*)take(n * (n + 1) / 2 + n + 8, sizeof(T));
    b.partials = (T*)take((size_t)kChainMax * kPartials, sizeof(T));
    b.sum = (T*)take(8 + kChainMax, sizeof(T));
    b.st = (LmState<T>*)take(1, sizeof(LmState<T>));
    b.rec = (ChainRec<T>*)take(kChainMax, sizeof(ChainRec<T>));
    b.slabs = (T*)take(jtj_slab_elems(jtj_plan<T>(m, (int)n, num_cu)), sizeof(T));
    b.lrD = (T*)take((size_t)kLrMax * n, sizeof(T));
    b.lrvec = (T*)take((size_t)lr_len((int)n) + 6, sizeof(T));
    b.lrpart = (T*)take((size_t)lr_blocks(m, num_cu) * lr_len((int)n), sizeof(T));
    for (int k = 0; k < kChainMax; ++k) {
        b.sc[k].Pm = (T*)take(n * n, sizeof(T));
        b.sc[k].A = (T*)take(n * n, sizeof(T));
        b.sc[k].Fg = (T*)take(n * (n | 1), sizeof(T));
        b.sc[k].vec = (T*)take(12 * n, sizeof(T));
        b.sc[k].ivec = (int32_t*)take(2 * n, sizeof(int32_t));
        b.sc[k].dbg = nullptr;
        b.sc[k].coop = (unsigned long long*)take(n > (size_t)kSolveMaxN ? kCoopWords : 0, sizeof(unsigned long long));
        b.sc[k].cS = (T*)take(coop_scratch_elems((int)n), sizeof(T));
    }
    b.sc[0].dbg = (long long*)take(32, sizeof(long long));
    b.bytes = off;
    return b;
}

template <typename T>
mir_lsq_workspace* workspace_create(size_t m, size_t n)
{
    auto* ws = new mir_lsq_workspace();
    ws->m = m; ws->n = n; ws->elem = sizeof(T);
    ws->num_cu = query_num_cu();
    const Buffers<T> sz = carve<T>(nullptr, m, n, ws->num_cu);
    ws->dev_bytes = sz.bytes;
    if (hipMalloc(&ws->dev, ws->dev_bytes) != hipSuccess) {
        std::fprintf(stderr, "[mir_optim_amd] hipMalloc(%zu bytes) failed\n", ws->dev_bytes);
        delete ws;
        return nullptr;
    }
    if (n > (size_t)kSolveMaxN) {
        const Buffers<T> bb = carve<T>(ws->dev, m, n, ws->num_cu);
        for (int k = 0; k < kChainMax; ++k)
            if (hipMemset(bb.sc[k].coop, 0, kCoopWords * sizeof(unsigned long long)) != hipSuccess) {
                std::fprintf(stderr, "[mir_optim_amd] workspace: hipMemset failed\n");
                workspace_destroy(ws);
                return nullptr;
            }
        (void)hipStreamSynchronize(nullptr);
    }
    if (hipGetDevice(&ws->device) != hipSuccess) ws->device = 0;
    if (hipMalloc(&ws->ulr, (size_t)kLrMax * m * sizeof(T)) != hipSuccess
        || hipMalloc(&ws->ytrial, (size_t)kChainMax * m * sizeof(T)) != hipSuccess
        || hipHostMalloc(&ws->pinned, 2 * sizeof(LmState<T>) + (3 * n + 8) * sizeof(T) + 3 * align_up(n * sizeof(T), 256) + 256, hipHostMallocMapped | hipHostMallocCoherent) != hipSuccess
        || hipHostGetDevicePointer(&ws->pinned_dev, ws->pinned, 0) != hipSuccess) {
        std::fprintf(stderr, "[mir_optim_amd] workspace side buffers: allocation failed\n");
        workspace_destroy(ws);
        return nullptr;
    }
    return ws;
}

void workspace_destroy(mir_lsq_workspace* ws)
{
    if (!ws) return;
    for (hipEvent_t e : ws->event_pool) (void)hipEventDestroy(e);
    if (ws->dev) (void)hipFree(ws->dev);
    if (ws->ypanel) (void)hipFree(ws->ypanel);
    if (ws->ytrial) (void)hipFree(ws->ytrial);
    if (ws->ulr) (void)hipFree(ws->ulr);
    if (ws->pinned) (void)hipHostFree(ws->pinned);
    if (ws->pinned_y) (void)hipHostFree(ws->pinned_y);
    if (ws->pinned_J) (void)hipHostFree(ws->pinned_J);
    if (ws->pinned_panel) (void)hipHostFree(ws->pinned_panel);
    for (int k = 0; k < mir_lsq_workspace::kCopyStreams; ++k) {
        if (ws->copy_event[k]) (void)hipEventDestroy(ws->copy_event[k]);
        if (ws->copy_stream[k]) (void)hipStreamDestroy(ws->copy_stream[k]);
    }
    delete ws;
}

template Buffers<double> carve<double>(void*, size_t, size_t, int);
template Buffers<float> carve<float>(void*, size_t, size_t, int);
template mir_lsq_workspace* workspace_create<double>(size_t, size_t);
template mir_lsq_workspace* workspace_create<float>(size_t, size_t);

}


extern "C" {

mir_lsq_workspace* mir_lsq_workspace_create(size_t m, size_t n, size_t elem_size)
{
    if (!mirlsq::device_available() || n == 0 || m == 0) return nullptr;
    mirlsq::preload_jtj(); mirlsq::preload_broyden(); mirlsq::preload_loop(); mirlsq::preload_jacobian();
    if (elem_size == 8) mirlsq::preload_solve_d(); else mirlsq::preload_solve_s();
    (void)hipStreamSynchronize(nullptr);
    if (elem_size == 8) return mirlsq::workspace_create<double>(m, n);
    if (elem_size == 4) return mirlsq::workspace_create<float>(m, n);
    return nullptr;
}
void mir_lsq_workspace_destroy(mir_lsq_workspace* ws) { mirlsq::workspace_destroy(ws); }

}
```

Measured before the change: 1133.

## Skip writing FD Jacobian; keep difference panel and rescale on the fly in Broyden

When the fused finite-difference + JtJ kernel runs in diff mode for f64 with n ≤ 128 and low-rank Broyden enabled, the Jacobian is no longer written out. The raw difference panel is kept instead, and later Broyden sweep and flush kernels rebuild J rows on the fly as panel times 1/twh. This removes one m×n store per full Jacobian evaluation. In exchange the later kernels read the panel plus precomputed inverse step sizes, which adds a small kernel variant and more complex state tracking (j0_panel).

New measurement: 1133. About the same (-0.1%).

```diff
diff --git a/include/mir_optim_amd.h b/include/mir_optim_amd.h
--- a/include/mir_optim_amd.h
+++ b/include/mir_optim_amd.h
@@ -134,6 +134,7 @@
     MIR_LSQ_VARIANT_SOLVE_GENERIC = 1u << 10,
     MIR_LSQ_VARIANT_SOLVE_ONE_WORKGROUP = 1u << 11,
     MIR_LSQ_VARIANT_FD_HOST_COLUMNS = 1u << 13,
+    MIR_LSQ_VARIANT_FD_WRITE_J = 1u << 23,
     MIR_LSQ_VARIANT_NO_PIPELINE = 1u << 22,
     MIR_LSQ_VARIANT_DEBUG_HELPERS_ABSENT = 1u << 12,
     MIR_LSQ_VARIANT_DEBUG_SOLVE = 1u << 7,
@@ -205,6 +206,8 @@
     uint32_t stats_size;
     uint32_t reserved0;
 } mir_lsq_gpu_options;
+
+uint64_t mir_lsq_fd_j_writes_skipped(void);
 
 mir_least_squares_result_d mir_optimize_least_squares_gpu_d(
     const mir_least_squares_settings_d* settings, size_t m, size_t n,
@@ -339,6 +342,11 @@
                      double* JJ, double* Jy, void* stream, float* kernel_ms);
 int mir_lsq_fd_diff_jtj_d(size_t m, size_t n, const double* Drm, const double* twh, const double* y, double* J,
                           double* JJ, double* Jy, void* stream, float* kernel_ms);
+int mir_lsq_broyden_sweep_d(size_t m, size_t n, int k, const double* J, const double* twh, double* U, const double* D,
+                            const double* dx, const double* y, const double* y_old, double* partials, int* nblk, double* reduced,
+                            void* stream);
+int mir_lsq_broyden_flush_d(size_t m, size_t n, int k, double* J, const double* panel, const double* twh, const double* U,
+                            const double* D, void* stream);
 int mir_lsq_jtj_plan(size_t elem_size, size_t m, size_t n, int num_cu, int op, int aligned16, size_t out[10]);
 
 mir_lsq_workspace* mir_lsq_workspace_create(size_t m, size_t n, size_t elem_size);
diff --git a/mir_optim_amd/api.py b/mir_optim_amd/api.py
--- a/mir_optim_amd/api.py
+++ b/mir_optim_amd/api.py
@@ -16,7 +16,7 @@
     "fit_spline_residuals", "variant_lr_cap",
     "VARIANT_BROYDEN_REWRITE", "VARIANT_FD_SEPARATE_FILL", "VARIANT_NO_SPECULATION", "VARIANT_NO_NULL_SKIP",
     "VARIANT_SOLVE_BOUNDED", "VARIANT_DEBUG_SOLVE", "VARIANT_HOST_PROFILE", "VARIANT_SOLVE_GENERIC", "VARIANT_SOLVE_ONE_WORKGROUP", "VARIANT_DEBUG_HELPERS_ABSENT", "VARIANT_FD_HOST_COLUMNS",
-    "VARIANT_NO_PIPELINE", "BatchedOptions", "BatchedExtras", "BATCHED_ABSOLUTE_SIGMA",
+    "VARIANT_NO_PIPELINE", "VARIANT_FD_WRITE_J", "broyden_sweep", "fd_j_writes_skipped", "broyden_flush", "BatchedOptions", "BatchedExtras", "BATCHED_ABSOLUTE_SIGMA",
 ]
 
 MODEL_EXP_DECAY = 0
@@ -38,6 +38,7 @@
 VARIANT_DEBUG_HELPERS_ABSENT = 1 << 12
 VARIANT_FD_HOST_COLUMNS = 1 << 13
 VARIANT_NO_PIPELINE = 1 << 22
+VARIANT_FD_WRITE_J = 1 << 23
 
 
 def variant_lr_cap(k):
@@ -267,6 +268,12 @@
         L.mir_lsq_batched_kernel_s.restype = C.c_int
         L.mir_lsq_batched_kernel_s.argtypes = [C.POINTER(_Ss), sz, sz, C.c_int, C.c_void_p, C.c_void_p, C.c_void_p,
                                                C.c_void_p, sz, C.c_void_p, C.c_void_p, C.POINTER(BatchedOptions)]
+        L.mir_lsq_fd_j_writes_skipped.restype = C.c_uint64
+        L.mir_lsq_fd_j_writes_skipped.argtypes = []
+        L.mir_lsq_broyden_sweep_d.restype = C.c_int
+        L.mir_lsq_broyden_sweep_d.argtypes = [sz, sz, C.c_int] + [C.c_void_p] * 8 + [C.POINTER(C.c_int), C.c_void_p, C.c_void_p]
+        L.mir_lsq_broyden_flush_d.restype = C.c_int
+        L.mir_lsq_broyden_flush_d.argtypes = [sz, sz, C.c_int] + [C.c_void_p] * 6
         L.mir_lsq_jtj_plan.restype = C.c_int
         L.mir_lsq_jtj_plan.argtypes = [sz, sz, sz, C.c_int, C.c_int, C.c_int, C.POINTER(sz * 10)]
         L.mir_lsq_selftest_reductions.restype = C.c_int
@@ -713,6 +720,46 @@
     return out
 
 
+def fd_j_writes_skipped():
+    return int(lib().mir_lsq_fd_j_writes_skipped())
+
+
+def broyden_sweep(J, U, D, dx, y, y_old, k, twh=None):
+    J = np.ascontiguousarray(J, dtype=np.float64)
+    m, n = J.shape
+    ln = 2 * n + 35
+    dJ, dU, dD = DeviceBuffer(J), DeviceBuffer(np.ascontiguousarray(U, dtype=np.float64)), DeviceBuffer(np.ascontiguousarray(D, dtype=np.float64))
+    ddx, dy, dyo = (DeviceBuffer(np.ascontiguousarray(v, dtype=np.float64)) for v in (dx, y, y_old))
+    dt = DeviceBuffer(np.ascontiguousarray(twh, dtype=np.float64)) if twh is not None else None
+    dP = DeviceBuffer(nbytes=1024 * ln * 8, dtype=np.float64, shape=(1024, ln))
+    dR = DeviceBuffer(nbytes=ln * 8, dtype=np.float64, shape=(ln,))
+    nblk = C.c_int(0)
+    rc = lib().mir_lsq_broyden_sweep_d(m, n, int(k), dJ.ptr, dt.ptr if dt else None, dU.ptr, dD.ptr, ddx.ptr, dy.ptr, dyo.ptr, dP.ptr,
+                                       C.byref(nblk), dR.ptr, None)
+    if rc != 0:
+        raise RuntimeError(f"mir_lsq_broyden_sweep_d failed: {rc}")
+    out = dP.download()[:nblk.value].copy(), dR.download(), dU.download().reshape(16, m)[k].copy()
+    for b in (dJ, dU, dD, ddx, dy, dyo, dP, dR) + ((dt,) if dt else ()):
+        b.free()
+    return out
+
+
+def broyden_flush(J, U, D, k, panel=None, twh=None):
+    src = np.ascontiguousarray(J if panel is None else panel, dtype=np.float64)
+    m, n = src.shape
+    dJ = DeviceBuffer(src) if panel is None else DeviceBuffer(np.full((m, n), np.nan))
+    dU, dD = DeviceBuffer(np.ascontiguousarray(U, dtype=np.float64)), DeviceBuffer(np.ascontiguousarray(D, dtype=np.float64))
+    dp = DeviceBuffer(src) if panel is not None else None
+    dt = DeviceBuffer(np.ascontiguousarray(twh, dtype=np.float64)) if panel is not None else None
+    rc = lib().mir_lsq_broyden_flush_d(m, n, int(k), dJ.ptr, dp.ptr if dp else None, dt.ptr if dt else None, dU.ptr, dD.ptr, None)
+    if rc != 0:
+        raise RuntimeError(f"mir_lsq_broyden_flush_d failed: {rc}")
+    out = dJ.download()
+    for b in (dJ, dU, dD) + ((dp, dt) if dp else ()):
+        b.free()
+    return out
+
+
 
 class Spline:
 
diff --git a/mir_optim_amd/csrc/broyden_launch.h b/mir_optim_amd/csrc/broyden_launch.h
--- a/mir_optim_amd/csrc/broyden_launch.h
+++ b/mir_optim_amd/csrc/broyden_launch.h
@@ -40,4 +40,9 @@
 template <typename T> hipError_t lr_sumsq_final(const T* partials, int pstride, int nblk, int count, T* out, hipStream_t s);
 template <typename T> hipError_t lr_flush(T* J, const T* U, const T* D, int k, size_t m, int n, int num_cu, hipStream_t s);
 
+constexpr int kLrPanelMaxN = 128;
+hipError_t lr_sweep_panel(const LrArgs<double>& a, const double* inv_twh, int nblk, hipStream_t s);
+hipError_t lr_flush_panel(double* J, const double* panel, const double* inv_twh, const double* U, const double* D, int k, size_t m, int n,
+                          int num_cu, hipStream_t s);
+
 }
diff --git a/mir_optim_amd/csrc/broyden_lr.h b/mir_optim_amd/csrc/broyden_lr.h
--- a/mir_optim_amd/csrc/broyden_lr.h
+++ b/mir_optim_amd/csrc/broyden_lr.h
@@ -41,135 +41,25 @@
     return yy;
 }
 
+template <typename T>
+__device__ __forceinline__ T lr_panel_elem(T d, T inv)
+{
+#pragma clang fp contract(off)
+    return inv == T(0) ? T(0) : d * inv;
+}
+
 template <typename T, int NCP, bool VEC>
 __global__ __launch_bounds__(256, (NCP <= 4 ? 4 : 1)) void k_broyden_lr(const LrArgs<T> a)
 {
-    using P2 = typename LrPair<T>::type;
-    __shared__ T red[4][lr_len(kLrMaxN)];
-    __shared__ T coef[kLrMax];
-    const int lane = threadIdx.x & 63, wave = threadIdx.x >> 6;
-    const int q = lane >> 4, p = lane & 15;
-    const int n = a.n, k = a.k;
-    const size_t m = a.m;
-    const size_t G = (m + 3) / 4;
-    const size_t nw = (size_t)gridDim.x * 4, wid = (size_t)blockIdx.x * 4 + wave;
-    const size_t per = (G + nw - 1) / nw;
-    const size_t gb = wid * per;
-    const size_t ge = gb + per < G ? gb + per : G;
-    if (a.spec_rec && !lr_spec_go(a.spec_rec[0], a.absTolerance, a.relTolerance)) {
-        const T yy = lr_wave_sumsq(a.y, m, gb, ge, q);
-        if (q == 0 && p == 0) red[wave][0] = yy;
-        __syncthreads();
-        const int len = lr_len(n);
-        T* out = a.partials + (size_t)blockIdx.x * len;
-        for (int e = threadIdx.x; e < len; e += blockDim.x) out[e] = e == lr_yy(n) ? (red[0][0] + red[1][0]) + (red[2][0] + red[3][0]) : T(0);
-        return;
-    }
-
-    for (int l = wave; l < k; l += 4) {
-        T s = 0;
-        for (int j = lane; j < n; j += kWave) s += a.D[(size_t)l * n + j] * a.dx[j];
-        s = wave_sum(s);
-        if (lane == 0) coef[l] = s;
-    }
-    T d0[NCP], d1[NCP];
-    int coff[NCP];
-    bool ok0[NCP], ok1[NCP];
-#pragma unroll
-    for (int c = 0; c < NCP; ++c) {
-        const int col = 32 * c + 2 * p;
-        ok0[c] = col < n;
-        ok1[c] = col + 1 < n;
-        coff[c] = ok0[c] ? col : 0;
-        const T t0 = a.dx[ok0[c] ? col : 0], t1 = a.dx[ok1[c] ? col + 1 : 0];
-        d0[c] = ok0[c] ? t0 : T(0);
-        d1[c] = ok1[c] ? t1 : T(0);
-    }
-    __syncthreads();
-    const bool own = p < k;
-    const T cp = own ? coef[p] : T(0);
-    const T* __restrict__ Up = a.U + (size_t)(own ? p : 0) * m;
-    T* __restrict__ Uk = a.U + (size_t)k * m;
-    const T nd = -(T(1) / *a.dx_dot);
-
-    T va0[NCP], va1[NCP], ga0[NCP], ga1[NCP];
-#pragma unroll
-    for (int c = 0; c < NCP; ++c) { va0[c] = 0; va1[c] = 0; ga0[c] = 0; ga1[c] = 0; }
-    T wl = 0, hl = 0, uu = 0, uy = 0, yy = 0;
-
-    constexpr int UNR = NCP == 1 ? 4 : (NCP == 2 ? 2 : 1);
-    for (size_t g0 = gb; g0 < ge; g0 += UNR) {
-        T v0[UNR][NCP], v1[UNR][NCP], ynv[UNR], yov[UNR], ulv[UNR];
-#pragma unroll
-        for (int e = 0; e < UNR; ++e) {
-            const size_t g = g0 + e < ge ? g0 + e : ge - 1;
-            const size_t row = 4 * g + q;
-            const size_t rr = row < m ? row : m - 1;
-            const T* __restrict__ rp = a.J + rr * (size_t)n;
-#pragma unroll
-            for (int c = 0; c < NCP; ++c) {
-                if constexpr (VEC) {
-                    typedef T lr_v2 __attribute__((ext_vector_type(2)));
-                    const lr_v2 t = __builtin_nontemporal_load(reinterpret_cast<const lr_v2*>(rp + coff[c]));
-                    v0[e][c] = t.x;
-                    v1[e][c] = t.y;
-                } else {
-                    v0[e][c] = rp[coff[c]];
-                    v1[e][c] = rp[ok1[c] ? coff[c] + 1 : 0];
-                }
-            }
-            ynv[e] = a.y[rr];
-            yov[e] = a.y_old[rr];
-            ulv[e] = own ? Up[rr] : T(0);
-        }
-#pragma unroll
-        for (int e = 0; e < UNR; ++e) {
-            if (g0 + e < ge) {
-                const size_t row = 4 * (g0 + e) + q;
-                const bool rok = row < m;
-                T yn = ynv[e];
-                const T yo = yov[e], ul = ulv[e];
-                T s = ul * cp;
-#pragma unroll
-                for (int c = 0; c < NCP; ++c) s += v0[e][c] * d0[c] + v1[e][c] * d1[c];
-                s = sum16(s);
-                T u = nd * ((yo - yn) + s);
-                if (!rok) { u = 0; yn = 0; }
-                if (rok && p == 0) Uk[row] = u;
-#pragma unroll
-                for (int c = 0; c < NCP; ++c) {
-                    va0[c] += v0[e][c] * u;
-                    va1[c] += v1[e][c] * u;
-                    ga0[c] += v0[e][c] * yn;
-                    ga1[c] += v1[e][c] * yn;
-                }
-                wl += ul * u;
-                hl += ul * yn;
-                uu += u * u;
-                uy += u * yn;
-                yy = dfma(yn, yn, yy);
-            }
-        }
-    }
-
-    auto qsum = [](T v) { v += wave_shfl_xor(v, 16); v += wave_shfl_xor(v, 32); return v; };
-#pragma unroll
-    for (int c = 0; c < NCP; ++c) { va0[c] = qsum(va0[c]); va1[c] = qsum(va1[c]); ga0[c] = qsum(ga0[c]); ga1[c] = qsum(ga1[c]); }
-    wl = qsum(wl); hl = qsum(hl); uu = qsum(uu); uy = qsum(uy); yy = qsum(yy);
-    if (q == 0) {
-#pragma unroll
-        for (int c = 0; c < NCP; ++c) {
-            if (ok0[c]) { red[wave][coff[c]] = va0[c]; red[wave][n + coff[c]] = ga0[c]; }
-            if (ok1[c]) { red[wave][coff[c] + 1] = va1[c]; red[wave][n + coff[c] + 1] = ga1[c]; }
-        }
-        red[wave][2 * n + p] = wl;
-        red[wave][2 * n + kLrMax + p] = hl;
-        if (p == 0) { red[wave][2 * n + 2 * kLrMax] = uu; red[wave][2 * n + 2 * kLrMax + 1] = uy; red[wave][lr_yy(n)] = yy; }
-    }
-    __syncthreads();
-    const int len = lr_len(n);
-    T* out = a.partials + (size_t)blockIdx.x * len;
-    for (int e = threadIdx.x; e < len; e += blockDim.x) out[e] = (red[0][e] + red[1][e]) + (red[2][e] + red[3][e]);
+    constexpr bool PANEL = false;
+    const T* const inv_twh = nullptr;
+#include "broyden_lr_sweep.inc"
+}
+template <typename T, int NCP, bool VEC>
+__global__ __launch_bounds__(256, 4) void k_broyden_lr_panel(const LrArgs<T> a, const T* __restrict__ inv_twh)
+{
+    constexpr bool PANEL = true;
+#include "broyden_lr_sweep.inc"
 }
 
 template <typename T>
@@ -285,68 +175,17 @@
 __global__ __launch_bounds__(256) void k_lr_flush(T* J, const T* __restrict__ U, const T* __restrict__ D,
                                                   int k, size_t m, int n)
 {
-    using P2 = typename LrPair<T>::type;
-    extern __shared__ unsigned char lr_smem[];
-    T* Ds = reinterpret_cast<T*>(lr_smem);
-    for (int e = threadIdx.x; e < k * n; e += blockDim.x) Ds[e] = D[e];
-    __syncthreads();
-    const int lane = threadIdx.x & 63;
-    const int q = lane >> 4, p = lane & 15;
-    int coff[NCP];
-    bool ok0[NCP], ok1[NCP];
-#pragma unroll
-    for (int c = 0; c < NCP; ++c) {
-        const int col = 32 * c + 2 * p;
-        ok0[c] = col < n;
-        ok1[c] = col + 1 < n;
-        coff[c] = ok0[c] ? col : 0;
-    }
-    const size_t G = (m + 3) / 4;
-    const size_t wave_id = ((size_t)blockIdx.x * blockDim.x + threadIdx.x) >> 6;
-    const size_t nwaves = ((size_t)gridDim.x * blockDim.x) >> 6;
-    for (size_t g = wave_id; g < G; g += nwaves) {
-        const size_t row = 4 * g + q;
-        const bool rok = row < m;
-        const size_t rr = rok ? row : m - 1;
-        T* rp = J + rr * (size_t)n;
-        const T* sp = rp;
-        T v0[NCP], v1[NCP];
-#pragma unroll
-        for (int c = 0; c < NCP; ++c) {
-            if constexpr (VEC) {
-                typedef T lr_v2 __attribute__((ext_vector_type(2)));
-                const lr_v2 t = __builtin_nontemporal_load(reinterpret_cast<const lr_v2*>(sp + coff[c]));
-                v0[c] = t.x;
-                v1[c] = t.y;
-            } else {
-                v0[c] = sp[coff[c]];
-                v1[c] = sp[ok1[c] ? coff[c] + 1 : 0];
-            }
-        }
-        for (int l = 0; l < k; ++l) {
-            const T ul = U[(size_t)l * m + rr];
-#pragma unroll
-            for (int c = 0; c < NCP; ++c) {
-                v0[c] += ul * Ds[l * n + coff[c]];
-                v1[c] += ul * Ds[l * n + (ok1[c] ? coff[c] + 1 : 0)];
-            }
-        }
-        if (rok) {
-#pragma unroll
-            for (int c = 0; c < NCP; ++c) {
-                if constexpr (VEC) {
-                    if (ok0[c]) {
-                        typedef T lr_v2 __attribute__((ext_vector_type(2)));
-                        lr_v2 t; t.x = v0[c]; t.y = v1[c];
-                        __builtin_nontemporal_store(t, reinterpret_cast<lr_v2*>(rp + coff[c]));
-                    }
-                } else {
-                    if (ok0[c]) rp[coff[c]] = v0[c];
-                    if (ok1[c]) rp[coff[c] + 1] = v1[c];
-                }
-            }
-        }
-    }
+    constexpr bool PANEL = false;
+    const T* const panel = nullptr;
+    const T* const inv_twh = nullptr;
+#include "broyden_lr_flush.inc"
+}
+template <typename T, int NCP, bool VEC>
+__global__ __launch_bounds__(256) void k_lr_flush_panel(T* J, const T* __restrict__ panel, const T* __restrict__ inv_twh,
+                                                        const T* __restrict__ U, const T* __restrict__ D, int k, size_t m, int n)
+{
+    constexpr bool PANEL = true;
+#include "broyden_lr_flush.inc"
 }
 
 }
diff --git a/mir_optim_amd/csrc/broyden_lr_flush.inc b/mir_optim_amd/csrc/broyden_lr_flush.inc
--- /dev/null
+++ b/mir_optim_amd/csrc/broyden_lr_flush.inc
@@ -0,0 +1,75 @@
+    using P2 = typename LrPair<T>::type;
+    extern __shared__ unsigned char lr_smem[];
+    T* Ds = reinterpret_cast<T*>(lr_smem);
+    for (int e = threadIdx.x; e < k * n; e += blockDim.x) Ds[e] = D[e];
+    __syncthreads();
+    const int lane = threadIdx.x & 63;
+    const int q = lane >> 4, p = lane & 15;
+    int coff[NCP];
+    bool ok0[NCP], ok1[NCP];
+#pragma unroll
+    for (int c = 0; c < NCP; ++c) {
+        const int col = 32 * c + 2 * p;
+        ok0[c] = col < n;
+        ok1[c] = col + 1 < n;
+        coff[c] = ok0[c] ? col : 0;
+    }
+    T i0[PANEL ? NCP : 1], i1[PANEL ? NCP : 1];
+    if constexpr (PANEL) {
+#pragma unroll
+        for (int c = 0; c < NCP; ++c) {
+            i0[c] = inv_twh[coff[c]];
+            i1[c] = inv_twh[ok1[c] ? coff[c] + 1 : 0];
+        }
+    }
+    const size_t G = (m + 3) / 4;
+    const size_t wave_id = ((size_t)blockIdx.x * blockDim.x + threadIdx.x) >> 6;
+    const size_t nwaves = ((size_t)gridDim.x * blockDim.x) >> 6;
+    for (size_t g = wave_id; g < G; g += nwaves) {
+        const size_t row = 4 * g + q;
+        const bool rok = row < m;
+        const size_t rr = rok ? row : m - 1;
+        T* rp = J + rr * (size_t)n;
+        const T* sp = rp;
+        if constexpr (PANEL) sp = panel + rr * (size_t)n;
+        T v0[NCP], v1[NCP];
+#pragma unroll
+        for (int c = 0; c < NCP; ++c) {
+            if constexpr (VEC) {
+                typedef T lr_v2 __attribute__((ext_vector_type(2)));
+                const lr_v2 t = __builtin_nontemporal_load(reinterpret_cast<const lr_v2*>(sp + coff[c]));
+                v0[c] = t.x;
+                v1[c] = t.y;
+            } else {
+                v0[c] = sp[coff[c]];
+                v1[c] = sp[ok1[c] ? coff[c] + 1 : 0];
+            }
+            if constexpr (PANEL) {
+                v0[c] = lr_panel_elem(v0[c], i0[c]);
+                v1[c] = lr_panel_elem(v1[c], i1[c]);
+            }
+        }
+        for (int l = 0; l < k; ++l) {
+            const T ul = U[(size_t)l * m + rr];
+#pragma unroll
+            for (int c = 0; c < NCP; ++c) {
+                v0[c] += ul * Ds[l * n + coff[c]];
+                v1[c] += ul * Ds[l * n + (ok1[c] ? coff[c] + 1 : 0)];
+            }
+        }
+        if (rok) {
+#pragma unroll
+            for (int c = 0; c < NCP; ++c) {
+                if constexpr (VEC) {
+                    if (ok0[c]) {
+                        typedef T lr_v2 __attribute__((ext_vector_type(2)));
+                        lr_v2 t; t.x = v0[c]; t.y = v1[c];
+                        __builtin_nontemporal_store(t, reinterpret_cast<lr_v2*>(rp + coff[c]));
+                    }
+                } else {
+                    if (ok0[c]) rp[coff[c]] = v0[c];
+                    if (ok1[c]) rp[coff[c] + 1] = v1[c];
+                }
+            }
+        }
+    }
diff --git a/mir_optim_amd/csrc/broyden_lr_sweep.inc b/mir_optim_amd/csrc/broyden_lr_sweep.inc
--- /dev/null
+++ b/mir_optim_amd/csrc/broyden_lr_sweep.inc
@@ -0,0 +1,138 @@
+    using P2 = typename LrPair<T>::type;
+    __shared__ T red[4][lr_len(kLrMaxN)];
+    __shared__ T coef[kLrMax];
+    const int lane = threadIdx.x & 63, wave = threadIdx.x >> 6;
+    const int q = lane >> 4, p = lane & 15;
+    const int n = a.n, k = a.k;
+    const size_t m = a.m;
+    const size_t G = (m + 3) / 4;
+    const size_t nw = (size_t)gridDim.x * 4, wid = (size_t)blockIdx.x * 4 + wave;
+    const size_t per = (G + nw - 1) / nw;
+    const size_t gb = wid * per;
+    const size_t ge = gb + per < G ? gb + per : G;
+    if (a.spec_rec && !lr_spec_go(a.spec_rec[0], a.absTolerance, a.relTolerance)) {
+        const T yy = lr_wave_sumsq(a.y, m, gb, ge, q);
+        if (q == 0 && p == 0) red[wave][0] = yy;
+        __syncthreads();
+        const int len = lr_len(n);
+        T* out = a.partials + (size_t)blockIdx.x * len;
+        for (int e = threadIdx.x; e < len; e += blockDim.x) out[e] = e == lr_yy(n) ? (red[0][0] + red[1][0]) + (red[2][0] + red[3][0]) : T(0);
+        return;
+    }
+
+    for (int l = wave; l < k; l += 4) {
+        T s = 0;
+        for (int j = lane; j < n; j += kWave) s += a.D[(size_t)l * n + j] * a.dx[j];
+        s = wave_sum(s);
+        if (lane == 0) coef[l] = s;
+    }
+    T d0[NCP], d1[NCP];
+    T i0[PANEL ? NCP : 1], i1[PANEL ? NCP : 1];
+    int coff[NCP];
+    bool ok0[NCP], ok1[NCP];
+#pragma unroll
+    for (int c = 0; c < NCP; ++c) {
+        const int col = 32 * c + 2 * p;
+        ok0[c] = col < n;
+        ok1[c] = col + 1 < n;
+        coff[c] = ok0[c] ? col : 0;
+        const T t0 = a.dx[ok0[c] ? col : 0], t1 = a.dx[ok1[c] ? col + 1 : 0];
+        d0[c] = ok0[c] ? t0 : T(0);
+        d1[c] = ok1[c] ? t1 : T(0);
+        if constexpr (PANEL) {
+            i0[c] = inv_twh[coff[c]];
+            i1[c] = inv_twh[ok1[c] ? coff[c] + 1 : 0];
+        }
+    }
+    __syncthreads();
+    const bool own = p < k;
+    const T cp = own ? coef[p] : T(0);
+    const T* __restrict__ Up = a.U + (size_t)(own ? p : 0) * m;
+    T* __restrict__ Uk = a.U + (size_t)k * m;
+    const T nd = -(T(1) / *a.dx_dot);
+
+    T va0[NCP], va1[NCP], ga0[NCP], ga1[NCP];
+#pragma unroll
+    for (int c = 0; c < NCP; ++c) { va0[c] = 0; va1[c] = 0; ga0[c] = 0; ga1[c] = 0; }
+    T wl = 0, hl = 0, uu = 0, uy = 0, yy = 0;
+
+    constexpr int UNR = NCP == 1 ? 4 : (NCP == 2 ? 2 : 1);
+    for (size_t g0 = gb; g0 < ge; g0 += UNR) {
+        T v0[UNR][NCP], v1[UNR][NCP], ynv[UNR], yov[UNR], ulv[UNR];
+#pragma unroll
+        for (int e = 0; e < UNR; ++e) {
+            const size_t g = g0 + e < ge ? g0 + e : ge - 1;
+            const size_t row = 4 * g + q;
+            const size_t rr = row < m ? row : m - 1;
+            const T* __restrict__ rp = a.J + rr * (size_t)n;
+#pragma unroll
+            for (int c = 0; c < NCP; ++c) {
+                if constexpr (VEC) {
+                    typedef T lr_v2 __attribute__((ext_vector_type(2)));
+                    const lr_v2 t = __builtin_nontemporal_load(reinterpret_cast<const lr_v2*>(rp + coff[c]));
+                    v0[e][c] = t.x;
+                    v1[e][c] = t.y;
+                } else {
+                    v0[e][c] = rp[coff[c]];
+                    v1[e][c] = rp[ok1[c] ? coff[c] + 1 : 0];
+                }
+            }
+            ynv[e] = a.y[rr];
+            yov[e] = a.y_old[rr];
+            ulv[e] = own ? Up[rr] : T(0);
+        }
+#pragma unroll
+        for (int e = 0; e < UNR; ++e) {
+            if (g0 + e < ge) {
+                const size_t row = 4 * (g0 + e) + q;
+                const bool rok = row < m;
+                T yn = ynv[e];
+                const T yo = yov[e], ul = ulv[e];
+                if constexpr (PANEL) {
+#pragma unroll
+                    for (int c = 0; c < NCP; ++c) {
+                        v0[e][c] = lr_panel_elem(v0[e][c], i0[c]);
+                        v1[e][c] = lr_panel_elem(v1[e][c], i1[c]);
+                    }
+                }
+                T s = ul * cp;
+#pragma unroll
+                for (int c = 0; c < NCP; ++c) s += v0[e][c] * d0[c] + v1[e][c] * d1[c];
+                s = sum16(s);
+                T u = nd * ((yo - yn) + s);
+                if (!rok) { u = 0; yn = 0; }
+                if (rok && p == 0) Uk[row] = u;
+#pragma unroll
+                for (int c = 0; c < NCP; ++c) {
+                    va0[c] += v0[e][c] * u;
+                    va1[c] += v1[e][c] * u;
+                    ga0[c] += v0[e][c] * yn;
+                    ga1[c] += v1[e][c] * yn;
+                }
+                wl += ul * u;
+                hl += ul * yn;
+                uu += u * u;
+                uy += u * yn;
+                yy = dfma(yn, yn, yy);
+            }
+        }
+    }
+
+    auto qsum = [](T v) { v += wave_shfl_xor(v, 16); v += wave_shfl_xor(v, 32); return v; };
+#pragma unroll
+    for (int c = 0; c < NCP; ++c) { va0[c] = qsum(va0[c]); va1[c] = qsum(va1[c]); ga0[c] = qsum(ga0[c]); ga1[c] = qsum(ga1[c]); }
+    wl = qsum(wl); hl = qsum(hl); uu = qsum(uu); uy = qsum(uy); yy = qsum(yy);
+    if (q == 0) {
+#pragma unroll
+        for (int c = 0; c < NCP; ++c) {
+            if (ok0[c]) { red[wave][coff[c]] = va0[c]; red[wave][n + coff[c]] = ga0[c]; }
+            if (ok1[c]) { red[wave][coff[c] + 1] = va1[c]; red[wave][n + coff[c] + 1] = ga1[c]; }
+        }
+        red[wave][2 * n + p] = wl;
+        red[wave][2 * n + kLrMax + p] = hl;
+        if (p == 0) { red[wave][2 * n + 2 * kLrMax] = uu; red[wave][2 * n + 2 * kLrMax + 1] = uy; red[wave][lr_yy(n)] = yy; }
+    }
+    __syncthreads();
+    const int len = lr_len(n);
+    T* out = a.partials + (size_t)blockIdx.x * len;
+    for (int e = threadIdx.x; e < len; e += blockDim.x) out[e] = (red[0][e] + red[1][e]) + (red[2][e] + red[3][e]);
diff --git a/mir_optim_amd/csrc/driver.h b/mir_optim_amd/csrc/driver.h
--- a/mir_optim_amd/csrc/driver.h
+++ b/mir_optim_amd/csrc/driver.h
@@ -92,6 +92,7 @@
 struct Buffers {
     T *J, *y, *mB, *ytmp;
     T *X, *twh;
+    T* inv_twh;
     T *x, *lower, *upper, *dx, *dx_acc, *trial, *Jy, *JJ, *packed, *partials, *sum;
     LmState<T>* st;
     ChainRec<T>* rec;
@@ -129,6 +130,9 @@
     FB fbr = nullptr;
     FB fbd = nullptr;
     int fd_fused = 0;
+    bool j0_panel = false;
+    bool fd_keep_panel = false;
+    uint64_t fd_j_writes_skipped = 0;
     int sums_pending = 0;
     uint32_t fd_batch;
     bool device_cb;
@@ -248,6 +252,17 @@
     bool unpack_in_reduce(JtjOp op) const { return !comm && jtj_unpacks(plan, op); }
     JtjUnpack<T> unpack_target() { JtjUnpack<T> u; u.JJ = B.JJ; u.Jy = B.Jy; return u; }
     bool finish_products(bool direct);
+    hipError_t sweep_j0(LrArgs<T>& a, int nblk)
+    {
+        if constexpr (sizeof(T) == 8) {
+            if (j0_panel) {
+                a.J = static_cast<const T*>(ws->ypanel);
+                return lr_sweep_panel(a, B.inv_twh, nblk, stream);
+            }
+        }
+        a.J = B.J;
+        return lr_sweep<T>(a, nblk, stream);
+    }
     bool jacobian_products(bool broyden, const T* y_dev, const T* yold_dev);
     bool fd_device();
     static void fd_task_trampoline(mir_least_squares_task task, uint32_t totalThreads, uint32_t threadId, uint32_t j);
diff --git a/mir_optim_amd/csrc/launch_broyden.hip b/mir_optim_amd/csrc/launch_broyden.hip
--- a/mir_optim_amd/csrc/launch_broyden.hip
+++ b/mir_optim_amd/csrc/launch_broyden.hip
@@ -56,6 +56,48 @@
     return lr_flush_ncp<T, 16>(J, U, D, k, m, n, (int)blocks, vec, s);
 }
 
+namespace {
+template <int NCP>
+hipError_t lr_sweep_panel_ncp(const LrArgs<double>& a, const double* inv_twh, int nblk, bool vec, hipStream_t s)
+{
+    if (vec) MIRLSQ_LAUNCH((k_broyden_lr_panel<double, NCP, true>), dim3(nblk), dim3(256), 0, s, a, inv_twh);
+    else MIRLSQ_LAUNCH((k_broyden_lr_panel<double, NCP, false>), dim3(nblk), dim3(256), 0, s, a, inv_twh);
+    return hipGetLastError();
+}
+template <int NCP>
+hipError_t lr_flush_panel_ncp(double* J, const double* panel, const double* inv_twh, const double* U, const double* D, int k, size_t m,
+                              int n, int nblk, bool vec, hipStream_t s)
+{
+    const size_t lds = (size_t)k * n * sizeof(double);
+    if (vec) MIRLSQ_LAUNCH((k_lr_flush_panel<double, NCP, true>), dim3(nblk), dim3(256), lds, s, J, panel, inv_twh, U, D, k, m, n);
+    else MIRLSQ_LAUNCH((k_lr_flush_panel<double, NCP, false>), dim3(nblk), dim3(256), lds, s, J, panel, inv_twh, U, D, k, m, n);
+    return hipGetLastError();
+}
+}
+hipError_t lr_sweep_panel(const LrArgs<double>& a, const double* inv_twh, int nblk, hipStream_t s)
+{
+    if (a.n > kLrPanelMaxN || a.k < 0 || a.k >= kLrMax || !inv_twh) return hipErrorInvalidValue;
+    const bool vec = (a.n % 2 == 0) && (reinterpret_cast<uintptr_t>(a.J) % (2 * sizeof(double)) == 0);
+    const int ncp = (a.n + 31) / 32;
+    if (ncp <= 1) return lr_sweep_panel_ncp<1>(a, inv_twh, nblk, vec, s);
+    if (ncp <= 2) return lr_sweep_panel_ncp<2>(a, inv_twh, nblk, vec, s);
+    return lr_sweep_panel_ncp<4>(a, inv_twh, nblk, vec, s);
+}
+hipError_t lr_flush_panel(double* J, const double* panel, const double* inv_twh, const double* U, const double* D, int k, size_t m, int n,
+                          int num_cu, hipStream_t s)
+{
+    if (n > kLrPanelMaxN || k < 0 || k > kLrMax || !panel || !inv_twh || panel == J) return hipErrorInvalidValue;
+    const size_t G = (m + 3) / 4;
+    size_t blocks = (G + 3) / 4;
+    if (blocks > (size_t)num_cu * 8) blocks = (size_t)num_cu * 8;
+    if (blocks < 1) blocks = 1;
+    const bool vec = (n % 2 == 0) && (reinterpret_cast<uintptr_t>(J) % 16 == 0) && (reinterpret_cast<uintptr_t>(panel) % 16 == 0);
+    const int ncp = (n + 31) / 32;
+    if (ncp <= 1) return lr_flush_panel_ncp<1>(J, panel, inv_twh, U, D, k, m, n, (int)blocks, vec, s);
+    if (ncp <= 2) return lr_flush_panel_ncp<2>(J, panel, inv_twh, U, D, k, m, n, (int)blocks, vec, s);
+    return lr_flush_panel_ncp<4>(J, panel, inv_twh, U, D, k, m, n, (int)blocks, vec, s);
+}
+
 template <typename T>
 hipError_t lr_reduce(const T* partials, int nblk, int n, T* out, hipStream_t s)
 {
diff --git a/mir_optim_amd/csrc/misc_kernels.h b/mir_optim_amd/csrc/misc_kernels.h
--- a/mir_optim_amd/csrc/misc_kernels.h
+++ b/mir_optim_amd/csrc/misc_kernels.h
@@ -114,6 +114,27 @@
         X[(size_t)(2 * j + 1) * n + k] = k == j ? xmh : xv;
     }
     if (threadIdx.x == 0) twh[j] = xph - xmh;
+}
+
+template <typename T>
+__global__ void k_fd_points_inv(const T* __restrict__ x, const T* __restrict__ lower, const T* __restrict__ upper,
+                                T eps, int n, T* __restrict__ X, T* __restrict__ twh, T* __restrict__ inv_twh)
+{
+    const int j = blockIdx.x;
+    const T save = x[j];
+    T xmh = save - eps, xph = save + eps;
+    xmh = dfmax(xmh, lower[j]);
+    xph = dfmin(xph, upper[j]);
+    for (int k = threadIdx.x; k < n; k += blockDim.x) {
+        const T xv = x[k];
+        X[(size_t)(2 * j) * n + k] = k == j ? xph : xv;
+        X[(size_t)(2 * j + 1) * n + k] = k == j ? xmh : xv;
+    }
+    if (threadIdx.x == 0) {
+        const T t = xph - xmh;
+        twh[j] = t;
+        inv_twh[j] = t == 0 ? T(0) : T(1) / t;
+    }
 }
 
 template <typename T>
diff --git a/mir_optim_amd/csrc/solver_jacobian.hip b/mir_optim_amd/csrc/solver_jacobian.hip
--- a/mir_optim_amd/csrc/solver_jacobian.hip
+++ b/mir_optim_amd/csrc/solver_jacobian.hip
@@ -11,18 +11,26 @@
     if (lr_k >= lr_cap) {
         const uint64_t launches_before = launches_now();
         struct Excl { Solver* s; uint64_t l0; ~Excl() { s->launches_excluded += s->launches_now() - l0; } } excl{this, launches_before};
-        if (!ok(lr_flush<T>(B.J, U, B.lrD, lr_k, m, (int)n, ws->num_cu, stream), "broyden flush")) return false;
+        bool folded = false;
+        if constexpr (sizeof(T) == 8) {
+            if (j0_panel) {
+                if (!ok(lr_flush_panel(B.J, static_cast<const T*>(ws->ypanel), B.inv_twh, U, B.lrD, lr_k, m, (int)n, ws->num_cu, stream), "broyden flush")) return false;
+                j0_panel = false;
+                folded = true;
+            }
+        }
+        if (!folded && !ok(lr_flush<T>(B.J, U, B.lrD, lr_k, m, (int)n, ws->num_cu, stream), "broyden flush")) return false;
         lr_k = 0;
         if (stats) stats->broyden_flushes++;
         if (!plain_products(yold_dev)) return false;
         if (stats) stats->jtj_resyncs++;
     }
     LrArgs<T> a{};
-    a.J = B.J; a.U = U; a.D = B.lrD; a.dx = B.dx_acc; a.dx_dot = &B.st->dx_dot; a.y = y_dev; a.y_old = yold_dev;
+    a.U = U; a.D = B.lrD; a.dx = B.dx_acc; a.dx_dot = &B.st->dx_dot; a.y = y_dev; a.y_old = yold_dev;
     a.partials = B.lrpart; a.m = m; a.n = (int)n; a.k = lr_k;
     const int nblk = lr_blocks(m, ws->num_cu), len = lr_len((int)n);
     ev_begin(1);
-    if (!ok(lr_sweep<T>(a, nblk, stream), "broyden sweep")) return false;
+    if (!ok(sweep_j0(a, nblk), "broyden sweep")) return false;
     ev_end();
     if (!ok(lr_reduce<T>(B.lrpart, nblk, (int)n, B.lrvec, stream), "broyden reduce")) return false;
     if (comm && !allreduce(B.lrvec, (size_t)len, 1)) return false;
@@ -57,7 +65,7 @@
 bool Solver<T>::jacobian_products(bool broyden, const T* y_dev, const T* yold_dev)
 {
     if (broyden && lowrank) return broyden_lowrank(y_dev, yold_dev);
-    if (!broyden) lr_k = 0;
+    if (!broyden) { lr_k = 0; j0_panel = false; }
     JtjArgs<T> a{};
     a.J = B.J; a.Jout = B.J; a.y = y_dev; a.y_old = yold_dev; a.dx = B.dx_acc; a.dx_dot = &B.st->dx_dot;
     a.slabs = B.slabs; a.m = m; a.n = (int)n;
@@ -65,6 +73,12 @@
         const JtjOp op = fd_fused == 2 ? JtjOp::fd_diff : JtjOp::fd;
         fd_fused = 0;
         a.J = static_cast<const T*>(ws->ypanel); a.twh = B.twh;
+        if (op == JtjOp::fd_diff && fd_keep_panel) {
+            a.Jout = nullptr;
+            j0_panel = true;
+            ++fd_j_writes_skipped;
+        }
+        fd_keep_panel = false;
         const bool direct = unpack_in_reduce(op);
         ev_begin(3);
         if (!ok(jtj_run<T>(plan, op, a, B.packed, stream, direct ? unpack_target() : JtjUnpack<T>{}), "fd + jtj kernel")) return false;
@@ -82,7 +96,6 @@
 template <typename T>
 bool Solver<T>::fd_device()
 {
-    MIRLSQ_LAUNCH(k_fd_points<T>, dim3(n), dim3(64), 0, stream, B.x, B.lower, B.upper, sd.jacobianEpsilon, (int)n, B.X, B.twh);
     for (uint32_t j = 0; j < n; ++j) {
         const T save = xh[j];
         T xmh = save - S->jacobianEpsilon, xph = save + S->jacobianEpsilon;
@@ -108,6 +121,12 @@
     if (fb && fd_batch && fd_batch / 2 < pb) pb = fd_batch / 2 ? fd_batch / 2 : 1;
     const bool no_fuse = (variant & MIR_LSQ_VARIANT_FD_SEPARATE_FILL) != 0;
     const bool use_diff = fbd && plan.fd_diff.kernel != JtjKernel::none && pb == n && !no_fuse;
+    fd_keep_panel = use_diff && sizeof(T) == 8 && plan.fd_diff.kernel == JtjKernel::fdp && (int)n <= kLrPanelMaxN && lowrank
+        && !(variant & MIR_LSQ_VARIANT_FD_WRITE_J);
+    if (fd_keep_panel)
+        MIRLSQ_LAUNCH(k_fd_points_inv<T>, dim3(n), dim3(64), 0, stream, B.x, B.lower, B.upper, sd.jacobianEpsilon, (int)n, B.X, B.twh, B.inv_twh);
+    else
+        MIRLSQ_LAUNCH(k_fd_points<T>, dim3(n), dim3(64), 0, stream, B.x, B.lower, B.upper, sd.jacobianEpsilon, (int)n, B.X, B.twh);
     const size_t need = (use_diff ? 1 : 2) * pb * m * sizeof(T);
     if (ws->ypanel_bytes < need) {
         if (ws->ypanel) (void)hipFree(ws->ypanel);
diff --git a/mir_optim_amd/csrc/solver_loop.hip b/mir_optim_amd/csrc/solver_loop.hip
--- a/mir_optim_amd/csrc/solver_loop.hip
+++ b/mir_optim_amd/csrc/solver_loop.hip
@@ -326,13 +326,13 @@
     spec_events_from = events.size();
     if (stats) stats->fused_rounds++;
     LrArgs<T> a{};
-    a.J = B.J; a.U = static_cast<T*>(ws->ulr); a.D = B.lrD; a.dx = B.dx; a.dx_dot = &B.rec[0].new_dx_dot; a.y = ytr; a.y_old = y;
+    a.U = static_cast<T*>(ws->ulr); a.D = B.lrD; a.dx = B.dx; a.dx_dot = &B.rec[0].new_dx_dot; a.y = ytr; a.y_old = y;
     a.partials = B.lrpart; a.m = m; a.n = (int)n; a.k = lr_k;
     a.spec_rec = B.rec; a.absTolerance = sd.absTolerance; a.relTolerance = sd.relTolerance;
     const int nblk = lr_blocks(m, ws->num_cu), len = lr_len((int)n);
     spec_enqueue = true;
     ev_begin(1);
-    const bool swept = ok(lr_sweep<T>(a, nblk, stream), "broyden sweep");
+    const bool swept = ok(sweep_j0(a, nblk), "broyden sweep");
     ev_end();
     spec_enqueue = false;
     if (!swept || !ok(lr_reduce<T>(B.lrpart, nblk, (int)n, B.lrvec, stream), "broyden reduce")) return false;
@@ -586,6 +586,8 @@
     teardown();
     return ret;
 }
+
+thread_local uint64_t tl_fd_j_writes_skipped = 0;
 
 template <typename T>
 typename Abi<T>::Result solve_entry(const typename Abi<T>::Settings* settings, size_t m, size_t n, T* x, const T* l,
@@ -627,6 +629,7 @@
         if (s.trace) s.trace->count = 0;
     }
     const typename Abi<T>::Result r = s.run();
+    tl_fd_j_writes_skipped = s.fd_j_writes_skipped;
     if (s.stats_user) std::memcpy(s.stats_user, &s.stats_local, s.stats_bytes);
     return r;
 }
@@ -642,3 +645,5 @@
 }
 
 MIRLSQ_DEFINE_PRELOAD(loop)
+
+extern "C" uint64_t mir_lsq_fd_j_writes_skipped(void) { return mirlsq::tl_fd_j_writes_skipped; }
diff --git a/mir_optim_amd/csrc/unit_entries.hip b/mir_optim_amd/csrc/unit_entries.hip
--- a/mir_optim_amd/csrc/unit_entries.hip
+++ b/mir_optim_amd/csrc/unit_entries.hip
@@ -140,6 +140,19 @@
     (void)hipFree(slabs); (void)hipFree(packed); (void)hipFree(st);
     return rc;
 }
+
+__global__ void k_unit_inv_twh(const double* __restrict__ twh, int n, double* __restrict__ inv)
+{
+    const int j = blockIdx.x * blockDim.x + threadIdx.x;
+    if (j < n) { const double t = twh[j]; inv[j] = t == 0 ? 0.0 : 1.0 / t; }
+}
+struct LrUnitScratch {
+    double* p = nullptr;
+    double* dxdot() const { return p; }
+    double* inv() const { return p + 8; }
+    bool make(size_t n) { return hipMalloc((void**)&p, sizeof(double) * (8 + n)) == hipSuccess; }
+    ~LrUnitScratch() { if (p) (void)hipFree(p); }
+};
 }
 
 extern "C" {
@@ -169,6 +182,49 @@
                           double* JJ, double* Jy, void* stream_, float* kernel_ms)
 {
     return fd_jtj_entry(m, n, Drm, twh, y, J, JJ, Jy, stream_, kernel_ms, true);
+}
+int mir_lsq_broyden_sweep_d(size_t m, size_t n, int k, const double* J, const double* twh, double* U, const double* D, const double* dx,
+                            const double* y, const double* y_old, double* partials, int* nblk, double* reduced, void* stream_)
+{
+    if (!device_available()) return -1;
+    if (n == 0 || m == 0 || n > (size_t)kLrMaxN || k < 0 || k >= kLrMax || !nblk) return -2;
+    hipStream_t stream = static_cast<hipStream_t>(stream_);
+    LrUnitScratch sc;
+    if (!sc.make(n)) return -3;
+    hipLaunchKernelGGL(k_sumsq_partial<double>, dim3(1), dim3(256), 0, stream, dx, n, sc.dxdot() + 1);
+    hipLaunchKernelGGL(k_sumsq_final<double>, dim3(1), dim3(256), 0, stream, sc.dxdot() + 1, 1, sc.dxdot());
+    LrArgs<double> a{};
+    a.J = J; a.U = U; a.D = D; a.dx = dx; a.dx_dot = sc.dxdot(); a.y = y; a.y_old = y_old; a.partials = partials;
+    a.m = m; a.n = (int)n; a.k = k;
+    *nblk = lr_blocks(m, query_num_cu());
+    hipError_t e;
+    if (twh) {
+        hipLaunchKernelGGL(k_unit_inv_twh, dim3((unsigned)((n + 63) / 64)), dim3(64), 0, stream, twh, (int)n, sc.inv());
+        e = lr_sweep_panel(a, sc.inv(), *nblk, stream);
+    } else {
+        e = lr_sweep<double>(a, *nblk, stream);
+    }
+    if (e != hipSuccess) return -4;
+    if (lr_reduce<double>(partials, *nblk, (int)n, reduced, stream) != hipSuccess) return -4;
+    return hipStreamSynchronize(stream) == hipSuccess ? 0 : -5;
+}
+int mir_lsq_broyden_flush_d(size_t m, size_t n, int k, double* J, const double* panel, const double* twh, const double* U,
+                            const double* D, void* stream_)
+{
+    if (!device_available()) return -1;
+    if (n == 0 || m == 0 || n > (size_t)kLrMaxN || k < 0 || k > kLrMax || (panel && !twh)) return -2;
+    hipStream_t stream = static_cast<hipStream_t>(stream_);
+    LrUnitScratch sc;
+    if (!sc.make(n)) return -3;
+    hipError_t e;
+    if (panel) {
+        hipLaunchKernelGGL(k_unit_inv_twh, dim3((unsigned)((n + 63) / 64)), dim3(64), 0, stream, twh, (int)n, sc.inv());
+        e = lr_flush_panel(J, panel, sc.inv(), U, D, k, m, (int)n, query_num_cu(), stream);
+    } else {
+        e = lr_flush<double>(J, U, D, k, m, (int)n, query_num_cu(), stream);
+    }
+    if (e != hipSuccess) return -4;
+    return hipStreamSynchronize(stream) == hipSuccess ? 0 : -5;
 }
 int mir_lsq_jtj_plan(size_t elem_size, size_t m, size_t n, int num_cu, int op, int aligned16, size_t out[10])
 {
diff --git a/mir_optim_amd/csrc/workspace.hip b/mir_optim_amd/csrc/workspace.hip
--- a/mir_optim_amd/csrc/workspace.hip
+++ b/mir_optim_amd/csrc/workspace.hip
@@ -66,6 +66,7 @@
         b.sc[k].cS = (T*)take(coop_scratch_elems((int)n), sizeof(T));
     }
     b.sc[0].dbg = (long long*)take(32, sizeof(long long));
+    b.inv_twh = (T*)take(n, sizeof(T));
     b.bytes = off;
     return b;
 }
```
